# ssheybani/baby-vision-curriculum

Hardware: AMD Instinct MI355X
Metric: video clips/sec (node) VideoMAE-base 16x224^2 bf16 pretraining (higher is better)
Workload: dtype bf16; 1 GPU; VideoMAE-base (ViT-B/16 encoder, 4-layer decoder), 16x224x224 clips, tubelet 2, 90% tube mask, full training step (fwd + MSE + bwd + GradScaler + SGD-Nesterov); clips_per_gpu=256, global_batch=256, parallelism=dp1, weights=random init N(0,0.02), seed 0

## Files before the change

### baby-vision-curriculum_amd/_lib.py

```python
import ctypes
import os
import sys

_HERE = os.path.dirname(os.path.abspath(__file__))
LIB_PATH = os.environ.get("BVC_LIB_PATH") or os.path.join(_HERE, "libbvc_hip.so")

c_void_p, c_int, c_int64, c_float, c_char_p = ctypes.c_void_p, ctypes.c_int, ctypes.c_int64, ctypes.c_float, ctypes.c_char_p
c_double = ctypes.c_double


class BvcError(RuntimeError):
    pass


class VideoMAEConfigC(ctypes.Structure):
    _fields_ = [(n, c_int) for n in (
        "image_size", "patch_size", "num_channels", "num_frames", "tubelet_size",
        "hidden_size", "num_hidden_layers", "num_attention_heads", "intermediate_size",
        "decoder_hidden_size", "decoder_num_hidden_layers", "decoder_num_attention_heads",
        "decoder_intermediate_size")] + [("layer_norm_eps", c_float), ("decoder_norm_eps", c_float),
                                         ("norm_pix_loss", c_int)]


class VitConfigC(ctypes.Structure):
# ... 110 lines not shown
                                        c_void_p]),
    "bvc_videomae_forward_dual": (c_int, [c_void_p, c_void_p, ctypes.POINTER(PixelFormatC), c_void_p, c_void_p, c_int, c_void_p, c_void_p,
                                          c_void_p, c_void_p]),
    "bvc_videomae_backward": (c_int, [c_void_p, c_void_p, c_void_p, BUCKET_FN, c_void_p, c_void_p]),
    "bvc_videomae_tap": (c_int, [c_void_p, c_char_p, c_void_p, c_int64, ctypes.POINTER(c_int64), c_void_p]),
    "bvc_videomae_encoder_param_numel": (c_int64, [ctypes.POINTER(VideoMAEConfigC)]),
    "bvc_videomae_encoder_create": (c_int, [ctypes.POINTER(VideoMAEConfigC), c_int, ctypes.POINTER(c_void_p)]),
    "bvc_videomae_encoder_destroy": (None, [c_void_p]),
    "bvc_videomae_encode": (c_int, [c_void_p, c_void_p, c_int, c_void_p, c_void_p, c_void_p, c_float, c_void_p, c_void_p, c_void_p]),
    "bvc_videomae_encode_px": (c_int, [c_void_p, c_void_p, ctypes.POINTER(PixelFormatC), c_int, c_void_p, c_void_p, c_void_p, c_float,
                                       c_void_p, c_void_p, c_void_p]),
    "bvc_videomae_encode_ex": (c_int, [c_void_p, c_void_p, ctypes.POINTER(PixelFormatC), c_int, c_void_p, c_void_p, c_void_p, c_float,
                                       c_void_p, c_void_p, ctypes.POINTER(IntrospectC), c_void_p]),
    "bvc_videomae_cls_introspect": (c_int, [c_void_p, ctypes.POINTER(IntrospectC), c_void_p]),
    "bvc_videomae_encoder_fc_norm_backward": (c_int, [c_void_p, c_void_p, c_void_p, c_void_p, c_void_p, c_void_p]),
    "bvc_videomae_cls_create": (c_int, [ctypes.POINTER(VideoMAEConfigC), c_int, ctypes.POINTER(c_void_p)]),
    "bvc_videomae_cls_destroy": (None, [c_void_p]),
    "bvc_videomae_cls_forward_px": (c_int, [c_void_p, c_void_p, ctypes.POINTER(PixelFormatC), c_int, c_void_p, c_void_p, c_void_p,
                                            c_float, c_void_p, c_void_p, c_void_p]),
    "bvc_videomae_cls_backward": (c_int, [c_void_p, c_void_p, c_void_p, c_void_p, c_void_p, BUCKET_FN, c_void_p, c_void_p]),
    "bvc_videomae_cls_shadow": (c_int, [c_void_p, c_int, ctypes.POINTER(c_void_p), ctypes.POINTER(c_int64)]),
    "bvc_vit_param_count":(c_int, [ctypes.POINTER(VitConfigC)]),
    "bvc_vit_param_numel": (c_int64, [ctypes.POINTER(VitConfigC)]),
    "bvc_vit_param_info": (c_int, [ctypes.POINTER(VitConfigC), c_int, ctypes.c_char_p, c_int, ctypes.POINTER(c_int64),
                                   ctypes.POINTER(c_int64), ctypes.POINTER(c_int), ctypes.POINTER(c_int64)]),
    "bvc_vit_create": (c_int, [ctypes.POINTER(VitConfigC), c_int, ctypes.POINTER(c_void_p)]),
    "bvc_vit_destroy": (None, [c_void_p]),
    "bvc_vit_forward": (c_int, [c_void_p, c_void_p, c_void_p, c_int, c_int, c_void_p, c_void_p, c_void_p]),
    "bvc_vit_forward_px": (c_int, [c_void_p, c_void_p, ctypes.POINTER(PixelFormatC), c_void_p, c_int, c_int, c_void_p, c_void_p, c_void_p]),
    "bvc_vit_backward": (c_int, [c_void_p, c_void_p, c_void_p, BUCKET_FN, c_void_p, c_void_p]),
    "bvc_predictor_param_count": (c_int, [ctypes.POINTER(PredictorConfigC)]),
    "bvc_predictor_param_numel": (c_int64, [ctypes.POINTER(PredictorConfigC)]),
    "bvc_predictor_param_info": (c_int, [ctypes.POINTER(PredictorConfigC), c_int, ctypes.c_char_p, c_int, ctypes.POINTER(c_int64),
                                         ctypes.POINTER(c_int64), ctypes.POINTER(c_int), ctypes.POINTER(c_int64)]),
    "bvc_predictor_create": (c_int, [ctypes.POINTER(PredictorConfigC), c_int, c_int, c_int, ctypes.POINTER(c_void_p)]),
    "bvc_predictor_destroy": (None, [c_void_p]),
    "bvc_predictor_forward": (c_int, [c_void_p, c_void_p, c_void_p, c_void_p, c_int, c_int, c_int, c_int, c_void_p, c_void_p, c_void_p]),
    "bvc_predictor_backward": (c_int, [c_void_p, c_void_p, c_void_p, c_void_p, c_void_p]),
    "bvc_predictor_backward_cb": (c_int, [c_void_p, c_void_p, c_void_p, c_void_p, BUCKET_FN, c_void_p, c_void_p]),
    "bvc_op_target_select": (c_int, [c_void_p, c_void_p, c_void_p, c_int, c_int, c_int, c_int, c_int, c_float, c_void_p]),
    "bvc_op_smooth_l1_workspace": (c_int, [c_int64]),
    "bvc_op_smooth_l1_fwd": (c_int, [c_void_p, c_void_p, c_int64, c_void_p, c_void_p, c_void_p]),
    "bvc_op_smooth_l1_bwd": (c_int, [c_void_p, c_void_p, c_void_p, c_int64, c_void_p, c_void_p]),
    "bvc_op_ema": (c_int, [c_void_p, c_void_p, c_int64, c_float, c_void_p]),
    "bvc_op_token_mean": (c_int, [c_void_p, c_int, c_int, c_int, c_void_p, c_void_p]),
    "bvc_op_token_mean_bwd": (c_int, [c_void_p, c_int, c_int, c_int, c_void_p, c_void_p]),
    "bvc_op_gemm": (c_int, [ctypes.POINTER(GemmDesc), c_int, c_int, c_int, c_int, c_void_p]),
    "bvc_op_gemm_num_tiles": (c_int, [ctypes.POINTER(GemmDesc), c_int]),
    "bvc_op_gemm_kernel": (c_int, [ctypes.POINTER(GemmDesc), c_int, c_int, c_int, c_int, ctypes.c_char_p, c_int]),
    "bvc_op_gemm_plan_dw": (c_int, [ctypes.POINTER(GemmDesc), c_int]),
    "bvc_op_gemm_gate": (c_int, [ctypes.POINTER(GemmDesc), ctypes.POINTER(BranchDropC), c_int, c_int, c_int, c_void_p]),
    "bvc_op_gemm_gate_kernel": (c_int, [ctypes.POINTER(GemmDesc), c_int, ctypes.c_char_p, c_int]),
    "bvc_op_layernorm_bwd_gate": (c_int, [c_void_p, c_void_p, c_void_p, c_void_p, c_void_p, c_void_p, c_int, c_void_p, c_void_p, c_void_p,
                                          c_void_p, c_int, c_int, ctypes.POINTER(BranchDropC), c_int, c_int, c_void_p]),
    "bvc_op_dropout_mask": (c_int, [ctypes.c_uint64, ctypes.c_uint64, c_int, c_int, c_int, c_int, c_float, c_void_p, c_void_p]),
    "bvc_dropout_mask_host": (c_int, [ctypes.c_uint64, ctypes.c_uint64, c_int, c_int, c_int, c_int, c_float, c_void_p]),
    "bvc_op_clip_transform_workspace": (c_int64, [c_int, c_int, c_int]),
    "bvc_op_clip_transform": (c_int, [c_void_p, c_int, c_int, c_int, c_int, c_void_p, c_void_p, c_int, c_int, c_int, c_void_p, c_void_p, c_void_p]),
    "bvc_clip_transform_host": (c_int, [c_void_p, c_int, c_int, c_int, c_int, c_void_p, c_int, c_int, c_int, c_void_p]),
    "bvc_aug_blur_weights": (c_int, [c_float, ctypes.POINTER(ctypes.c_int32), ctypes.POINTER(ctypes.c_uint32), ctypes.POINTER(ctypes.c_uint32)]),
    "bvc_op_clip_post_workspace": (c_int64, [c_int, c_int, c_int]),
    "bvc_op_clip_post": (c_int, [c_void_p, c_void_p, c_void_p, c_int, c_int, c_int, c_void_p, c_void_p, c_void_p]),
    "bvc_clip_post_host": (c_int, [c_void_p, c_void_p, c_int, c_int, c_int, c_void_p]),
    "bvc_videomae_cls_set_drop": (c_int, [c_void_p, ctypes.POINTER(BranchDropC), c_int, c_void_p]),
    "bvc_videomae_encoder_set_drop": (c_int, [c_void_p, ctypes.POINTER(BranchDropC), c_int, c_void_p]),
    "bvc_videomae_cls_set_mix": (c_int, [c_void_p, c_void_p, c_int, c_void_p]),
    "bvc_videomae_encoder_set_mix": (c_int, [c_void_p, c_void_p, c_int, c_void_p]),
    "bvc_vit_set_drop": (c_int, [c_void_p, ctypes.POINTER(BranchDropC), c_int, c_void_p]),
    "bvc_predictor_set_drop": (c_int, [c_void_p, ctypes.POINTER(BranchDropC), c_int, c_void_p]),
    "bvc_op_attention_fwd": (c_int, [c_void_p, c_void_p, c_void_p, c_int, c_int, c_int, c_int, c_void_p]),
    "bvc_op_attention_bwd": (c_int, [c_void_p, c_void_p, c_void_p, c_void_p, c_void_p, c_void_p, c_int, c_int, c_int, c_int, c_void_p]),
    "bvc_op_attention_bwd_part": (c_int, [c_void_p, c_void_p, c_void_p, c_void_p, c_void_p, c_void_p, c_int, c_int, c_int, c_int, c_int, c_void_p]),
    "bvc_op_attention_width": (c_int, [c_int]),
    "bvc_op_attention_fwd_scaled": (c_int, [c_void_p, c_void_p, c_void_p, c_int, c_int, c_int, c_int, ctypes.c_float, c_void_p]),
    "bvc_op_attention_bwd_scaled": (c_int, [c_void_p, c_void_p, c_void_p, c_void_p, c_void_p, c_void_p, c_int, c_int, c_int, c_int,
                                            ctypes.c_float, c_void_p]),
    "bvc_op_attention_probs": (c_int, [c_void_p, c_void_p, c_void_p, c_int, c_int, c_int, c_int, ctypes.c_float, c_void_p]),
    "bvc_op_layernorm_fwd": (c_int, [c_void_p, c_int, c_int, c_int, c_void_p, c_void_p, c_void_p, c_void_p, c_void_p,
                                     c_int, c_int, c_float, c_void_p]),
    "bvc_op_layernorm_bwd": (c_int, [c_void_p, c_void_p, c_int, c_int, c_int, c_void_p, c_void_p, c_void_p, c_void_p,
                                     c_int, c_void_p, c_void_p, c_void_p, c_void_p, c_int, c_int, c_void_p]),
    "bvc_op_layernorm_bwd_workspace": (c_int64, [c_int, c_int]),
    "bvc_op_colsum_bf16": (c_int, [c_void_p, c_int, c_int, c_int, c_float, c_void_p, c_void_p, c_void_p]),
    "bvc_op_colsum_f32": (c_int, [c_void_p, c_int, c_int, c_int, c_int, c_int, c_void_p, c_void_p]),
    "bvc_op_cast_bf16": (c_int, [c_void_p, c_void_p, c_int64, c_void_p]),
    "bvc_op_row_normalize": (c_int, [c_void_p, c_void_p, c_void_p, c_int, c_int, c_float, c_void_p]),
    "bvc_op_row_normalize_bwd": (c_int, [c_void_p, c_void_p, c_void_p, c_void_p, c_int, c_int, c_void_p]),
    "bvc_op_nce_finalize": (c_int, [c_void_p, c_int, c_float, c_int64, c_void_p, c_void_p, c_void_p]),
    "bvc_op_sgd_step": (c_int, [c_void_p, c_void_p, c_void_p, c_int64, c_float, c_float, c_float, c_float, c_int, c_int, c_int,
                                c_void_p, c_void_p, c_int, c_void_p, c_void_p]),
    "bvc_videomae_shadow": (c_int, [c_void_p, c_int, ctypes.POINTER(c_void_p), ctypes.POINTER(c_int64)]),
    "bvc_vit_shadow": (c_int, [c_void_p, c_int, ctypes.POINTER(c_void_p), ctypes.POINTER(c_int64)]),
    "bvc_predictor_shadow": (c_int, [c_void_p, c_int, ctypes.POINTER(c_void_p), ctypes.POINTER(c_int64)]),
    "bvc_op_adam_prepare": (c_int, [c_void_p, c_double, c_double, c_double, c_void_p, c_void_p]),
    "bvc_op_adam_step": (c_int, [c_void_p, c_void_p, c_void_p, c_void_p, c_int64, c_double, c_double, c_double, c_double, c_double,
                                 c_int, c_int, c_void_p, c_void_p, c_void_p, c_int, c_void_p, c_void_p]),
    "bvc_op_row_ln_selected": (c_int, [c_int, c_int, c_int, c_int]),
    "bvc_op_sgd_step_segments": (c_int, [c_void_p, c_void_p, c_void_p, c_int64, c_void_p, c_void_p, c_void_p, c_int, c_void_p, c_void_p, c_void_p,
                                         c_int, c_void_p, c_void_p]),
    "bvc_op_adam_step_segments": (c_int, [c_void_p, c_void_p, c_void_p, c_void_p, c_int64, c_void_p, c_void_p, c_void_p, c_int, c_void_p, c_void_p,
                                          c_void_p, c_void_p, c_void_p, c_int, c_void_p, c_void_p]),
    "bvc_op_sgd_step_table": (c_int, [c_void_p, c_void_p, c_void_p, c_int64, c_void_p, c_void_p, c_void_p, c_int, c_int] + [c_void_p] * 7 +
                                      [c_void_p, c_void_p, c_void_p, c_int, c_void_p, c_void_p]),
    "bvc_op_adam_step_table": (c_int, [c_void_p, c_void_p, c_void_p, c_void_p, c_int64, c_void_p, c_void_p, c_void_p, c_int, c_int] + [c_void_p] * 7 +
                                       [c_void_p, c_void_p, c_void_p, c_void_p, c_int, c_void_p, c_void_p]),
    "bvc_op_lars_step_table": (c_int, [c_void_p, c_void_p, c_void_p, c_int64, c_void_p, c_void_p, c_void_p, c_int, c_void_p, c_int64, c_void_p,
                                       c_int] + [c_void_p] * 7 + [c_void_p, c_void_p, c_void_p, c_void_p, c_void_p, c_int, c_void_p, c_void_p]),
    "bvc_op_lamb_step_table": (c_int, [c_void_p, c_void_p, c_void_p, c_void_p, c_int64, c_void_p, c_void_p, c_void_p, c_int, c_void_p, c_int64,
                                       c_void_p, c_int] + [c_void_p] * 7 +
                                      [c_void_p, c_void_p, c_void_p, c_void_p, c_void_p, c_void_p, c_int, c_void_p, c_void_p]),
    "bvc_op_nonfinite_check": (c_int, [c_void_p, c_int64, c_void_p, c_void_p]),
    "bvc_op_grad_norm_item_cap": (c_int, []),
    "bvc_op_grad_norm_chain": (c_int, []),
    "bvc_grad_norm_items_host": (c_int, [c_void_p, c_void_p, c_int, c_void_p, c_int64, c_void_p, ctypes.POINTER(c_int64)]),
    "bvc_op_grad_sqnorm_items": (c_int, [c_void_p, c_void_p, c_int64, c_void_p, c_int, c_void_p, c_void_p, c_void_p, c_int, c_void_p, c_void_p]),
    "bvc_op_clip_finalize": (c_int, [c_void_p, c_int, c_float, c_void_p, c_void_p, c_void_p]),
    "bvc_op_scale_by_dev": (c_int, [c_void_p, c_int64, c_void_p, c_void_p]),
    "bvc_op_mask_index": (c_int, [c_void_p, c_int, c_int, c_int, c_int, c_void_p, c_void_p, c_void_p, c_void_p]),
    "bvc_op_dual_mask_index": (c_int, [c_void_p, c_void_p, c_int, c_int, c_int, c_int, c_void_p, c_void_p, c_void_p, c_void_p]),
    "bvc_op_gather_patches": (c_int, [c_void_p, c_void_p, c_void_p, c_int, c_int, c_int, c_int, c_int, c_int, c_int, c_int, c_void_p]),
    "bvc_op_gather_patches_mix": (c_int, [c_void_p, ctypes.POINTER(PixelFormatC), c_void_p, c_void_p, c_void_p, c_int, c_int, c_int, c_int,
                                          c_int, c_int, c_int, c_int, c_void_p]),
    "bvc_op_pixel_labels": (c_int, [c_void_p, c_void_p, c_void_p, c_int, c_int, c_int, c_int, c_int, c_int, c_int, c_int, c_int, c_void_p]),
    "bvc_comm_unique_id": (c_int, [c_void_p]),
    "bvc_comm_init": (c_int, [c_int, c_int, c_void_p, ctypes.POINTER(c_void_p)]),
    "bvc_comm_destroy": (c_int, [c_void_p]),
    "bvc_comm_stream": (c_void_p, [c_void_p]),
    "bvc_comm_rank": (c_int, [c_void_p]),
    "bvc_comm_world": (c_int, [c_void_p]),
    "bvc_comm_library": (c_char_p, []),
    "bvc_allreduce_bucket": (c_int, [c_void_p, c_void_p, c_int64, c_int, c_void_p]),
    "bvc_comm_wait": (c_int, [c_void_p, c_void_p]),
    "bvc_allgather": (c_int, [c_void_p, c_void_p, c_void_p, c_int64, c_void_p]),
    "bvc_allreduce": (c_int, [c_void_p, c_void_p, c_int64, c_int, c_void_p]),
    "bvc_broadcast": (c_int, [c_void_p, c_void_p, c_int64, c_int, c_void_p]),
}

_lib = None

_det_flag = False
_det_pushed = False


def use_deterministic_algorithms(mode):
    global _det_flag
    _det_flag = bool(mode)
    lib()


def are_deterministic_algorithms_enabled():
    return _det_flag


def _sync_deterministic(L):
    global _det_pushed
    torch = sys.modules.get("torch")
    want = _det_flag or (torch is not None and torch.are_deterministic_algorithms_enabled())
    if want != _det_pushed:
        rc = L.bvc_set_option(b"deterministic", 1 if want else 0)
        if rc != 0:
            raise BvcError(f"bvc_set_option(deterministic) failed with status {rc}")
        _det_pushed = want


def lib():
    global _lib
# ... 32 lines not shown
```

### baby-vision-curriculum_amd/csrc/context.h

```cpp
#pragma once
#include <functional>

#include "stack.h"

namespace bvc {

struct Shadow {
    bf16_t* wbf = nullptr;
    int64_t numel = 0;
    bool valid = false;
    int alloc(Arena& a, int64_t n) { numel = n; return a.alloc(&wbf, (size_t)n); }
    int refresh(const float* params, hipStream_t st);
    int query(int vouch, void** p, int64_t* n);
};

struct MixState {
    ClipMix* table = nullptr;
    int* status = nullptr;
    const bvc_clip_mix* armed = nullptr;
    int samples = 0;
};
int alloc_mix(Arena& a, MixState& m, int max_batch);
int set_mix(MixState& m, const bvc_clip_mix* mix, int samples, int max_batch, const char* who);

template <typename Config>
PatchGeom patch_geom(const Config& c) { return PatchGeom{c.num_frames, c.num_channels, c.image_size, c.image_size, c.tubelet_size, c.patch_size}; }
inline int seq_len(PatchGeom g) { return (g.T / g.ts) * (g.H / g.ps) * (g.W / g.ps); }
inline int patch_dim(PatchGeom g) { return g.C * g.ts * g.ps * g.ps; }
int pixel_src(const char* who, const void* pixels, const bvc_pixel_format* fmt, int channels, PixelSrc* out);

struct PatchFront {
    PatchGeom pg;
    int L = 0, Kp = 0;
    int* idx_all = nullptr;
    bf16_t* Ape = nullptr;
    int alloc(Arena& a, PatchGeom geom, size_t max_tokens, bool identity_list);
    int embed(PixelSrc px, const int* idx, int B, int N, const bf16_t* w, const float* bias, const float* pos, float* out, int D,
              hipStream_t st, const char* who, MixState* mix = nullptr, bool* mixed = nullptr);
    int embed_backward(Work& w, int M, int D, float* gw, float* gb, hipStream_t st);
};

int stack_forward(Work& w, Stack& s, const std::vector<LayerOff>& off, int B, int N, hipStream_t st, bool chain_ln, const LayerTail* last = nullptr);
int stack_backward(Work& w, Stack& s, const std::vector<LayerOff>& off, float* dres, float* G, int B, int N, hipStream_t st,
                   bvc_bucket_fn on_bucket, void* user, const LayerTail* last = nullptr);
int join_both(Work& w, hipStream_t st, bvc_bucket_fn on_bucket, void* user);

int param_info(const ParamTable& t, int index, char* name, int name_cap, int64_t* offset, int64_t* numel, int* ndim, int64_t shape[5]);

struct Making {
    std::function<void()> undo;
    bool done = false;
    ~Making() { if (!done) undo(); }
};
int refuse_operand_extent(const char* who, int max_batch, size_t tokens_per_clip, size_t bf16_columns, const char* side_name);

}
```

### baby-vision-curriculum_amd/csrc/context.hip

```cpp
#include "context.h"

#include <stdio.h>

namespace bvc {

int Shadow::refresh(const float* params, hipStream_t st) {
    const bool vouched = valid;
    valid = false;
    return vouched ? BVC_OK : launch_cast_bf16(params, wbf, (size_t)numel, st);
}

int Shadow::query(int vouch, void** p, int64_t* n) {
    if (p) *p = wbf;
    if (n) *n = numel;
    if (vouch >= 0) valid = vouch != 0;
    return BVC_OK;
}

int alloc_mix(Arena& a, MixState& m, int max_batch) {
    TRY(a.alloc(&m.table, (size_t)max_batch));
    return a.alloc(&m.status, 4);
}

int set_mix(MixState& m, const bvc_clip_mix* mix, int samples, int max_batch, const char* who) {
    m.armed = nullptr;
    if (!mix) return BVC_OK;
    BVC_REQUIRE(samples >= 1 && samples <= max_batch, "%s: %d samples outside [1, %d]", who, samples, max_batch);
    m.armed = mix;
    m.samples = samples;
    return BVC_OK;
}

static int gather_for_forward(MixState& m, bool* mixed, PixelSrc pixels, const int* idx, bf16_t* A, int B, int N, PatchGeom pg, const char* who,
                              hipStream_t st) {
    const bvc_clip_mix* src = m.armed;
    m.armed = nullptr;
    *mixed = src != nullptr;
    if (!src) return launch_gather_patches(pixels, idx, A, B, N, pg, st);
    BVC_REQUIRE(m.samples == B, "%s: the mix was set for %d samples, the call has %d", who, m.samples, B);
    BVC_CHECK_HIP(hipMemcpyAsync(m.table, src, (size_t)B * sizeof(ClipMix), hipMemcpyDeviceToDevice, st));
    BVC_CHECK_HIP(hipMemsetAsync(m.status, 0, 4, st));
    return launch_gather_patches_mix(pixels, idx, A, B, N, pg, m.table, st, m.status);
}

int pixel_src(const char* who, const void* pixels, const bvc_pixel_format* fmt, int channels, PixelSrc* out) {
    PixelSrc px = pixels_f32((const float*)pixels);
    if (fmt && fmt->dtype != BVC_PIXELS_F32) {
        BVC_REQUIRE(fmt->dtype == BVC_PIXELS_U8, "%s: pixel format: dtype %d unknown", who, fmt->dtype);
        BVC_REQUIRE(channels <= 4, "%s: pixel format: uint8 input supports at most 4 channels", who);
        px.is_u8 = 1;
        for (int c = 0; c < 4; ++c) {
            BVC_REQUIRE(fmt->std[c] != 0.f || c >= channels, "%s: pixel format: std[%d] is zero", who, c);
            px.mean[c] = fmt->mean[c];
            px.stdv[c] = c < channels ? fmt->std[c] : 1.f;
        }
    }
    *out = px;
    return BVC_OK;
}

int PatchFront::alloc(Arena& a, PatchGeom geom, size_t max_tokens, bool identity_list) {
    pg = geom;
    L = seq_len(geom);
    Kp = patch_dim(geom);
    TRY(a.alloc(&Ape, max_tokens * Kp));
    if (!identity_list) return BVC_OK;
    TRY(a.alloc(&idx_all, max_tokens));
    TRY(launch_iota_mod(idx_all, (int)max_tokens, L, nullptr));
    BVC_CHECK_HIP(hipStreamSynchronize(nullptr));
    return BVC_OK;
}

int PatchFront::embed(PixelSrc px, const int* idx, int B, int N, const bf16_t* w, const float* bias, const float* pos, float* out, int D,
                      hipStream_t st, const char* who, MixState* mix, bool* mixed) {
    if (mix) TRY(gather_for_forward(*mix, mixed, px, idx, Ape, B, N, pg, who, st));
    else TRY(launch_gather_patches(px, idx, Ape, B, N, pg, st));
    const int M = B * N;
    GemmProblem p = gemm(Ape, (size_t)M * Kp, Kp, w, (size_t)D * Kp, Kp, M, D, Kp, EPI_POS, out, D);
    p.bias = bias; p.rowtok = idx; p.pos = pos;
    return launch_gemm(&p, 1, GEMM_NT, -1, st);
}

int PatchFront::embed_backward(Work& w, int M, int D, float* gw, float* gb, hipStream_t st) {
    GemmProblem p = gemm(w.dyb[w.seq % 3], (size_t)M * D, D, Ape, (size_t)M * Kp, Kp, D, Kp, M, EPI_F32, gw, Kp);
    p.rowsum = gb;
    const int tile = plan_dw(&p, 1);
    return launch_gemm(&p, 1, GEMM_TN, tile, st);
}

int stack_forward(Work& w, Stack& s, const std::vector<LayerOff>& off, int B, int N, hipStream_t st, bool chain_ln, const LayerTail* last) {
    for (int i = 0; i < s.nlayers; ++i) {
        const bool end = i + 1 == s.nlayers;
        TRY(layer_forward(w, s, i, off[i], s.act[i].x_in, end ? s.x_out : s.act[i + 1].x_in, B, N, st, chain_ln && !end ? &off[i + 1] : nullptr,
                          end ? last : nullptr));
    }
    return BVC_OK;
}

int stack_backward(Work& w, Stack& s, const std::vector<LayerOff>& off, float* dres, float* G, int B, int N, hipStream_t st,
                   bvc_bucket_fn on_bucket, void* user, const LayerTail* last) {
    for (int i = s.nlayers - 1; i >= 0; --i)
        TRY(layer_backward(w, s, i, off[i], s.act[i].x_in, dres, G, B, N, st, on_bucket, user, i + 1 == s.nlayers ? last : nullptr));
    return BVC_OK;
}

int join_both(Work& w, hipStream_t st, bvc_bucket_fn on_bucket, void* user) {
    TRY(join_side(w, w.seq & 1, st, on_bucket, user));
    return join_side(w, (w.seq + 1) & 1, st, on_bucket, user);
}

int param_info(const ParamTable& t, int index, char* name, int name_cap, int64_t* offset, int64_t* numel, int* ndim, int64_t shape[5]) {
    BVC_REQUIRE(index >= 0 && index < (int)t.entries.size(), "param_info: index %d out of range", index);
    const ParamEntry& e = t.entries[index];
    snprintf(name, name_cap, "%s", e.name.c_str());
    *offset = e.offset; *numel = e.numel; *ndim = e.ndim;
    for (int i = 0; i < 5; ++i) shape[i] = e.shape[i];
    return BVC_OK;
}

int refuse_operand_extent(const char* who, int max_batch, size_t tokens_per_clip, size_t bf16_columns, const char* side_name) {
    const size_t per_clip = tokens_per_clip * bf16_columns * 2, bytes = (size_t)max_batch * per_clip;
    const size_t limit = 0x100000000ull - operand_tail_bytes(bf16_columns);
    if (bytes <= limit) return BVC_OK;
    char side[32] = "";
    if (side_name) snprintf(side, sizeof(side), "the %s's ", side_name);
    set_error("%s: max_batch %d exceeds the 4 GiB operand extent: %s%zu tokens x %zu bf16 columns are %.2f GiB; at most %zu clips", who, max_batch,
              side, (size_t)max_batch * tokens_per_clip, bf16_columns, bytes / 1073741824.0, limit / per_clip);
    return BVC_ERR_INVALID;
}

}
```

### baby-vision-curriculum_amd/csrc/gemm.h

```cpp
#pragma once
#include "common.h"
#include "dropgate.h"
#include "../../include/bvc.h"

namespace bvc {

enum GemmLayout { GEMM_NT = BVC_GEMM_NT, GEMM_NN = BVC_GEMM_NN, GEMM_TN = BVC_GEMM_TN };

enum GemmEpilogue {
    EPI_F32 = BVC_EPI_F32,
    EPI_BF16 = BVC_EPI_BF16,
    EPI_GELU = BVC_EPI_GELU,
    EPI_RESID = BVC_EPI_RESID,
    EPI_POS = BVC_EPI_POS,
    EPI_E2D = BVC_EPI_E2D,
    EPI_LOSS = BVC_EPI_LOSS,
    EPI_DGELU = BVC_EPI_DGELU,
    EPI_F32_BF16 = BVC_EPI_F32_BF16,
    EPI_RELU = BVC_EPI_RELU,
    EPI_DRELU = BVC_EPI_DRELU,
    EPI_NCE = BVC_EPI_NCE,
    EPI_NCE_BWD = BVC_EPI_NCE_BWD,
    EPI_RESID_LN = BVC_EPI_RESID_LN,
    EPI_DLN = BVC_EPI_DLN,
    EPI_RESID_GATE = BVC_EPI_RESID_GATE
};

using GemmProblem = bvc_gemm_desc;

constexpr int kMaxGroup = 4;

struct Options { int gemm8 = 0; int dw_overlap = 0; int row_ln = 0; int row_stagger = 1; int deterministic = 0; int head_pad = 0; int dec_tail = 1; };
Options& options();

float* det_scratch(size_t floats, hipStream_t stream);
size_t det_scratch_bytes();
int det_scratch_release();

struct DryRun { bool on = false; char name[160] = ""; };
DryRun& dry_run();

constexpr size_t operand_tail_bytes(size_t bf16_columns) { return 64 * bf16_columns * 2 + 1024; }
constexpr bool tn_tail_ok(int K, int ld) { return K % 64 == 0 || ((size_t)K + 63) / 64 * 64 * (size_t)ld * 2 + 1024 <= 0x100000000ull; }

int launch_gemm(const GemmProblem* probs, int nprob, GemmLayout layout, int tile_cfg, hipStream_t stream, int stages = -1);

int launch_gemm_gate(const GemmProblem& p, const Gate& gate, int tile_cfg, hipStream_t stream);

int gemm_num_tiles(const GemmProblem& p, int tile_cfg);
int gemm_pick_tile(const GemmProblem* probs, int nprob, int tile_cfg);
bool gemm_row_ln_ok(int M, int N, int K);
constexpr size_t kRowLnPartFloats = 512 * 2 * 384;

}
```

### baby-vision-curriculum_amd/csrc/ops.hip

```cpp
#include <stdarg.h>
#include <stdio.h>
#include <string.h>

#include "context.h"
#include "optim_layerwise.h"

namespace bvc {
static thread_local char g_err[1024] = "";
void set_error(const char* fmt, ...) {
    va_list ap;
    va_start(ap, fmt);
    vsnprintf(g_err, sizeof(g_err), fmt, ap);
    va_end(ap);
}
const char* last_error() { return g_err; }
}

using namespace bvc;

extern "C" {

const char* bvc_last_error(void) { return bvc::last_error(); }
const char* bvc_version(void) { return "gfx950;bvc-hip-r5"; }

int bvc_set_option(const char* name, int value) {
    BVC_REQUIRE(name != nullptr, "set_option: null name");
    if (!strcmp(name, "gemm8")) { BVC_REQUIRE(value >= -1 && value <= 1, "set_option: gemm8 takes -1 / 0 / 1"); options().gemm8 = value; }
    else if (!strcmp(name, "dw_overlap")) options().dw_overlap = value != 0;
    else if (!strcmp(name, "row_stagger")) options().row_stagger = value != 0;
    else if (!strcmp(name, "row_ln")) { BVC_REQUIRE(value >= -1 && value <= 1, "set_option: row_ln takes -1 / 0 / 1"); options().row_ln = value; }
    else if (!strcmp(name, "deterministic")) { BVC_REQUIRE(value == 0 || value == 1, "set_option: deterministic takes 0 / 1"); options().deterministic = value; }
    else if (!strcmp(name, "head_pad")) { BVC_REQUIRE(value == 0 || value == 1, "set_option: head_pad takes 0 / 1"); options().head_pad = value; }
    else if (!strcmp(name, "dec_tail")) { BVC_REQUIRE(value == 0 || value == 1, "set_option: dec_tail takes 0 / 1"); options().dec_tail = value; }
    else BVC_REQUIRE(false, "set_option: unknown option '%s'", name);
    return BVC_OK;
}
int bvc_get_option(const char* name) {
    if (name && !strcmp(name, "gemm8")) return options().gemm8;
    if (name && !strcmp(name, "dw_overlap")) return options().dw_overlap;
    if (name && !strcmp(name, "row_ln")) return options().row_ln;
    if (name && !strcmp(name, "row_stagger")) return options().row_stagger;
    if (name && !strcmp(name, "deterministic")) return options().deterministic;
    if (name && !strcmp(name, "head_pad")) return options().head_pad;
    if (name && !strcmp(name, "dec_tail")) return options().dec_tail;
    bvc::set_error("get_option: unknown option '%s'", name ? name : "(null)");
    return BVC_ERR_INVALID;
}

int bvc_op_gemm(const bvc_gemm_desc* problems, int count, int layout, int tile_cfg, int stages, void* stream) {
    BVC_REQUIRE(problems, "op_gemm: null problems");
    BVC_REQUIRE(layout >= 0 && layout <= 2, "op_gemm: bad layout %d", layout);
    return launch_gemm(problems, count, (GemmLayout)layout, tile_cfg, (hipStream_t)stream, stages);
}
static int op_gate(const bvc_branch_drop* drop, int layer, int branch, int M, Gate* g) {
    BVC_REQUIRE(drop && layer >= 0 && layer < (1 << 22) && (branch == 0 || branch == 1), "gate: null description, or layer / branch out of range");
    BVC_REQUIRE(drop->hidden_p >= 0.f && drop->hidden_p < 1.f && drop->rows_per_sample >= 1, "gate: hidden_p outside [0, 1) or rows_per_sample < 1");
    const int samples = (M + drop->rows_per_sample - 1) / drop->rows_per_sample;
    *g = make_gate(drop->hidden_p, drop->seed, drop->offset,
                   drop->path_scale ? drop->path_scale + ((size_t)layer * 2 + branch) * samples : nullptr, drop->rows_per_sample, layer, branch);
    return BVC_OK;
}
int bvc_op_gemm_gate(const bvc_gemm_desc* problem, const bvc_branch_drop* drop, int layer, int branch, int tile_cfg, void* stream) {
    BVC_REQUIRE(problem, "op_gemm_gate: null problem");
    Gate g;
    TRY(op_gate(drop, layer, branch, problem->M, &g));
    return launch_gemm_gate(*problem, g, tile_cfg, (hipStream_t)stream);
}
int bvc_op_gemm_gate_kernel(const bvc_gemm_desc* problem, int tile_cfg, char* name, int name_cap) {
    BVC_REQUIRE(problem && name && name_cap > 0, "op_gemm_gate_kernel: null argument");
    DryRun& d = dry_run();
    d.on = true;
    d.name[0] = 0;
    const int rc = launch_gemm_gate(*problem, make_gate(0.f, 0, 0, nullptr, 1, 0, 0), tile_cfg, nullptr);
    d.on = false;
    if (rc == BVC_OK) snprintf(name, name_cap, "%s", d.name);
    return rc;
}
int bvc_op_dropout_mask(uint64_t seed, uint64_t offset, int layer, int branch, int M, int N, float p, uint8_t* out_dev, void* stream) {
    BVC_REQUIRE(out_dev && M >= 1 && N >= 1 && layer >= 0 && layer < (1 << 22) && (branch == 0 || branch == 1) && p >= 0.f && p < 1.f,
                "op_dropout_mask: bad argument");
    return launch_dropout_mask(make_gate(p, seed, offset, nullptr, 1, layer, branch), (size_t)M * N, out_dev, (hipStream_t)stream);
}
int bvc_dropout_mask_host(uint64_t seed, uint64_t offset, int layer, int branch, int M, int N, float p, uint8_t* out_host) {
    BVC_REQUIRE(out_host && M >= 1 && N >= 1 && layer >= 0 && layer < (1 << 22) && (branch == 0 || branch == 1) && p >= 0.f && p < 1.f,
                "dropout_mask_host: bad argument");
    dropout_mask_host(make_gate(p, seed, offset, nullptr, 1, layer, branch), (size_t)M * N, out_host);
    return BVC_OK;
}
int bvc_op_layernorm_bwd_gate(const void* dy, const float* x, const float* mean, const float* rstd, const float* gamma, float* dres,
                              int accumulate, void* dres_bf16, float* dgamma, float* dbeta, float* workspace, int M, int D,
                              const bvc_branch_drop* drop, int layer, int branch, void* stream) {
    Gate g;
    TRY(op_gate(drop, layer, branch, M, &g));
    return launch_ln_bwd((const bf16_t*)dy, x, identity_rows(), mean, rstd, gamma, dres, accumulate, (bf16_t*)dres_bf16, dgamma, dbeta,
                         workspace, M, D, (hipStream_t)stream, &g);
}
int bvc_op_gemm_kernel(const bvc_gemm_desc* problems, int count, int layout, int tile_cfg, int stages, char* name, int name_cap) {
    BVC_REQUIRE(problems && name && name_cap > 0, "op_gemm_kernel: null argument");
    BVC_REQUIRE(layout >= 0 && layout <= 2, "op_gemm_kernel: bad layout %d", layout);
    DryRun& d = dry_run();
    d.on = true;
    d.name[0] = 0;
    const int rc = launch_gemm(problems, count, (GemmLayout)layout, tile_cfg, nullptr, stages);
    d.on = false;
    if (rc == BVC_OK) snprintf(name, name_cap, "%s", d.name);
    return rc;
}
int64_t bvc_deterministic_workspace_bytes(void) { return (int64_t)det_scratch_bytes(); }
int bvc_deterministic_workspace_release(void) { return det_scratch_release(); }
int bvc_op_gemm_plan_dw(bvc_gemm_desc* problems, int count) {
    BVC_REQUIRE(problems && count >= 1 && count <= 4, "op_gemm_plan_dw: bad argument");
    return plan_dw(problems, count);
}
int bvc_op_gemm_num_tiles(const bvc_gemm_desc* problem, int tile_cfg) {
    if (!problem) return BVC_ERR_INVALID;
    return gemm_num_tiles(*problem, tile_cfg);
}
int bvc_op_attention_fwd(const void* qkv, void* ctx_out, float* lse, int B, int N, int H, int head_dim, void* stream) {
    BVC_REQUIRE(qkv && ctx_out && lse, "op_attention_fwd: null argument");
    return launch_attn_fwd((const bf16_t*)qkv, (bf16_t*)ctx_out, lse, B, N, H, head_dim, (hipStream_t)stream);
}
int bvc_op_attention_bwd(const void* qkv, const void* ctx_in, const void* dctx, const float* lse, float* delta, void* dqkv,
                         int B, int N, int H, int head_dim, void* stream) {
    BVC_REQUIRE(qkv && ctx_in && dctx && lse && delta && dqkv, "op_attention_bwd: null argument");
    return launch_attn_bwd((const bf16_t*)qkv, (const bf16_t*)ctx_in, (const bf16_t*)dctx, lse, delta, (bf16_t*)dqkv, B, N, H, head_dim,
                           (hipStream_t)stream);
}
int bvc_op_attention_bwd_part(const void* qkv, const void* ctx_in, const void* dctx, const float* lse, float* delta, void* dqkv,
                              int B, int N, int H, int head_dim, int part, void* stream) {
    BVC_REQUIRE(qkv && ctx_in && dctx && lse && delta && dqkv, "op_attention_bwd_part: null argument");
    BVC_REQUIRE(part == 1 || part == 2, "op_attention_bwd_part: part is 1 (dQ + delta) or 2 (dK, dV)");
    return launch_attn_bwd((const bf16_t*)qkv, (const bf16_t*)ctx_in, (const bf16_t*)dctx, lse, delta, (bf16_t*)dqkv, B, N, H, head_dim,
                           (hipStream_t)stream, 0.f, part);
}
int bvc_op_attention_width(int head_dim) {
    BVC_REQUIRE(head_dim > 0 && head_dim <= 128 && head_dim % 8 == 0, "op_attention_width: head_dim %d unsupported", head_dim);
    return attn_width(head_dim);
}
int bvc_op_attention_fwd_scaled(const void* qkv, void* ctx_out, float* lse, int B, int N, int H, int head_dim, float softmax_scale,
                                void* stream) {
    BVC_REQUIRE(qkv && ctx_out && lse && softmax_scale >= 0.f, "op_attention_fwd_scaled: bad argument");
    return launch_attn_fwd((const bf16_t*)qkv, (bf16_t*)ctx_out, lse, B, N, H, head_dim, (hipStream_t)stream, softmax_scale);
}
int bvc_op_attention_bwd_scaled(const void* qkv, const void* ctx_in, const void* dctx, const float* lse, float* delta, void* dqkv,
                                int B, int N, int H, int head_dim, float softmax_scale, void* stream) {
    BVC_REQUIRE(qkv && ctx_in && dctx && lse && delta && dqkv && softmax_scale >= 0.f, "op_attention_bwd_scaled: bad argument");
    return launch_attn_bwd((const bf16_t*)qkv, (const bf16_t*)ctx_in, (const bf16_t*)dctx, lse, delta, (bf16_t*)dqkv, B, N, H, head_dim,
                           (hipStream_t)stream, softmax_scale);
}
int bvc_op_attention_probs(const void* qkv, const float* lse, float* probs, int B, int N, int H, int head_dim, float softmax_scale,
                           void* stream) {
    BVC_REQUIRE(qkv && lse && probs && softmax_scale >= 0.f, "op_attention_probs: bad argument");
    return launch_attn_probs((const bf16_t*)qkv, lse, probs, B, N, H, head_dim, (hipStream_t)stream, softmax_scale);
}
int bvc_op_layernorm_fwd(const float* x, int rin, int rout, int roff, const float* gamma, const float* beta, void* y,
                         float* mean, float* rstd, int M, int D, float eps, void* stream) {
    BVC_REQUIRE(x && gamma && beta && y && mean && rstd, "op_layernorm_fwd: null argument");
    return launch_ln_fwd(x, RowMap{rin, rout, roff}, gamma, beta, (bf16_t*)y, mean, rstd, M, D, eps, (hipStream_t)stream);
}
int bvc_op_layernorm_bwd(const void* dy, const float* x, int rin, int rout, int roff, const float* mean, const float* rstd,
                         const float* gamma, float* dres, int accumulate, void* dres_bf16, float* dgamma, float* dbeta,
                         float* workspace, int M, int D, void* stream) {
    BVC_REQUIRE(dy && x && mean && rstd && gamma && dres && dgamma && dbeta && workspace, "op_layernorm_bwd: null argument");
    return launch_ln_bwd((const bf16_t*)dy, x, RowMap{rin, rout, roff}, mean, rstd, gamma, dres, accumulate, (bf16_t*)dres_bf16,
                         dgamma, dbeta, workspace, M, D, (hipStream_t)stream);
}
int64_t bvc_op_layernorm_bwd_workspace(int M, int D) { return (int64_t)ln_bwd_workspace_floats(M, D); }
int bvc_op_colsum_f32(const float* X, int rin, int rout, int roff, int M, int D, float* out, void* stream) {
    BVC_REQUIRE(X && out && M > 0 && D > 0, "op_colsum_f32: bad argument");
    return launch_colsum_f32(X, RowMap{rin, rout, roff}, M, D, out, (hipStream_t)stream);
}
int bvc_op_colsum_bf16(const void* X, int M, int N, int ld, float alpha, const float* alpha_dev, float* out, void* stream) {
    BVC_REQUIRE(X && out, "op_colsum_bf16: null argument");
    return launch_colsum_bf16_scaled((const bf16_t*)X, M, N, ld, alpha, alpha_dev, out, (hipStream_t)stream);
}
int bvc_op_sgd_step(float* params, float* grads, float* momentum_buf, int64_t n, float lr, float momentum, float dampening,
                    float weight_decay, int nesterov, int first_step, int maximize, const float* grad_scale,
                    const float* found_inf, int write_unscaled_grads, void* bf16_shadow, void* stream) {
    BVC_REQUIRE(params && grads && n >= 0, "op_sgd_step: bad argument");
    return launch_sgd_step(params, grads, momentum_buf, (size_t)n, lr, momentum, dampening, weight_decay, nesterov, first_step,
                           maximize, grad_scale, found_inf, write_unscaled_grads, (bf16_t*)bf16_shadow, (hipStream_t)stream);
}
int bvc_op_adam_prepare(float* state3, double lr, double beta1, double beta2, const float* found_inf, void* stream) {
    BVC_REQUIRE(state3, "op_adam_prepare: null state");
    return launch_adam_prep(state3, lr, beta1, beta2, found_inf, (hipStream_t)stream);
}
int bvc_op_adam_step(float* params, float* grads, float* exp_avg, float* exp_avg_sq, int64_t n, double lr, double beta1, double beta2,
                     double eps, double weight_decay, int decoupled, int maximize, const float* state3, const float* grad_scale,
                     const float* found_inf, int write_unscaled_grads, void* bf16_shadow, void* stream) {
    BVC_REQUIRE(params && grads && exp_avg && exp_avg_sq && state3 && n >= 0, "op_adam_step: bad argument");
    return launch_adam_step(params, grads, exp_avg, exp_avg_sq, (size_t)n, lr, beta1, beta2, eps, weight_decay, decoupled, maximize,
                            state3, grad_scale, found_inf, write_unscaled_grads, (bf16_t*)bf16_shadow, (hipStream_t)stream);
}
int bvc_op_row_ln_selected(int tokens, int width, int mlp_width, int heads) {
    if (tokens <= 0 || width <= 0 || heads <= 0 || width % heads != 0) return 0;
    Stack s;
    s.D = width; s.I = mlp_width; s.H = heads; s.nlayers = 0; s.eps = 0.f; s.x_out = nullptr;
    s.hd = width / heads; s.hdp = attn_width(s.hd); s.Da = heads * s.hdp;
    return fuse_row_ln(s, tokens) ? 1 : 0;
}
int bvc_op_sgd_step_segments(float* params, float* grads, float* momentum_buf, int64_t n, const int64_t* seg_start, const int32_t* seg_group,
                             const int32_t* blk_seg, int nseg, const bvc_sgd_groups* groups, const float* grad_scale, const float* found_inf,
                             int write_unscaled_grads, void* bf16_shadow, void* stream) {
    BVC_REQUIRE(params && grads && n >= 0, "op_sgd_step_segments: bad argument");
    return launch_sgd_step_segments(params, grads, momentum_buf, n, seg_start, seg_group, blk_seg, nseg, groups, grad_scale, found_inf,
                                    write_unscaled_grads, (bf16_t*)bf16_shadow, (hipStream_t)stream);
}
int bvc_op_adam_step_segments(float* params, float* grads, float* exp_avg, float* exp_avg_sq, int64_t n, const int64_t* seg_start,
                              const int32_t* seg_group, const int32_t* blk_seg, int nseg, const bvc_adam_groups* groups, float* state,
                              double* hyper_scratch, const float* grad_scale, const float* found_inf, int write_unscaled_grads,
                              void* bf16_shadow, void* stream) {
    BVC_REQUIRE(params && grads && exp_avg && exp_avg_sq && n >= 0, "op_adam_step_segments: bad argument");
    return launch_adam_step_segments(params, grads, exp_avg, exp_avg_sq, n, seg_start, seg_group, blk_seg, nseg, groups, state, hyper_scratch,
                                     grad_scale, found_inf, write_unscaled_grads, (bf16_t*)bf16_shadow, (hipStream_t)stream);
}
int bvc_op_sgd_step_table(float* params, float* grads, float* momentum_buf, int64_t n, const int64_t* seg_start, const int32_t* seg_group,
                          const int32_t* blk_seg, int nseg, int ngroups, const float* lr, const float* momentum, const float* dampening,
                          const float* weight_decay, const int32_t* nesterov, const int32_t* first_step, const int32_t* maximize,
                          float* group_table, const float* grad_scale, const float* found_inf, int write_unscaled_grads,
                          void* bf16_shadow, void* stream) {
    BVC_REQUIRE(params && grads && n >= 0, "op_sgd_step_table: bad argument");
    return launch_sgd_step_table(params, grads, momentum_buf, n, seg_start, seg_group, blk_seg, nseg, ngroups, lr, momentum, dampening,
                                 weight_decay, nesterov, first_step, maximize, group_table, grad_scale, found_inf, write_unscaled_grads,
                                 (bf16_t*)bf16_shadow, (hipStream_t)stream);
}
int bvc_op_adam_step_table(float* params, float* grads, float* exp_avg, float* exp_avg_sq, int64_t n, const int64_t* seg_start,
                           const int32_t* seg_group, const int32_t* blk_seg, int nseg, int ngroups, const double* lr, const double* beta1,
                           const double* beta2, const double* eps, const double* weight_decay, const int32_t* decoupled,
                           const int32_t* maximize, float* state, float* group_table, const float* grad_scale, const float* found_inf,
                           int write_unscaled_grads, void* bf16_shadow, void* stream) {
    BVC_REQUIRE(params && grads && exp_avg && exp_avg_sq && n >= 0, "op_adam_step_table: bad argument");
    return launch_adam_step_table(params, grads, exp_avg, exp_avg_sq, n, seg_start, seg_group, blk_seg, nseg, ngroups, lr, beta1, beta2, eps,
                                  weight_decay, decoupled, maximize, state, group_table, grad_scale, found_inf, write_unscaled_grads,
                                  (bf16_t*)bf16_shadow, (hipStream_t)stream);
}
int bvc_op_nonfinite_check(const float* x, int64_t n, float* found_inf, void* stream) {
    BVC_REQUIRE(x && found_inf && n >= 0, "op_nonfinite_check: bad argument");
    return launch_nonfinite_check(x, (size_t)n, found_inf, (hipStream_t)stream);
}
int bvc_op_grad_norm_item_cap(void) { return BVC_GRAD_NORM_ITEM_CAP; }
int bvc_op_grad_norm_chain(void) { return grad_norm_chain(); }
int bvc_grad_norm_items_host(const int64_t* seg_start, const int32_t* seg_group, int nseg, bvc_norm_item* items, int64_t items_cap,
                             int64_t* seg_first_item, int64_t* nitems) {
    BVC_REQUIRE(nseg >= 0 && nitems && (nseg == 0 || (seg_start && seg_group)) && (items == nullptr || items_cap >= 0),
                "grad_norm_items_host: bad argument");
    return grad_norm_items_host(seg_start, seg_group, nseg, items, items_cap, seg_first_item, nitems);
}
int bvc_op_grad_sqnorm_items(const float* x, const bvc_norm_item* items, int64_t nitems, const int64_t* seg_first_item, int nseg,
                             double* item_partial, float* seg_sq, float* total_sq, int as_norm, float* found_inf, void* stream) {
    BVC_REQUIRE(x && total_sq && nitems >= 0, "op_grad_sqnorm_items: bad argument");
    return launch_grad_sqnorm_items(x, items, nitems, seg_first_item, nseg, item_partial, seg_sq, total_sq, as_norm, found_inf,
                                    (hipStream_t)stream);
}
int bvc_op_clip_finalize(const float* sq, int nranges, float max_norm, const float* grad_scale, float* out3, void* stream) {
    BVC_REQUIRE(out3 && nranges >= 0 && (nranges == 0 || sq) && !(max_norm < 0.f) && max_norm == max_norm, "op_clip_finalize: bad argument");
    return launch_clip_finalize(sq, nranges, max_norm, grad_scale, out3, (hipStream_t)stream);
}
int bvc_op_scale_by_dev(float* x, int64_t n, const float* coef, void* stream) {
    BVC_REQUIRE(x && coef && n >= 0 && ((uintptr_t)x % 4) == 0, "op_scale_by_dev: bad argument");
    return launch_scale_by_dev(x, (size_t)n, coef, (hipStream_t)stream);
}
int bvc_op_lars_step_table(float* params, float* grads, float* momentum_buf, int64_t n, const int64_t* seg_start, const int32_t* seg_group,
                           const int32_t* blk_seg, int nseg, const bvc_norm_item* items, int64_t nitems, const int64_t* seg_first_item,
                           int ngroups, const float* lr, const float* momentum, const float* weight_decay, const float* trust_coefficient,
                           const int32_t* nesterov, const int32_t* adapt, const int32_t* maximize, float* group_table, double* item_partial,
                           float* seg_stats, const float* grad_scale, float* found_inf, int write_unscaled_grads, void* bf16_shadow,
                           void* stream) {
    BVC_REQUIRE(params && grads && n >= 0, "op_lars_step_table: bad argument");
    return launch_lars_step_table(params, grads, momentum_buf, n, seg_start, seg_group, blk_seg, nseg, items, nitems, seg_first_item, ngroups,
                                  lr, momentum, weight_decay, trust_coefficient, nesterov, adapt, maximize, group_table, item_partial,
                                  seg_stats, grad_scale, found_inf, write_unscaled_grads, (bf16_t*)bf16_shadow, (hipStream_t)stream);
}
int bvc_op_lamb_step_table(float* params, float* grads, float* exp_avg, float* exp_avg_sq, int64_t n, const int64_t* seg_start,
                           const int32_t* seg_group, const int32_t* blk_seg, int nseg, const bvc_norm_item* items, int64_t nitems,
                           const int64_t* seg_first_item, int ngroups, const double* lr, const double* beta1, const double* beta2,
                           const double* eps, const double* weight_decay, const int32_t* adapt, const int32_t* maximize, float* state,
                           float* group_table, double* item_partial, float* seg_stats, const float* grad_scale, const float* found_inf,
                           int write_unscaled_grads, void* bf16_shadow, void* stream) {
    BVC_REQUIRE(params && grads && exp_avg && exp_avg_sq && n >= 0, "op_lamb_step_table: bad argument");
    return launch_lamb_step_table(params, grads, exp_avg, exp_avg_sq, n, seg_start, seg_group, blk_seg, nseg, items, nitems, seg_first_item,
                                  ngroups, lr, beta1, beta2, eps, weight_decay, adapt, maximize, state, group_table, item_partial, seg_stats,
                                  grad_scale, found_inf, write_unscaled_grads, (bf16_t*)bf16_shadow, (hipStream_t)stream);
}
int bvc_op_row_normalize(const float* f, void* fn_bf16, float* inv_norm, int n, int p, float eps, void* stream) {
    BVC_REQUIRE(f && fn_bf16 && inv_norm, "op_row_normalize: null argument");
    return launch_row_normalize(f, (bf16_t*)fn_bf16, inv_norm, n, p, eps, (hipStream_t)stream);
}
int bvc_op_row_normalize_bwd(const float* f, const float* inv_norm, const float* dfn, float* df, int n, int p, void* stream) {
    BVC_REQUIRE(f && inv_norm && dfn && df, "op_row_normalize_bwd: null argument");
    return launch_row_normalize_bwd(f, inv_norm, dfn, df, n, p, (hipStream_t)stream);
}
int bvc_op_nce_finalize(const float* partial, int ntiles, float inv_temperature, int64_t npos, float* loss, float* stats, void* stream) {
    BVC_REQUIRE(partial && loss && stats && ntiles > 0 && npos > 0, "op_nce_finalize: bad argument");
    return launch_nce_finalize(partial, ntiles, inv_temperature, (double)npos, loss, stats, (hipStream_t)stream);
}
int bvc_op_cast_bf16(const float* in, void* out, int64_t n, void* stream) {
    BVC_REQUIRE(in && out && n >= 0, "op_cast_bf16: bad argument");
    return launch_cast_bf16(in, (bf16_t*)out, (size_t)n, (hipStream_t)stream);
}
int bvc_op_mask_index(const uint8_t* mask, int B, int L, int nvis, int nmask, int* vis_idx, int* msk_idx, int* status, void* stream) {
    BVC_REQUIRE(mask && vis_idx && msk_idx && status, "op_mask_index: null argument");
    return launch_mask_index(mask, B, L, nvis, nmask, vis_idx, msk_idx, status, (hipStream_t)stream);
}
int bvc_op_dual_mask_index(const uint8_t* mask, const uint8_t* decode_mask, int B, int L, int nvis, int ndec, int* vis_idx, int* dec_idx,
                           int* status, void* stream) {
    BVC_REQUIRE(mask && decode_mask && vis_idx && dec_idx && status, "op_dual_mask_index: null argument");
    BVC_REQUIRE(B >= 1 && L >= 1 && nvis >= 1 && nvis < L && ndec >= 1 && ndec <= L - nvis, "op_dual_mask_index: bad counts (L %d, nvis %d, ndec %d)", L, nvis, ndec);
    return launch_dual_mask_index(mask, decode_mask, B, L, nvis, ndec, vis_idx, dec_idx, status, (hipStream_t)stream);
}
int bvc_op_gather_patches(const float* clip, const int* vis_idx, void* A, int B, int nvis, int T, int C, int H, int W, int ts,
                          int ps, void* stream) {
    BVC_REQUIRE(clip && vis_idx && A, "op_gather_patches: null argument");
    return launch_gather_patches(pixels_f32(clip), vis_idx, (bf16_t*)A, B, nvis, PatchGeom{T, C, H, W, ts, ps}, (hipStream_t)stream);
}
int bvc_op_gather_patches_mix(const void* clip, const bvc_pixel_format* fmt, const int* idx, void* A, const bvc_clip_mix* mix, int B, int n,
                              int T, int C, int H, int W, int ts, int ps, void* stream) {
    BVC_REQUIRE(clip && idx && A && mix, "op_gather_patches_mix: null argument");
    BVC_REQUIRE(T >= 1 && C >= 1 && H >= 1 && W >= 1 && ts >= 1 && ps >= 1 && T % ts == 0 && H % ps == 0 && W % ps == 0,
                "op_gather_patches_mix: bad geometry");
    PixelSrc px;
    TRY(pixel_src("op_gather_patches_mix", clip, fmt, C, &px));
    return launch_gather_patches_mix(px, idx, (bf16_t*)A, B, n, PatchGeom{T, C, H, W, ts, ps}, mix, (hipStream_t)stream);
}
int bvc_op_pixel_labels(const float* clip, const int* msk_idx, float* labels, int B, int nmask, int T, int C, int H, int W, int ts,
                        int ps, int norm_pix, void* stream) {
    BVC_REQUIRE(clip && msk_idx && labels, "op_pixel_labels: null argument");
    return launch_labels(pixels_f32(clip), msk_idx, labels, B, nmask, PatchGeom{T, C, H, W, ts, ps}, norm_pix, (hipStream_t)stream);
}

int bvc_op_target_select(const float* h, const int* idx_pred, float* out, int nsets, int B, int Np, int L, int D, float eps, void* stream) {
    BVC_REQUIRE(h && idx_pred && out, "op_target_select: null argument");
    return launch_target_select(h, idx_pred, out, nsets, B, Np, L, D, eps, (hipStream_t)stream);
}
int bvc_op_smooth_l1_workspace(int64_t n) { return smooth_l1_blocks((size_t)n); }
int bvc_op_smooth_l1_fwd(const float* z, const float* h, int64_t n, float* workspace, float* loss, void* stream) {
    BVC_REQUIRE(z && h && workspace && loss && n > 0, "op_smooth_l1_fwd: bad argument");
    return launch_smooth_l1_fwd(z, h, (size_t)n, workspace, loss, (hipStream_t)stream);
}
int bvc_op_smooth_l1_bwd(const float* z, const float* h, const float* grad_loss, int64_t n, float* dz, void* stream) {
    BVC_REQUIRE(z && h && grad_loss && dz && n > 0, "op_smooth_l1_bwd: bad argument");
    return launch_smooth_l1_bwd(z, h, grad_loss, (size_t)n, dz, (hipStream_t)stream);
}
int bvc_op_ema(float* target, const float* online, int64_t n, float momentum, void* stream) {
    BVC_REQUIRE(target && online && n >= 0, "op_ema: bad argument");
    return launch_ema(target, online, (size_t)n, momentum, (hipStream_t)stream);
}

int bvc_op_token_mean(const float* x, int batch, int ntok, int dim, float* out, void* stream) {
    BVC_REQUIRE(x && out && batch > 0 && ntok > 0 && dim > 0, "op_token_mean: bad argument");
    return launch_token_mean(x, batch, ntok, dim, out, (hipStream_t)stream);
}
int bvc_op_token_mean_bwd(const float* dmean, int batch, int ntok, int dim, float* dx, void* stream) {
    BVC_REQUIRE(dmean && dx && batch > 0 && ntok > 0 && dim > 0, "op_token_mean_bwd: bad argument");
    return launch_token_mean_bwd(dmean, batch, ntok, dim, dx, (hipStream_t)stream);
}

}
```

### baby-vision-curriculum_amd/csrc/rowops.h

```cpp
#pragma once
#include "common.h"
#include "dropgate.h"

namespace bvc {

struct RowMap { int rin, rout, roff; };
static inline RowMap identity_rows() { return RowMap{0, 0, 0}; }

struct PatchGeom { int T, C, H, W, ts, ps; };

struct PixelSrc {
    const void* ptr;
    int is_u8;
    float mean[4], stdv[4];
};
static inline PixelSrc pixels_f32(const float* p) { return PixelSrc{p, 0, {0, 0, 0, 0}, {1, 1, 1, 1}}; }

int launch_ln_fwd(const float* x, RowMap rm, const float* gamma, const float* beta, bf16_t* y, float* mean, float* rstd,
                  int M, int D, float eps, hipStream_t s, float* y32 = nullptr);
size_t ln_bwd_workspace_floats(int M, int D);
size_t ln_bwd_workspace_floats_upto(int Mmax, int D);
int launch_ln_bwd(const bf16_t* dy, const float* x, RowMap rm, const float* mean, const float* rstd, const float* gamma,
                  float* dres, int accumulate, bf16_t* dres_bf, float* dgamma, float* dbeta, float* part, int M, int D, hipStream_t s,
                  const Gate* gate = nullptr,
                  bool compact_x = false);
int launch_ln_param_reduce(const float* part, int nblk, int D, float* dgamma, float* dbeta, hipStream_t s);
int launch_colsum_bf16(const bf16_t* X, int M, int N, int ld, float alpha, float* out, hipStream_t s);
int launch_colsum_bf16_scaled(const bf16_t* X, int M, int N, int ld, float alpha, const float* alpha_dev, float* out, hipStream_t s);
int launch_colsum_f32(const float* X, RowMap rm, int M, int D, float* out, hipStream_t s);
int launch_token_mean(const float* x, int B, int N, int D, float* out, hipStream_t s);
int launch_token_mean_bwd(const float* dmean, int B, int N, int D, float* dx, hipStream_t s);
int launch_fcnorm_bwd_bcast(const float* dy, const float* p, const float* mean, const float* rstd, const float* gamma, float* dres,
                            bf16_t* dres_bf, float* dgamma, float* dbeta, int B, int N, int D, hipStream_t s, const Gate* gate = nullptr);
int launch_dropout_mask(const Gate& gate, size_t n, uint8_t* out, hipStream_t s);
void dropout_mask_host(const Gate& gate, size_t n, uint8_t* out);
int launch_cast_bf16(const float* in, bf16_t* out, size_t n, hipStream_t s);
int launch_gather_rows_bf16(const float* in, RowMap rm, bf16_t* out, int M, int D, hipStream_t s);
int launch_mask_index(const uint8_t* mask, int B, int L, int nvis, int nmask, int* vis_idx, int* msk_idx, int* status, hipStream_t s);
int launch_dual_mask_index(const uint8_t* mask, const uint8_t* decode, int B, int L, int nvis, int ndec, int* vis_idx, int* dec_idx,
                           int* status, hipStream_t s);
int launch_gather_patches(PixelSrc clip, const int* vis_idx, bf16_t* A, int B, int nvis, PatchGeom pg, hipStream_t s);
typedef bvc_clip_mix ClipMix;
int launch_gather_patches_mix(PixelSrc clip, const int* idx, bf16_t* A, int B, int n, PatchGeom pg, const ClipMix* mix, hipStream_t s,
                              int* status = nullptr);
int launch_poison_on_status(float* x, size_t count, const int* status, hipStream_t s);
int launch_labels(PixelSrc clip, const int* dec_idx, float* labels, int B, int ndec, PatchGeom pg, int norm_pix, hipStream_t s);
int launch_fill_masked(float* xfull, const float* mask_token, const float* pos, const int* dec_idx, int B, int Ld, int nvis,
                       int ndec, int D, hipStream_t s);
int launch_sgd_step(float* p, float* g, float* buf, size_t n, float lr, float momentum, float dampening, float wd, int nesterov,
                    int first, int maximize, const float* grad_scale, const float* found_inf, int write_grad, bf16_t* shadow,
                    hipStream_t s);
int launch_adam_prep(float* state, double lr, double beta1, double beta2, const float* found_inf, hipStream_t s);
int launch_adam_step(float* p, float* g, float* m, float* v, size_t n, double lr, double beta1, double beta2, double eps, double wd,
                     int decoupled, int maximize, const float* state, const float* grad_scale, const float* found_inf, int write_grad,
                     bf16_t* shadow, hipStream_t s);
int launch_sgd_step_segments(float* p, float* g, float* buf, int64_t n, const int64_t* seg_start, const int* seg_group, const int* blk_seg,
                             int nseg, const bvc_sgd_groups* groups, const float* grad_scale, const float* found_inf, int write_grad,
                             bf16_t* shadow, hipStream_t s);
int launch_adam_step_segments(float* p, float* g, float* m, float* v, int64_t n, const int64_t* seg_start, const int* seg_group,
                              const int* blk_seg, int nseg, const bvc_adam_groups* groups, float* state, double* hyper_dev,
                              const float* grad_scale, const float* found_inf, int write_grad, bf16_t* shadow, hipStream_t s);
int launch_sgd_step_table(float* p, float* g, float* buf, int64_t n, const int64_t* seg_start, const int* seg_group, const int* blk_seg,
                          int nseg, int ngroups, const float* lr, const float* momentum, const float* dampening, const float* wd,
                          const int* nesterov, const int* first_step, const int* maximize, float* table, const float* grad_scale,
                          const float* found_inf, int write_grad, bf16_t* shadow, hipStream_t s);
int launch_adam_step_table(float* p, float* g, float* m, float* v, int64_t n, const int64_t* seg_start, const int* seg_group,
                           const int* blk_seg, int nseg, int ngroups, const double* lr, const double* beta1, const double* beta2,
                           const double* eps, const double* wd, const int* decoupled, const int* maximize, float* state, float* table,
                           const float* grad_scale, const float* found_inf, int write_grad, bf16_t* shadow, hipStream_t s);
int launch_pad_heads(const bf16_t* wqkv, const float* bqkv, const bf16_t* wo, bf16_t* wqkv_p, float* bqkv_p, bf16_t* wo_p, int D, int H,
                     int hd, int hdp, hipStream_t s);
int launch_unpad_head_grads(const float* gwqkv_p, const float* gbqkv_p, const float* gwo_p, float* gwqkv, float* gbqkv, float* gwo, int D,
                            int H, int hd, int hdp, hipStream_t s);
int launch_nonfinite_check(const float* x, size_t n, float* found_inf, hipStream_t s);
int grad_norm_chain();
int grad_norm_items_host(const int64_t* seg_start, const int32_t* seg_group, int nseg, bvc_norm_item* items, int64_t items_cap,
                         int64_t* seg_first_item, int64_t* nitems);
int launch_grad_sqnorm_items(const float* x, const bvc_norm_item* items, int64_t nitems, const int64_t* seg_first_item, int nseg,
                             double* item_partial, float* seg_sq, float* total_sq, int as_norm, float* found_inf, hipStream_t s);
int launch_clip_finalize(const float* sq, int nranges, float max_norm, const float* grad_scale, float* out3, hipStream_t s);
int launch_scale_by_dev(float* x, size_t n, const float* coef, hipStream_t s);
int launch_row_normalize(const float* f, bf16_t* fn, float* inv, int n, int p, float eps, hipStream_t s);
int launch_row_normalize_bwd(const float* f, const float* inv, const float* dfn, float* df, int n, int p, hipStream_t s);
int launch_nce_finalize(const float* partial, int ntiles, float inv_t, double npos, float* loss, float* stats, hipStream_t s);
int launch_target_select(const float* h, const int* idx, float* out, int nsets, int B, int Np, int L, int D, float eps, hipStream_t s);
int launch_pred_assemble(const float* xe, const float* mask_token, const float* pos, const int* idx_pred, float* X, int nsets, int B,
                         int Nc, int Np, int D, hipStream_t s);
int launch_pred_ctx_grad(const float* dX, bf16_t* dxe, int nsets, int B, int Nc, int Np, int D, hipStream_t s);
int smooth_l1_blocks(size_t n);
int launch_smooth_l1_fwd(const float* z, const float* h, size_t n, float* partial, float* loss, hipStream_t s);
int launch_smooth_l1_bwd(const float* z, const float* h, const float* gout, size_t n, float* dz, hipStream_t s);
int launch_ema(float* k, const float* q, size_t n, float m, hipStream_t s);
int launch_iota_mod(int* idx, int n, int L, hipStream_t s);
int launch_loss_finalize(const float* partial, int n, double count, const int* status, float* loss, hipStream_t s);

}
```

### baby-vision-curriculum_amd/csrc/rowops.hip

```cpp
#include "rowops.h"
#include "gemm.h"

#include <algorithm>

namespace bvc {

constexpr int kMaxChunks = 4;
constexpr int kWideChunks = 6;

__device__ __forceinline__ int map_row(int m, RowMap rm) {
    return rm.rin > 0 ? (m / rm.rin) * rm.rout + rm.roff + (m % rm.rin) : m;
}

template <int LPR>
__device__ __forceinline__ float row_sum(float v) {
#pragma unroll
    for (int o = LPR / 2; o > 0; o >>= 1) v += __shfl_xor(v, o, 64);
    return v;
}

template <int LPR, int NC>
__global__ __launch_bounds__(256) void ln_fwd_kernel(const float* __restrict__ x, RowMap rm, const float* __restrict__ gamma,
                                                     const float* __restrict__ beta, bf16_t* __restrict__ y, float* __restrict__ y32,
                                                     float* __restrict__ mean, float* __restrict__ rstd, int M, int D, float eps) {
// ... 676 lines not shown

template <int NE>
__global__ __launch_bounds__(256, 6) void labels_wave3_kernel(const PixelSrc clip, const int* __restrict__ dec_idx, float* __restrict__ labels,
                                                              int ntok, int ndec, PatchGeom pg, int norm_pix) {
    extern __shared__ __attribute__((aligned(16))) char smem[];
    constexpr int C = 3, E = 256 * NE, CE = C * E, NCH = C * NE;
    const int lane = threadIdx.x & 63, wave = threadIdx.x >> 6;
    float* buf = reinterpret_cast<float*>(smem) + wave * CE;
    const int nb = gridDim.x, xq = nb >> 3, xr = nb & 7, xcd = blockIdx.x & 7;
    const int blk = (xcd < xr ? xcd * (xq + 1) : xr * (xq + 1) + (xcd - xr) * xq) + (blockIdx.x >> 3);
    const int m = blk * 4 + wave;
    if (m >= ntok) return;
    const int b = m / ndec, tok = dec_idx[m];
    const int wp = pg.W / pg.ps, hp = pg.H / pg.ps;
    const int tp = tok / (hp * wp), yp = (tok / wp) % hp, xp = tok % wp;
    const float mean3[3] = {0.485f, 0.456f, 0.406f}, std3[3] = {0.229f, 0.224f, 0.225f};
    f32x4 v[NCH];
#pragma unroll
    for (int k = 0; k < NCH; ++k) {
        constexpr int e4n = E / 4;
        const int i = lane + 64 * k;
        const int c = k / NE, e = (i - c * e4n) * 4;
        const int dx = e % pg.ps, dy = (e / pg.ps) % pg.ps, dt = e / (pg.ps * pg.ps);
        const size_t src = ((((size_t)b * pg.T + tp * pg.ts + dt) * C + c) * pg.H + yp * pg.ps + dy) * pg.W + xp * pg.ps + dx;
        v[k] = load_pixels4(clip, src, c);
    }
    float mu[3], rinv[3];
#pragma unroll
    for (int c = 0; c < C; ++c) {
        float sm = 0.f;
#pragma unroll
        for (int k = c * NE; k < (c + 1) * NE; ++k) {
            v[k] = v[k] * std3[c] + mean3[c];
            *reinterpret_cast<f32x4*>(buf + c * E + (lane + 64 * (k - c * NE)) * 4) = v[k];
            sm += (v[k][0] + v[k][1]) + (v[k][2] + v[k][3]);
        }
        const float mean = wave_sum(sm) * (1.0f / E);
        float q = 0.f;
#pragma unroll
        for (int k = c * NE; k < (c + 1) * NE; ++k)
#pragma unroll
            for (int j = 0; j < 4; ++j) { const float d = v[k][j] - mean; q += d * d; }
        const float var = wave_sum(q) / (float)(E - 1);
        mu[c] = norm_pix ? mean : 0.f;
        rinv[c] = norm_pix ? 1.0f / (sqrtf(var) + 1e-6f) : 1.f;
    }
    const int l3 = lane % 3;
    float mr[3], rr[3];
#pragma unroll
    for (int i = 0; i < 3; ++i) {
        const int c = l3 + i;
        mr[i] = (c == 0 || c == 3) ? mu[0] : (c == 1 || c == 4) ? mu[1] : mu[2];
        rr[i] = (c == 0 || c == 3) ? rinv[0] : (c == 1 || c == 4) ? rinv[1] : rinv[2];
    }
    __builtin_amdgcn_fence(__ATOMIC_RELEASE, "wavefront");
    __builtin_amdgcn_wave_barrier();
    __builtin_amdgcn_fence(__ATOMIC_ACQUIRE, "wavefront");
    float* out = labels + (size_t)m * CE;
#pragma unroll
    for (int k = 0; k < CE / 256; ++k) {
        const int o = lane * 4 + 256 * k;
        f32x4 r;
#pragma unroll
        for (int j = 0; j < 4; ++j) {
            const int t = o + j, e = t / 3, c = t - 3 * e;
            r[j] = (buf[c * E + e] - mr[(k + j) % 3]) * rr[(k + j) % 3];
        }
        *reinterpret_cast<f32x4*>(out + o) = r;
    }
}

__global__ void fill_masked_kernel(float* __restrict__ xfull, const float* __restrict__ mask_token, const float* __restrict__ pos,
                                   const int* __restrict__ dec_idx, int B, int Ld, int nvis, int ndec, int D) {
    const size_t i = (size_t)blockIdx.x * blockDim.x + threadIdx.x;
    const int nch = D >> 2;
    if (i >= (size_t)B * ndec * nch) return;
    const int m = (int)(i / nch), c = (int)(i % nch);
    const int b = m / ndec, j = m % ndec;
    const f32x4 mt = reinterpret_cast<const f32x4*>(mask_token)[c];
    const f32x4 pe = reinterpret_cast<const f32x4*>(pos + (size_t)dec_idx[m] * D)[c];
    reinterpret_cast<f32x4*>(xfull + ((size_t)b * Ld + nvis + j) * D)[c] = mt + pe;
}

__global__ __launch_bounds__(256) void loss_finalize_kernel(const float* __restrict__ partial, int n, double count,
                                                            const int* __restrict__ status, float* __restrict__ loss) {
    __shared__ double red[256];
    double s = 0.0;
    for (int i = threadIdx.x; i < n; i += 256) s += (double)partial[i];
    red[threadIdx.x] = s;
    __syncthreads();
    for (int o = 128; o > 0; o >>= 1) {
        if (threadIdx.x < o) red[threadIdx.x] += red[threadIdx.x + o];
        __syncthreads();
    }
    if (threadIdx.x == 0) *loss = (status && *status) ? __int_as_float(0x7fc00000) : (float)(red[0] / count);
}

template <int NC>
__global__ __launch_bounds__(256) void target_select_kernel(const float* __restrict__ h, const int* __restrict__ idx,
                                                            float* __restrict__ out, int rows, int B, int Np, int L, int D, float eps) {
    const int lane = threadIdx.x & 63, m = blockIdx.x * 4 + (threadIdx.x >> 6);
    if (m >= rows) return;
    const int b = (m / Np) % B;
    const f32x4* xr = reinterpret_cast<const f32x4*>(h + ((size_t)b * L + idx[m]) * D);
    const int nch = D >> 2;
    f32x4 v[NC];
    float s = 0.f;
#pragma unroll
    for (int i = 0; i < NC; ++i) {
        const int c = lane + 64 * i;
        if (c < nch) { v[i] = xr[c]; s += (v[i][0] + v[i][1]) + (v[i][2] + v[i][3]); }
    }
    const float mu = wave_sum(s) / D;
    float q = 0.f;
#pragma unroll
    for (int i = 0; i < NC; ++i) {
        const int c = lane + 64 * i;
        if (c < nch) {
#pragma unroll
            for (int e = 0; e < 4; ++e) { const float d = v[i][e] - mu; q += d * d; }
        }
    }
    const float rs = rsqrtf(wave_sum(q) / D + eps);
    f32x4* o = reinterpret_cast<f32x4*>(out + (size_t)m * D);
#pragma unroll
    for (int i = 0; i < NC; ++i) {
        const int c = lane + 64 * i;
        if (c < nch) o[c] = (v[i] - mu) * rs;
    }
}

__global__ void pred_assemble_kernel(const float* __restrict__ xe, const float* __restrict__ mask_token, const float* __restrict__ pos,
                                     const int* __restrict__ idx_pred, float* __restrict__ X, int nseq, int B, int Nc, int Np, int D) {
    const size_t i = (size_t)blockIdx.x * blockDim.x + threadIdx.x;
    const int nch = D >> 2, T = Nc + Np;
    if (i >= (size_t)nseq * T * nch) return;
    const int c = (int)(i % nch);
    const int t = (int)((i / nch) % T), sq = (int)(i / ((size_t)nch * T));
    f32x4 v;
    if (t < Nc) {
        v = reinterpret_cast<const f32x4*>(xe + ((size_t)(sq % B) * Nc + t) * D)[c];
    } else {
        v = reinterpret_cast<const f32x4*>(mask_token)[c] + reinterpret_cast<const f32x4*>(pos + (size_t)idx_pred[(size_t)sq * Np + (t - Nc)] * D)[c];
    }
    reinterpret_cast<f32x4*>(X + ((size_t)sq * T + t) * D)[c] = v;
}

__global__ void pred_ctx_grad_kernel(const float* __restrict__ dX, bf16_t* __restrict__ dxe, int nsets, int B, int Nc, int Np, int D) {
    const size_t i = (size_t)blockIdx.x * blockDim.x + threadIdx.x;
    const int nch = D >> 2, T = Nc + Np;
    if (i >= (size_t)B * Nc * nch) return;
    const int c = (int)(i % nch);
    const int t = (int)((i / nch) % Nc), b = (int)(i / ((size_t)nch * Nc));
    f32x4 a = {0, 0, 0, 0};
    for (int k = 0; k < nsets; ++k) a += reinterpret_cast<const f32x4*>(dX + (((size_t)k * B + b) * T + t) * D)[c];
    reinterpret_cast<uint2*>(dxe + ((size_t)b * Nc + t) * D)[c] = uint2{pack2bf(a[0], a[1]), pack2bf(a[2], a[3])};
}

__global__ __launch_bounds__(256) void smooth_l1_fwd_kernel(const float* __restrict__ z, const float* __restrict__ h, size_t n,
                                                            float* __restrict__ partial) {
    __shared__ float red[4];
    float s = 0.f;
    for (size_t i = ((size_t)blockIdx.x * 256 + threadIdx.x) * 4; i < n; i += (size_t)gridDim.x * 1024) {
        if (i + 4 <= n) {
            const f32x4 d = *reinterpret_cast<const f32x4*>(z + i) - *reinterpret_cast<const f32x4*>(h + i);
#pragma unroll
// ... 859 lines not shown
}

int launch_gather_rows_bf16(const float* in, RowMap rm, bf16_t* out, int M, int D, hipStream_t s) {
    hipLaunchKernelGGL(gather_rows_bf16_kernel, dim3(blocks_for((size_t)M * (D / 4))), dim3(256), 0, s, in, rm, out, M, D);
    BVC_CHECK_HIP(hipGetLastError());
    return BVC_OK;
}

int launch_mask_index(const uint8_t* mask, int B, int L, int nvis, int nmask, int* vis_idx, int* msk_idx, int* status, hipStream_t s) {
    hipLaunchKernelGGL(mask_index_kernel, dim3(B), dim3(64), 0, s, mask, L, nvis, nmask, vis_idx, msk_idx, status);
    BVC_CHECK_HIP(hipGetLastError());
    return BVC_OK;
}

int launch_dual_mask_index(const uint8_t* mask, const uint8_t* decode, int B, int L, int nvis, int ndec, int* vis_idx, int* dec_idx,
                           int* status, hipStream_t s) {
    hipLaunchKernelGGL(dual_mask_index_kernel, dim3(B), dim3(64), 0, s, mask, decode, L, nvis, ndec, vis_idx, dec_idx, status);
    BVC_CHECK_HIP(hipGetLastError());
    return BVC_OK;
}

int launch_gather_patches(PixelSrc clip, const int* vis_idx, bf16_t* A, int B, int nvis, PatchGeom pg, hipStream_t s) {
    BVC_REQUIRE(pg.ps % 8 == 0 && pg.W % 4 == 0, "gather_patches: patch size must be a multiple of 8");
    const size_t items = (size_t)B * nvis * (pg.C * pg.ts * pg.ps * pg.ps / 8);
    hipLaunchKernelGGL(gather_patches_kernel, dim3(blocks_for(items)), dim3(256), 0, s, clip, vis_idx, A, B, nvis, pg);
    BVC_CHECK_HIP(hipGetLastError());
    return BVC_OK;
}

int launch_gather_patches_mix(PixelSrc clip, const int* idx, bf16_t* A, int B, int n, PatchGeom pg, const ClipMix* mix, hipStream_t s,
                              int* status) {
    BVC_REQUIRE(clip.ptr && idx && A && mix, "gather_patches_mix: null argument");
    BVC_REQUIRE(B >= 1 && n >= 1, "gather_patches_mix: B=%d clips of n=%d tokens", B, n);
    BVC_REQUIRE(pg.ps % 8 == 0 && pg.W % 4 == 0, "gather_patches_mix: patch size must be a multiple of 8");
    const size_t items = (size_t)B * n * (pg.C * pg.ts * pg.ps * pg.ps / 8);
    if ((pg.C * pg.ts * pg.ps * pg.ps / 8) % 64 == 0)
        hipLaunchKernelGGL(gather_patches_mix_kernel<true>, dim3(blocks_for(items)), dim3(256), 0, s, clip, idx, A, B, n, pg, mix, status);
    else
        hipLaunchKernelGGL(gather_patches_mix_kernel<false>, dim3(blocks_for(items)), dim3(256), 0, s, clip, idx, A, B, n, pg, mix, status);
    BVC_CHECK_HIP(hipGetLastError());
    return BVC_OK;
}

int launch_poison_on_status(float* x, size_t count, const int* status, hipStream_t s) {
    hipLaunchKernelGGL(poison_on_status_kernel, dim3(blocks_for(count)), dim3(256), 0, s, x, count, status);
    BVC_CHECK_HIP(hipGetLastError());
    return BVC_OK;
}

int launch_labels(PixelSrc clip, const int* dec_idx, float* labels, int B, int ndec, PatchGeom pg, int norm_pix, hipStream_t s) {
    BVC_REQUIRE(pg.ps % 4 == 0, "labels: patch size must be a multiple of 4");
    const int E = pg.ts * pg.ps * pg.ps;
    const size_t lds = (size_t)(pg.C * E + 2 * pg.C) * 4;
    const int nchunk = pg.C * (E >> 2), ntok = B * ndec;
    if (pg.C == 3 && (E == 512 || E == 256)) {
        const int nblk = (ntok + 3) / 4;
        if (E == 512) hipLaunchKernelGGL(labels_wave3_kernel<2>, dim3(nblk), dim3(256), (size_t)4 * 3 * E * 4, s, clip, dec_idx, labels, ntok, ndec, pg, norm_pix);
        else hipLaunchKernelGGL(labels_wave3_kernel<1>, dim3(nblk), dim3(256), (size_t)4 * 3 * E * 4, s, clip, dec_idx, labels, ntok, ndec, pg, norm_pix);
        BVC_CHECK_HIP(hipGetLastError());
        return BVC_OK;
    }
    if (nchunk <= 512 && lds <= 16384) {
        const int per_wave = (pg.C * E + 2 * pg.C + 3) & ~3;
        const int nblk = (ntok + 3) / 4;
        if (nchunk <= 384)
            hipLaunchKernelGGL(labels_wave_kernel<6>, dim3(nblk), dim3(256), (size_t)per_wave * 16, s, clip, dec_idx, labels, ntok, ndec, pg, norm_pix);
        else
            hipLaunchKernelGGL(labels_wave_kernel<8>, dim3(nblk), dim3(256), (size_t)per_wave * 16, s, clip, dec_idx, labels, ntok, ndec, pg, norm_pix);
        BVC_CHECK_HIP(hipGetLastError());
        return BVC_OK;
    }
    hipLaunchKernelGGL(labels_kernel, dim3(B * ndec), dim3(256), lds, s, clip, dec_idx, labels, ndec, pg, norm_pix);
    BVC_CHECK_HIP(hipGetLastError());
    return BVC_OK;
}

int launch_fill_masked(float* xfull, const float* mask_token, const float* pos, const int* dec_idx, int B, int Ld, int nvis,
                       int ndec, int D, hipStream_t s) {
    hipLaunchKernelGGL(fill_masked_kernel, dim3(blocks_for((size_t)B * ndec * (D / 4))), dim3(256), 0, s, xfull, mask_token, pos, dec_idx, B, Ld, nvis, ndec, D);
    BVC_CHECK_HIP(hipGetLastError());
    return BVC_OK;
}

int launch_target_select(const float* h, const int* idx, float* out, int nsets, int B, int Np, int L, int D, float eps, hipStream_t s) {
    BVC_REQUIRE(D % 4 == 0 && D <= kWideChunks * 256, "target_select: D=%d unsupported", D);
    const int rows = nsets * B * Np;
    if (D > kMaxChunks * 256)
        hipLaunchKernelGGL(target_select_kernel<kWideChunks>, dim3((rows + 3) / 4), dim3(256), 0, s, h, idx, out, rows, B, Np, L, D, eps);
    else
        hipLaunchKernelGGL(target_select_kernel<kMaxChunks>, dim3((rows + 3) / 4), dim3(256), 0, s, h, idx, out, rows, B, Np, L, D, eps);
    BVC_CHECK_HIP(hipGetLastError());
    return BVC_OK;
}

int launch_pred_assemble(const float* xe, const float* mask_token, const float* pos, const int* idx_pred, float* X, int nsets, int B,
                         int Nc, int Np, int D, hipStream_t s) {
    const size_t items = (size_t)nsets * B * (Nc + Np) * (D / 4);
    hipLaunchKernelGGL(pred_assemble_kernel, dim3(blocks_for(items)), dim3(256), 0, s, xe, mask_token, pos, idx_pred, X, nsets * B, B, Nc, Np, D);
    BVC_CHECK_HIP(hipGetLastError());
    return BVC_OK;
}

int launch_pred_ctx_grad(const float* dX, bf16_t* dxe, int nsets, int B, int Nc, int Np, int D, hipStream_t s) {
    hipLaunchKernelGGL(pred_ctx_grad_kernel, dim3(blocks_for((size_t)B * Nc * (D / 4))), dim3(256), 0, s, dX, dxe, nsets, B, Nc, Np, D);
    BVC_CHECK_HIP(hipGetLastError());
    return BVC_OK;
}

int smooth_l1_blocks(size_t n) { return (int)std::min<size_t>(1024, (n + 1023) / 1024); }

int launch_smooth_l1_fwd(const float* z, const float* h, size_t n, float* partial, float* loss, hipStream_t s) {
    BVC_REQUIRE(n > 0, "smooth_l1: empty input");
    const int nb = smooth_l1_blocks(n);
    hipLaunchKernelGGL(smooth_l1_fwd_kernel, dim3(nb), dim3(256), 0, s, z, h, n, partial);
    BVC_CHECK_HIP(hipGetLastError());
    return launch_loss_finalize(partial, nb, (double)n, nullptr, loss, s);
}

int launch_smooth_l1_bwd(const float* z, const float* h, const float* gout, size_t n, float* dz, hipStream_t s) {
    hipLaunchKernelGGL(smooth_l1_bwd_kernel, dim3(blocks_for((n + 3) / 4)), dim3(256), 0, s, z, h, gout, n, dz);
    BVC_CHECK_HIP(hipGetLastError());
    return BVC_OK;
}

int launch_ema(float* k, const float* q, size_t n, float m, hipStream_t s) {
    if (n == 0) return BVC_OK;
    hipLaunchKernelGGL(ema_kernel, dim3(blocks_for((n + 3) / 4)), dim3(256), 0, s, k, q, n, m);
    BVC_CHECK_HIP(hipGetLastError());
    return BVC_OK;
}

int launch_iota_mod(int* idx, int n, int L, hipStream_t s) {
    hipLaunchKernelGGL(iota_mod_kernel, dim3(blocks_for((size_t)n)), dim3(256), 0, s, idx, n, L);
    BVC_CHECK_HIP(hipGetLastError());
    return BVC_OK;
}

int launch_row_normalize(const float* f, bf16_t* fn, float* inv, int n, int p, float eps, hipStream_t s) {
    BVC_REQUIRE(p % 4 == 0, "row_normalize: width must be a multiple of 4");
    hipLaunchKernelGGL(row_normalize_kernel, dim3((n + 3) / 4), dim3(256), 0, s, f, fn, inv, n, p, eps);
    BVC_CHECK_HIP(hipGetLastError());
    return BVC_OK;
}

int launch_row_normalize_bwd(const float* f, const float* inv, const float* dfn, float* df, int n, int p, hipStream_t s) {
    BVC_REQUIRE(p % 4 == 0, "row_normalize_bwd: width must be a multiple of 4");
    hipLaunchKernelGGL(row_normalize_bwd_kernel, dim3((n + 3) / 4), dim3(256), 0, s, f, inv, dfn, df, n, p);
    BVC_CHECK_HIP(hipGetLastError());
    return BVC_OK;
}

int launch_nce_finalize(const float* partial, int ntiles, float inv_t, double npos, float* loss, float* stats, hipStream_t s) {
    hipLaunchKernelGGL(nce_finalize_kernel, dim3(1), dim3(256), 0, s, partial, ntiles, inv_t, npos, loss, stats);
    BVC_CHECK_HIP(hipGetLastError());
    return BVC_OK;
}

int launch_sgd_step(float* p, float* g, float* buf, size_t n, float lr, float momentum, float dampening, float wd, int nesterov,
                    int first, int maximize, const float* grad_scale, const float* found_inf, int write_grad, bf16_t* shadow,
                    hipStream_t s) {
    BVC_REQUIRE(momentum == 0.f || buf != nullptr, "sgd_step: momentum needs a buffer");
    BVC_REQUIRE(shadow == nullptr || (uintptr_t)shadow % 8 == 0, "sgd_step: the bf16 shadow must be 8-byte aligned");
    BVC_REQUIRE(((uintptr_t)p % 16 == 0) && ((uintptr_t)g % 16 == 0) && (buf == nullptr || (uintptr_t)buf % 16 == 0),
                "sgd_step: buffers must be 16-byte aligned");
    if (n == 0) return BVC_OK;
    hipLaunchKernelGGL(sgd_step_kernel, dim3(blocks_for((n + 3) / 4)), dim3(256), 0, s, p, g, buf, n, lr, momentum, dampening, wd,
// ... 225 lines not shown
```

### baby-vision-curriculum_amd/csrc/stack.h

```cpp
#pragma once
#include <string>
#include <vector>

#include "attention.h"
#include "gemm.h"
#include "rowops.h"

namespace bvc {

#define TRY(expr)                      \
    do {                               \
        int _rc = (expr);              \
        if (_rc != BVC_OK) return _rc; \
    } while (0)

struct LayerOff {
    int64_t ln1w, ln1b, wqkv, bqkv, wo, bo, ln2w, ln2b, w1, b1, w2, b2, end;
};

struct ParamEntry {
    std::string name;
    int64_t offset, numel;
    int ndim;
    int64_t shape[5];
};

struct ParamTable {
    std::vector<ParamEntry> entries;
    int64_t total = 0;
    int64_t add(const std::string& name, std::initializer_list<int64_t> shp);
};

struct LayerAct {
    float* x_in;
    float* h;
    bf16_t* ln1o;
    bf16_t* qkv;
    bf16_t* ctx;
    float* lse;
    bf16_t* ln2o;
    bf16_t* pre;
    bf16_t* act;
    float *mean1, *rstd1, *mean2, *rstd2;
};

struct Stack {
    int D, I, H, nlayers;
    float eps;
    std::vector<LayerAct> act;
    float* x_out;
    int hd, hdp, Da;
    bool ln1_ready = false;
    bf16_t *wqkv_pad = nullptr, *wo_pad = nullptr;
    float *bqkv_pad = nullptr;
    float *gwqkv_pad = nullptr, *gbqkv_pad = nullptr, *gwo_pad = nullptr;
};

struct Arena {
    std::vector<void*> ptrs;
    template <typename T>
    int alloc(T** p, size_t count) {
        void* q = nullptr;
        BVC_CHECK_HIP(hipMalloc(&q, count * sizeof(T) + 256));
        ptrs.push_back(q);
        *p = reinterpret_cast<T*>(q);
        return BVC_OK;
    }
    void release() {
        for (void* p : ptrs) (void)hipFree(p);
        ptrs.clear();
    }
};

struct Work {
    const float* params = nullptr;
    const bf16_t* wbf = nullptr;
    bf16_t *dyb[3] = {}, *dhb[2] = {}, *dqkv[2] = {}, *dh[2] = {};
    bf16_t *dln = nullptr, *dctx = nullptr;
    float *delta = nullptr, *ln_part = nullptr;
    hipStream_t side = nullptr;
    hipEvent_t ev_fork = nullptr, ev_join[2] = {nullptr, nullptr};
    bool overlap = false;
    int seq = 0;
    bool join_pending[2] = {false, false};
    int64_t pend_lo[2], pend_hi[2];
    const DropState* drop = nullptr;
    int drop_layer = -1;
};

inline int attn_width(int hd) {
    if ((hd == 80 || hd == 88) && !options().head_pad) return hd;
    return hd <= 32 ? 32 : hd <= 64 ? 64 : hd <= 96 ? 96 : 128;
}

struct LayerTail { int nvis, ndec; };
bool layer_tail_ok(const Work& w, const Stack& s, int B, int nvis, int ndec);

LayerOff add_layer_params(ParamTable& t, const std::string& prefix, int64_t d, int64_t inter, bool hf_names);
int alloc_stack(Arena& a, Stack& s, int D, int I, int H, int nlayers, float eps, size_t M, size_t BHN);
int alloc_work(Arena& a, Work& w, size_t MD, size_t MI, size_t delta_elems, size_t lnpart_elems);
void free_work(Work& w);

GemmProblem gemm(const bf16_t* A, size_t a_elems, int lda, const bf16_t* B, size_t b_elems, int ldb, int M, int N, int K,
                 int epi, void* C, int ldc);
int plan_dw(GemmProblem* g, int n);
int join_side(Work& w, int parity, hipStream_t st, bvc_bucket_fn on_bucket, void* user);
void begin_backward(Work& w);
int layer_forward(Work& w, Stack& s, int li, const LayerOff& o, const float* x_in, float* x_out, int B, int N, hipStream_t st,
                  const LayerOff* next = nullptr, const LayerTail* tail = nullptr);
bool fuse_row_ln(const Stack& s, int M);
int set_drop(DropState& d, const bvc_branch_drop* drop, int samples, const char* who, hipStream_t st);
int alloc_drop(Arena& a, DropState& d, int nlayers, int max_samples);
int take_drop(DropState& d, int samples, int rows, const char* who);
inline const Gate* top_gate(const DropState& d, Gate& store) {
    if (!d.active) return nullptr;
    store = d.gate(d.nlayers - 1, 1);
    return &store;
}
int layer_backward(Work& w, Stack& s, int li, const LayerOff& o, const float* x_in, float* dres, float* G, int B, int N,
                   hipStream_t st, bvc_bucket_fn on_bucket, void* user, const LayerTail* tail = nullptr);

}
```

### baby-vision-curriculum_amd/csrc/stack.hip

```cpp
#include <math.h>
#include <stdlib.h>
#include <string.h>

#include <algorithm>

#include "stack.h"

namespace bvc {

int64_t ParamTable::add(const std::string& name, std::initializer_list<int64_t> shp) {
    ParamEntry e;
    e.name = name;
    e.offset = total;
    e.numel = 1;
    e.ndim = (int)shp.size();
    int i = 0;
    for (auto s : shp) { e.shape[i++] = s; e.numel *= s; }
    for (; i < 5; ++i) e.shape[i] = 1;
    entries.push_back(e);
    total += e.numel;
    return e.offset;
}

LayerOff add_layer_params(ParamTable& t, const std::string& p, int64_t d, int64_t inter, bool hf_names) {
// ... 51 lines not shown
        TRY(a.alloc(&s.gwo_pad, (size_t)D * Da));
    }
    s.act.resize(nlayers);
    for (auto& l : s.act) {
        TRY(a.alloc(&l.x_in, M * D));
        TRY(a.alloc(&l.h, M * D));
        TRY(a.alloc(&l.ln1o, M * D));
        TRY(a.alloc(&l.qkv, M * 3 * Da));
        TRY(a.alloc(&l.ctx, M * Da));
        TRY(a.alloc(&l.lse, BHN));
        TRY(a.alloc(&l.ln2o, M * D));
        TRY(a.alloc(&l.pre, M * I));
        TRY(a.alloc(&l.act, M * I));
        TRY(a.alloc(&l.mean1, M));
        TRY(a.alloc(&l.rstd1, M));
        TRY(a.alloc(&l.mean2, M));
        TRY(a.alloc(&l.rstd2, M));
    }
    TRY(a.alloc(&s.x_out, M * D));
    return BVC_OK;
}

int alloc_work(Arena& a, Work& w, size_t MD, size_t MI, size_t delta_elems, size_t lnpart_elems) {
    for (int i = 0; i < 3; ++i) TRY(a.alloc(&w.dyb[i], MD));
    for (int i = 0; i < 2; ++i) {
        TRY(a.alloc(&w.dhb[i], MD));
        TRY(a.alloc(&w.dqkv[i], 3 * MD));
        TRY(a.alloc(&w.dh[i], MI));
    }
    TRY(a.alloc(&w.dln, MD));
    TRY(a.alloc(&w.dctx, MD));
    TRY(a.alloc(&w.delta, delta_elems));
    TRY(a.alloc(&w.ln_part, std::max(lnpart_elems, kRowLnPartFloats)));
    w.overlap = false;
    BVC_CHECK_HIP(hipStreamCreateWithFlags(&w.side, hipStreamNonBlocking));
    BVC_CHECK_HIP(hipEventCreateWithFlags(&w.ev_fork, hipEventDisableTiming));
    BVC_CHECK_HIP(hipEventCreateWithFlags(&w.ev_join[0], hipEventDisableTiming));
    BVC_CHECK_HIP(hipEventCreateWithFlags(&w.ev_join[1], hipEventDisableTiming));
    return BVC_OK;
}

void free_work(Work& w) {
    if (w.side) { (void)hipStreamSynchronize(w.side); (void)hipStreamDestroy(w.side); w.side = nullptr; }
    if (w.ev_fork) { (void)hipEventDestroy(w.ev_fork); w.ev_fork = nullptr; }
    for (int i = 0; i < 2; ++i) if (w.ev_join[i]) { (void)hipEventDestroy(w.ev_join[i]); w.ev_join[i] = nullptr; }
}

void begin_backward(Work& w) {
    w.overlap = options().dw_overlap != 0;
    w.seq = 0;
    w.join_pending[0] = w.join_pending[1] = false;
}

GemmProblem gemm(const bf16_t* A, size_t a_elems, int lda, const bf16_t* B, size_t b_elems, int ldb, int M, int N, int K,
                 int epi, void* C, int ldc) {
    GemmProblem p;
    memset(&p, 0, sizeof(p));
    p.A = A; p.B = B; p.M = M; p.N = N; p.K = K; p.lda = lda; p.ldb = ldb;
    p.a_bytes = (uint32_t)(a_elems * 2); p.b_bytes = (uint32_t)(b_elems * 2);
    p.alpha = 1.f; p.epi = epi; p.split_k = 1; p.C = C; p.ldc = ldc;
    return p;
}

int plan_dw(GemmProblem* g, int n) {
    static const int bm[3] = {128, 128, 64}, bn[3] = {128, 64, 64};
    int ksteps = 1 << 30;
    for (int i = 0; i < n; ++i) ksteps = std::min(ksteps, (g[i].K + 63) / 64);
    const int g8 = options().gemm8;
    if (g8 >= 0) {
        bool ok = true, by384 = true;
        double flops = 0.0, outs = 0.0;
        int units256 = 0, units384 = 0;
        for (int i = 0; i < n; ++i) {
            ok = ok && g[i].epi == EPI_F32 && g[i].a_bytes < 0x80000000u && g[i].b_bytes < 0x80000000u;
            by384 = by384 && g[i].N % 384 == 0 && g[i].M % 128 == 0;
            flops += 2.0 * g[i].M * g[i].N * g[i].K;
            outs += (double)g[i].M * g[i].N;
            units256 += ((g[i].M + 255) / 256) * ((g[i].N + 255) / 256);
            units384 += ((g[i].M + 127) / 128) * ((g[i].N + 383) / 384);
        }
        const bool long_enough = g8 > 0 ? ksteps >= 2 : (ksteps >= 16 && flops >= 80e9);
        if (ok && by384 && long_enough && units256 * 65536.0 >= 1.2 * outs) {
            const int smax = std::max(1, std::min(24, ksteps / (g8 > 0 ? 2 : 16)));
            int best = 1;
            double best_cost = 1e300;
            for (int sp = 1; sp <= smax; ++sp) {
                const int rounds = (units384 * sp + 255) / 256;
                const double cost = (double)rounds * ((ksteps + sp - 1) / sp) + 4.0 * rounds;
                if (cost < best_cost * 0.999) { best_cost = cost; best = sp; }
            }
            if (units384 * best >= (g8 > 0 ? 1 : 160)) {
                for (int i = 0; i < n; ++i) g[i].split_k = best;
                return 12;
            }
        }
        if (ok && g8 > 0 && ksteps >= 2) {
            const int split = std::max(1, std::min((232 + units256 / 2) / units256, ksteps / 2));
            for (int i = 0; i < n; ++i) g[i].split_k = split;
            return 10;
        }
        if (ok && ksteps >= 16 && flops >= 140e9) {
            for (int t = 0; t < 2; ++t) {
                const int bnw = t == 0 ? 256 : 128;
                int units = 0;
                for (int i = 0; i < n; ++i) units += ((g[i].M + 255) / 256) * ((g[i].N + bnw - 1) / bnw);
                int split = std::max(1, (232 + units / 2) / units);
                split = std::min(split, std::max(1, ksteps / 16));
                if (units >= 16 && units * split >= (t == 0 ? 200 : 160) && units * split <= 272) {
                    for (int i = 0; i < n; ++i) g[i].split_k = split;
                    return t == 0 ? 10 : 11;
                }
            }
            if (units256 >= 128 && units256 <= 240 && ksteps >= 64) {
                for (int i = 0; i < n; ++i) g[i].split_k = 1;
                return 13;
            }
        }
    }
    const int cap = std::max(1, std::min(12, ksteps / 8));
    int tile = 2, split = 1;
    for (int t = 0; t < 3; ++t) {
        int tiles = 0;
        for (int i = 0; i < n; ++i) tiles += ((g[i].M + bm[t] - 1) / bm[t]) * ((g[i].N + bn[t] - 1) / bn[t]);
        const int s = std::max(1, std::min(cap, (480 + tiles / 2) / tiles));
        tile = t; split = s;
        if (tiles * s >= 400) break;
    }
    for (int i = 0; i < n; ++i) g[i].split_k = split;
    return tile;
}

bool fuse_row_ln(const Stack& s, int M) {
    const int mode = options().row_ln;
    if (mode < 0 || options().gemm8 < 0) return false;
    if (!gemm_row_ln_ok(M, s.D, s.D) || s.I % 64 != 0 || (3 * s.Da) % 64 != 0) return false;
    if ((size_t)M * std::max<size_t>(3 * (size_t)s.Da, (size_t)s.I) * 2 >= 0x80000000ull) return false;
    if (mode > 0 || options().gemm8 > 0) return true;
    return M >= 128 * 128;
}

bool layer_tail_ok(const Work& w, const Stack& s, int B, int nvis, int ndec) {
    if (!options().dec_tail || nvis < 1 || ndec < 128 || ndec % 128 != 0) return false;
    if (w.drop != nullptr && w.drop->active) return false;
    if (s.hdp != s.hd || !attn_window_ok(s.hd)) return false;
    if (nvis + ndec <= 160) return false;
    return fuse_row_ln(s, B * (nvis + ndec)) && gemm_row_ln_ok(B * ndec, s.D, s.D);
}

int alloc_drop(Arena& a, DropState& d, int nlayers, int max_samples) {
    d.nlayers = nlayers;
    d.max_samples = max_samples;
    return a.alloc(&d.path_scale, (size_t)nlayers * 2 * max_samples);
}

int set_drop(DropState& d, const bvc_branch_drop* drop, int samples, const char* who, hipStream_t st) {
    d.armed = false;
    if (!drop || (drop->hidden_p == 0.f && drop->path_scale == nullptr)) return BVC_OK;
    BVC_REQUIRE(drop->hidden_p >= 0.f && drop->hidden_p < 1.f, "%s: hidden_p %g outside [0, 1)", who, (double)drop->hidden_p);
    BVC_REQUIRE(samples >= 1 && samples <= d.max_samples, "%s: %d samples outside [1, %d]", who, samples, d.max_samples);
    BVC_REQUIRE(drop->rows_per_sample >= 1, "%s: rows_per_sample must be >= 1", who);
    d.hidden_p = drop->hidden_p;
    d.seed = drop->seed;
    d.offset = drop->offset;
    d.samples = samples;
    d.rows = drop->rows_per_sample;
    d.has_path = drop->path_scale != nullptr;
    if (d.has_path)
        BVC_CHECK_HIP(hipMemcpyAsync(d.path_scale, drop->path_scale, (size_t)d.nlayers * 2 * samples * sizeof(float), hipMemcpyDeviceToDevice, st));
    d.armed = true;
    return BVC_OK;
}

int take_drop(DropState& d, int samples, int rows, const char* who) {
    d.active = d.armed;
    d.armed = false;
    if (!d.active) return BVC_OK;
    if (d.samples != samples || d.rows != rows) {
        d.active = false;
        set_error("%s: the gate was set for %d samples of %d rows, the call has %d of %d", who, d.samples, d.rows, samples, rows);
        return BVC_ERR_INVALID;
    }
    return BVC_OK;
}

int layer_forward(Work& w, Stack& s, int li, const LayerOff& o, const float* x_in, float* x_out, int B, int N, hipStream_t st,
                  const LayerOff* next, const LayerTail* tail) {
    LayerAct& a = s.act[li];
    const int D = s.D, I = s.I, M = B * N;
    const int Mq = tail ? B * tail->ndec : M;
    if (tail) BVC_REQUIRE(next == nullptr && tail->nvis + tail->ndec == N && layer_tail_ok(w, s, B, tail->nvis, tail->ndec), "layer_forward: tail mode is not available for this layer");
    const float* P = w.params;
    const bf16_t* W = w.wbf;
    const float eps = s.eps;
    const bool gated = w.drop != nullptr && w.drop->active;
    const int gl = w.drop_layer >= 0 ? w.drop_layer : li;
    const bool fuse = !gated && fuse_row_ln(s, M);
    if (li == 0) s.ln1_ready = false;
    if (!(fuse && s.ln1_ready)) TRY(launch_ln_fwd(x_in, identity_rows(), P + o.ln1w, P + o.ln1b, a.ln1o, a.mean1, a.rstd1, M, D, eps, st));
    s.ln1_ready = false;
    const int Da = s.Da;
    const bool pad = s.hdp != s.hd;
    const bf16_t *Wqkv = W + o.wqkv, *Wo = W + o.wo;
    const float* bqkv = P + o.bqkv;
    const float sm_scale = pad ? 1.0f / sqrtf((float)s.hd) : 0.f;
    if (pad) {
        TRY(launch_pad_heads(W + o.wqkv, P + o.bqkv, W + o.wo, s.wqkv_pad, s.bqkv_pad, s.wo_pad, D, s.H, s.hd, s.hdp, st));
        Wqkv = s.wqkv_pad; Wo = s.wo_pad; bqkv = s.bqkv_pad;
    }
    {
        GemmProblem p = gemm(a.ln1o, (size_t)M * D, D, Wqkv, (size_t)3 * Da * D, D, M, 3 * Da, D, EPI_BF16, a.qkv, 3 * Da);
        p.bias = bqkv;
        TRY(launch_gemm(&p, 1, GEMM_NT, -1, st));
    }
    if (tail) TRY(launch_attn_fwd_win(a.qkv, a.ctx, a.lse, B, N, s.H, s.hdp, tail->nvis, tail->ndec, st, sm_scale));
    else TRY(launch_attn_fwd(a.qkv, a.ctx, a.lse, B, N, s.H, s.hdp, st, sm_scale));
    {
        GemmProblem p = gemm(a.ctx, (size_t)Mq * Da, Da, Wo, (size_t)D * Da, Da, Mq, D, Da, fuse ? EPI_RESID_LN : EPI_RESID, a.h, D);
        p.bias = P + o.bo; p.resid = x_in;
        if (fuse) { p.C2 = a.ln2o; p.ln_gamma = P + o.ln2w; p.ln_beta = P + o.ln2b; p.ln_mean = a.mean2; p.ln_rstd = a.rstd2; p.ln_eps = eps; }
        if (tail) { p.seg_rows = tail->ndec; p.seg_stride = N; p.seg_off = tail->nvis; }
        if (gated) TRY(launch_gemm_gate(p, w.drop->gate(gl, 0), -1, st));
        else TRY(launch_gemm(&p, 1, GEMM_NT, -1, st));
    }
    if (!fuse) TRY(launch_ln_fwd(a.h, identity_rows(), P + o.ln2w, P + o.ln2b, a.ln2o, a.mean2, a.rstd2, M, D, eps, st));
    {
        GemmProblem p = gemm(a.ln2o, (size_t)Mq * D, D, W + o.w1, (size_t)I * D, D, Mq, I, D, EPI_GELU, a.pre, I);
        p.bias = P + o.b1; p.C2 = a.act;
        TRY(launch_gemm(&p, 1, GEMM_NT, -1, st));
    }
    {
        const bool fuse_next = fuse && next != nullptr && li + 1 < (int)s.act.size();
        GemmProblem p = gemm(a.act, (size_t)Mq * I, I, W + o.w2, (size_t)D * I, I, Mq, D, I, fuse_next ? EPI_RESID_LN : EPI_RESID, x_out, D);
        p.bias = P + o.b2; p.resid = a.h;
        if (fuse_next) {
            LayerAct& an = s.act[li + 1];
            p.C2 = an.ln1o; p.ln_gamma = P + next->ln1w; p.ln_beta = P + next->ln1b; p.ln_mean = an.mean1; p.ln_rstd = an.rstd1; p.ln_eps = eps;
        }
        if (gated) TRY(launch_gemm_gate(p, w.drop->gate(gl, 1), -1, st));
        else TRY(launch_gemm(&p, 1, GEMM_NT, -1, st));
        s.ln1_ready = fuse_next;
    }
    return BVC_OK;
}

int join_side(Work& c_, int parity, hipStream_t st, bvc_bucket_fn on_bucket, void* user) {
    if (!c_.join_pending[parity]) return BVC_OK;
    BVC_CHECK_HIP(hipStreamWaitEvent(st, c_.ev_join[parity], 0));
    c_.join_pending[parity] = false;
    if (on_bucket) on_bucket(c_.pend_lo[parity], c_.pend_hi[parity] - c_.pend_lo[parity], user);
    return BVC_OK;
}

int layer_backward(Work& c_, Stack& s, int li, const LayerOff& o, const float* x_in, float* dres, float* G, int B, int N,
                   hipStream_t st, bvc_bucket_fn on_bucket, void* user, const LayerTail* tail) {
    LayerAct& a = s.act[li];
    const int D = s.D, I = s.I, M = B * N;
    const int Mq = tail ? B * tail->ndec : M;
    const float* P = c_.params;
    const bf16_t* W = c_.wbf;
    const int q = c_.seq, par = q & 1;
    bf16_t* dyb = c_.dyb[q % 3];
    bf16_t* dyb_next = c_.dyb[(q + 1) % 3];
    bf16_t *dh = c_.dh[par], *dhb = c_.dhb[par], *dqkv = c_.dqkv[par];
    TRY(join_side(c_, par, st, on_bucket, user));
    {
        GemmProblem p = gemm(dyb, (size_t)Mq * D, D, W + o.w2, (size_t)D * I, I, Mq, I, D, EPI_DGELU, dh, I);
        p.aux = a.pre; p.ldaux = I;
        TRY(launch_gemm(&p, 1, GEMM_NN, -1, st));
    }
    const bool gated = c_.drop != nullptr && c_.drop->active;
    Gate g_attn, g_below;
    if (gated) { g_attn = c_.drop->gate(li, 0); if (li > 0) g_below = c_.drop->gate(li - 1, 1); }
    const bool fuse = !gated && fuse_row_ln(s, M);
    if (tail) BVC_REQUIRE(fuse && tail->nvis + tail->ndec == N, "layer_backward: tail mode needs the row-LayerNorm epilogues");
    if (fuse) {
        GemmProblem p = gemm(dh, (size_t)Mq * I, I, W + o.w1, (size_t)I * D, D, Mq, D, I, EPI_DLN, dres, D);
        p.C2 = dhb; p.ln_x = a.h; p.ln_mean = a.mean2; p.ln_rstd = a.rstd2; p.ln_gamma = P + o.ln2w;
        p.ln_part = c_.ln_part; p.ln_dgamma = G + o.ln2w; p.ln_dbeta = G + o.ln2b;
        if (tail) { p.seg_rows = tail->ndec; p.seg_stride = N; p.seg_off = tail->nvis; }
        TRY(launch_gemm(&p, 1, GEMM_NN, -1, st));
    } else {
        GemmProblem p = gemm(dh, (size_t)M * I, I, W + o.w1, (size_t)I * D, D, M, D, I, EPI_BF16, c_.dln, D);
        TRY(launch_gemm(&p, 1, GEMM_NN, -1, st));
        TRY(launch_ln_bwd(c_.dln, a.h, identity_rows(), a.mean2, a.rstd2, P + o.ln2w, dres, 1, dhb, G + o.ln2w, G + o.ln2b, c_.ln_part, M, D, st,
                          gated ? &g_attn : nullptr));
    }
    const int Da = s.Da;
    const bool pad = s.hdp != s.hd;
    const bf16_t *Wqkv = W + o.wqkv, *Wo = W + o.wo;
    const float sm_scale = pad ? 1.0f / sqrtf((float)s.hd) : 0.f;
    if (pad) {
        TRY(launch_pad_heads(W + o.wqkv, P + o.bqkv, W + o.wo, s.wqkv_pad, s.bqkv_pad, s.wo_pad, D, s.H, s.hd, s.hdp, st));
        Wqkv = s.wqkv_pad; Wo = s.wo_pad;
    }
    {
        GemmProblem p = gemm(dhb, (size_t)Mq * D, D, Wo, (size_t)D * Da, Da, Mq, Da, D, EPI_BF16, c_.dctx, Da);
        TRY(launch_gemm(&p, 1, GEMM_NN, -1, st));
    }
    if (tail) TRY(launch_attn_bwd_win(a.qkv, a.ctx, c_.dctx, a.lse, c_.delta, dqkv, B, N, s.H, s.hdp, tail->nvis, tail->ndec, st, sm_scale));
    else TRY(launch_attn_bwd(a.qkv, a.ctx, c_.dctx, a.lse, c_.delta, dqkv, B, N, s.H, s.hdp, st, sm_scale));
    if (fuse) {
        GemmProblem p = gemm(dqkv, (size_t)M * 3 * Da, 3 * Da, Wqkv, (size_t)3 * Da * D, D, M, D, 3 * Da, EPI_DLN, dres, D);
        p.C2 = dyb_next; p.ln_x = x_in; p.ln_mean = a.mean1; p.ln_rstd = a.rstd1; p.ln_gamma = P + o.ln1w;
        p.ln_part = c_.ln_part; p.ln_dgamma = G + o.ln1w; p.ln_dbeta = G + o.ln1b;
        TRY(launch_gemm(&p, 1, GEMM_NN, -1, st));
    } else {
        GemmProblem p = gemm(dqkv, (size_t)M * 3 * Da, 3 * Da, Wqkv, (size_t)3 * Da * D, D, M, D, 3 * Da, EPI_BF16, c_.dln, D);
        TRY(launch_gemm(&p, 1, GEMM_NN, -1, st));
    }
    hipStream_t ws = st;
    if (c_.overlap) {
        BVC_CHECK_HIP(hipEventRecord(c_.ev_fork, st));
        BVC_CHECK_HIP(hipStreamWaitEvent(c_.side, c_.ev_fork, 0));
        ws = c_.side;
    }
    {
        GemmProblem g[4];
        g[0] = gemm(dyb, (size_t)Mq * D, D, a.act, (size_t)Mq * I, I, D, I, Mq, EPI_F32, G + o.w2, I);
        g[1] = gemm(dh, (size_t)Mq * I, I, a.ln2o, (size_t)Mq * D, D, I, D, Mq, EPI_F32, G + o.w1, D);
        g[2] = gemm(dhb, (size_t)Mq * D, D, a.ctx, (size_t)Mq * Da, Da, D, Da, Mq, EPI_F32, pad ? s.gwo_pad : G + o.wo, Da);
        g[3] = gemm(dqkv, (size_t)M * 3 * Da, 3 * Da, a.ln1o, (size_t)M * D, D, 3 * Da, D, M, EPI_F32, pad ? s.gwqkv_pad : G + o.wqkv, D);
        g[0].rowsum = G + o.b2;
        g[1].rowsum = G + o.b1;
        g[2].rowsum = G + o.bo;
        g[3].rowsum = pad ? s.gbqkv_pad : G + o.bqkv;
        const int tile = plan_dw(g, 4);
        if (pad) {
            BVC_CHECK_HIP(hipMemsetAsync(s.gwo_pad, 0, (size_t)D * Da * 4, ws));
            BVC_CHECK_HIP(hipMemsetAsync(s.gwqkv_pad, 0, (size_t)3 * Da * D * 4, ws));
            BVC_CHECK_HIP(hipMemsetAsync(s.gbqkv_pad, 0, (size_t)3 * Da * 4, ws));
        }
        TRY(launch_gemm(g, 4, GEMM_TN, tile, ws));
        if (pad)
            TRY(launch_unpad_head_grads(s.gwqkv_pad, s.gbqkv_pad, s.gwo_pad, G + o.wqkv, G + o.bqkv, G + o.wo, D, s.H, s.hd, s.hdp, ws));
    }
    if (!fuse) TRY(launch_ln_bwd(c_.dln, x_in, identity_rows(), a.mean1, a.rstd1, P + o.ln1w, dres, 1, dyb_next, G + o.ln1w, G + o.ln1b, c_.ln_part, M, D, st,
                                 gated && li > 0 ? &g_below : nullptr));
    if (c_.overlap) {
        BVC_CHECK_HIP(hipEventRecord(c_.ev_join[par], c_.side));
        c_.join_pending[par] = true;
        c_.pend_lo[par] = o.ln1w;
        c_.pend_hi[par] = o.end;
    } else if (on_bucket) {
        on_bucket(o.ln1w, o.end - o.ln1w, user);
    }
    c_.seq = q + 1;
    return BVC_OK;
}

}
```

### baby-vision-curriculum_amd/csrc/videomae.hip

```cpp
#include <math.h>
#include <stdio.h>
#include <string.h>

#include <algorithm>
#include <string>
#include <vector>

#include "context.h"

using namespace bvc;

namespace {

struct Layout : ParamTable {
    int64_t pe_w = 0, pe_b = 0, e2d_w = 0, mask_token = 0, norm_w = 0, norm_b = 0, head_w = 0, head_b = 0;
    std::vector<LayerOff> enc, dec;
};

int check_config(const bvc_videomae_config& c) {
    BVC_REQUIRE(c.image_size > 0 && c.patch_size > 0 && c.image_size % c.patch_size == 0, "config: image_size %% patch_size != 0");
    BVC_REQUIRE(c.num_frames > 0 && c.tubelet_size > 0 && c.num_frames % c.tubelet_size == 0, "config: num_frames %% tubelet_size != 0");
    BVC_REQUIRE(c.patch_size % 8 == 0, "config: patch_size must be a multiple of 8");
    BVC_REQUIRE(c.num_attention_heads > 0 && c.hidden_size % c.num_attention_heads == 0, "config: encoder head_dim undefined (hidden_size %d %% num_attention_heads %d != 0)",
                c.hidden_size, c.num_attention_heads);
    BVC_REQUIRE(c.decoder_num_attention_heads > 0 && c.decoder_hidden_size % c.decoder_num_attention_heads == 0,
                "config: decoder head_dim undefined (decoder_hidden_size %d %% decoder_num_attention_heads %d != 0)", c.decoder_hidden_size, c.decoder_num_attention_heads);
    const int hd = c.hidden_size / c.num_attention_heads, hdd = c.decoder_hidden_size / c.decoder_num_attention_heads;
    BVC_REQUIRE(hd % 8 == 0 && hd <= 128, "config: encoder head_dim %d unsupported (multiples of 8 up to 128)", hd);
    BVC_REQUIRE(hdd % 8 == 0 && hdd <= 128, "config: decoder head_dim %d unsupported (multiples of 8 up to 128)", hdd);
    BVC_REQUIRE(c.hidden_size % 64 == 0 && c.decoder_hidden_size % 64 == 0, "config: hidden sizes must be multiples of 64");
    BVC_REQUIRE(c.hidden_size <= 1536 && c.decoder_hidden_size <= 1536, "config: hidden sizes above 1536 unsupported (hidden %d, decoder %d)",
                c.hidden_size, c.decoder_hidden_size);
    BVC_REQUIRE(c.intermediate_size % 64 == 0 && c.decoder_intermediate_size % 64 == 0, "config: intermediate sizes must be multiples of 64");
    BVC_REQUIRE((c.num_channels * c.tubelet_size * c.patch_size * c.patch_size) % 64 == 0, "config: patch dim must be a multiple of 64");
    BVC_REQUIRE(c.num_hidden_layers >= 1 && c.decoder_num_hidden_layers >= 1, "config: need at least one layer each");
    return BVC_OK;
}

Layout make_layout(const bvc_videomae_config& c) {
    Layout L;
    const int64_t D = c.hidden_size, Dd = c.decoder_hidden_size;
    const int64_t P = (int64_t)c.num_channels * c.tubelet_size * c.patch_size * c.patch_size;
    const std::string pe = "videomae.embeddings.patch_embeddings.projection.";
    L.pe_w = L.add(pe + "weight", {D, c.num_channels, c.tubelet_size, c.patch_size, c.patch_size});
    L.pe_b = L.add(pe + "bias", {D});
    for (int i = 0; i < c.num_hidden_layers; ++i)
        L.enc.push_back(add_layer_params(L, "videomae.encoder.layer." + std::to_string(i) + ".", D, c.intermediate_size, true));
    L.e2d_w = L.add("encoder_to_decoder.weight", {Dd, D});
    L.mask_token = L.add("mask_token", {1, 1, Dd});
    for (int i = 0; i < c.decoder_num_hidden_layers; ++i)
        L.dec.push_back(add_layer_params(L, "decoder.decoder_layers." + std::to_string(i) + ".", Dd, c.decoder_intermediate_size, true));
    L.norm_w = L.add("decoder.norm.weight", {Dd});
    L.norm_b = L.add("decoder.norm.bias", {Dd});
    L.head_w = L.add("decoder.head.weight", {P, Dd});
    L.head_b = L.add("decoder.head.bias", {P});
    return L;
}

}

struct bvc_ctx {
    bvc_videomae_config cfg;
    Layout lay;
    int max_batch, nmask, nvis, L, P;
    int ndec, Ld;
    Arena arena;
    Work w;
    float *pos_enc, *pos_dec;
    int batch = 0;
    bool have_forward = false;
    Shadow shadow;
    const float* params = nullptr;
    int *vis_idx, *dec_idx, *status;
    PatchFront front;
    Stack enc, dec;
    bf16_t* xe_bf;
    float *meanf, *rstdf;
    bf16_t* lnf;
    float* labels;
    bf16_t* diff;
    float* partial;
    int npartial = 0;
    float *dres_enc, *dres_dec;
    bf16_t* de2d;
    bool tail_on = false;
};

namespace {

int upload_sinusoid(float* dst, int n, int d) {
    std::vector<float> out((size_t)n * d);
    for (int p = 0; p < n; ++p)
        for (int j = 0; j < d; ++j) {
            const double ang = (double)p / pow(10000.0, 2.0 * (j / 2) / (double)d);
            out[(size_t)p * d + j] = (float)((j & 1) ? cos(ang) : sin(ang));
        }
    if (hipMemcpy(dst, out.data(), out.size() * 4, hipMemcpyHostToDevice) != hipSuccess) { set_error("create: pos upload failed"); return BVC_ERR_HIP; }
    return BVC_OK;
}

float stack_sm_scale(const Stack& s) { return s.hdp != s.hd ? 1.0f / sqrtf((float)s.hd) : 0.f; }

}

extern "C" {

int bvc_videomae_param_count(const bvc_videomae_config* cfg) {
    if (!cfg || check_config(*cfg) != BVC_OK) return BVC_ERR_INVALID;
    return (int)make_layout(*cfg).entries.size();
}

int64_t bvc_videomae_param_numel(const bvc_videomae_config* cfg) {
    if (!cfg || check_config(*cfg) != BVC_OK) return BVC_ERR_INVALID;
    return make_layout(*cfg).total;
}

int bvc_videomae_param_info(const bvc_videomae_config* cfg, int index, char* name, int name_cap, int64_t* offset,
                            int64_t* numel, int* ndim, int64_t shape[5]) {
    BVC_REQUIRE(cfg && name && offset && numel && ndim && shape, "param_info: null argument");
    TRY(check_config(*cfg));
    return param_info(make_layout(*cfg), index, name, name_cap, offset, numel, ndim, shape);
}

void bvc_videomae_destroy(bvc_ctx* c) {
    if (!c) return;
    free_work(c->w);
    c->arena.release();
    delete c;
}

int bvc_videomae_create(const bvc_videomae_config* cfg, int max_batch, int num_masked, bvc_ctx** out) {
    return bvc_videomae_create_dual(cfg, max_batch, num_masked, num_masked, out);
}

int bvc_videomae_create_dual(const bvc_videomae_config* cfg, int max_batch, int num_masked, int num_decoded, bvc_ctx** out) {
    BVC_REQUIRE(cfg && out, "create: null argument");
    TRY(check_config(*cfg));
    BVC_REQUIRE(max_batch >= 1, "create: max_batch must be >= 1");
    const PatchGeom pg = patch_geom(*cfg);
    const int L = seq_len(pg), nvis = L - num_masked, Ld = nvis + num_decoded;
    BVC_REQUIRE(num_masked >= 1 && nvis >= 1, "create: num_masked=%d must leave at least one visible and one masked token of %d", num_masked, L);
    BVC_REQUIRE(num_decoded >= 1 && num_decoded <= num_masked, "create: num_decoded=%d must lie in [1, num_masked=%d]", num_decoded, num_masked);
    const size_t B = max_batch, Mv = B * nvis, Md = B * Ld, Mm = B * num_decoded;
    const int D = cfg->hidden_size, Dd = cfg->decoder_hidden_size, I = cfg->intermediate_size, Id = cfg->decoder_intermediate_size;
    const int H = cfg->num_attention_heads, Hd = cfg->decoder_num_attention_heads;
    {
        const size_t we = std::max<size_t>(3 * (size_t)H * attn_width(D / H), (size_t)I), wd = std::max<size_t>(3 * (size_t)Hd * attn_width(Dd / Hd), (size_t)Id);
        const bool dec = Ld * wd >= nvis * we;
        TRY(refuse_operand_extent("create", max_batch, dec ? Ld : nvis, dec ? wd : we, dec ? "decoder" : "encoder"));
    }
    bvc_ctx* c = new bvc_ctx();
    Making guard{[&] { bvc_videomae_destroy(c); }};
    c->cfg = *cfg;
    c->lay = make_layout(*cfg);
    c->max_batch = max_batch;
    c->L = L; c->P = patch_dim(pg);
    c->nmask = num_masked; c->nvis = nvis; c->ndec = num_decoded; c->Ld = Ld;
    TRY(c->arena.alloc(&c->pos_enc, (size_t)L * D));
    TRY(c->arena.alloc(&c->pos_dec, (size_t)L * Dd));
    TRY(c->shadow.alloc(c->arena, c->lay.total));
    TRY(c->arena.alloc(&c->vis_idx, Mv));
    TRY(c->arena.alloc(&c->dec_idx, Mm));
    BVC_CHECK_HIP(hipMemset(c->vis_idx, 0, (size_t)Mv * sizeof(int)));
    BVC_CHECK_HIP(hipMemset(c->dec_idx, 0, (size_t)Mm * sizeof(int)));
    TRY(c->arena.alloc(&c->status, 4));
    TRY(c->front.alloc(c->arena, pg, Mv, false));
    TRY(alloc_stack(c->arena, c->enc, D, I, H, cfg->num_hidden_layers, cfg->layer_norm_eps, Mv, B * H * nvis));
    TRY(alloc_stack(c->arena, c->dec, Dd, Id, Hd, cfg->decoder_num_hidden_layers, cfg->layer_norm_eps, Md, B * Hd * Ld));
    TRY(c->arena.alloc(&c->xe_bf, Mv * D));
    TRY(c->arena.alloc(&c->meanf, Mm));
    TRY(c->arena.alloc(&c->rstdf, Mm));
    TRY(c->arena.alloc(&c->lnf, Mm * Dd));
    TRY(c->arena.alloc(&c->labels, Mm * c->P));
    TRY(c->arena.alloc(&c->diff, Mm * c->P));
    TRY(c->arena.alloc(&c->partial, (Mm / 64 + 2) * (c->P / 64 + 2)));
    TRY(c->arena.alloc(&c->dres_enc, Mv * D));
    TRY(c->arena.alloc(&c->dres_dec, Md * Dd));
    TRY(c->arena.alloc(&c->de2d, Mv * Dd));
    TRY(alloc_work(c->arena, c->w, std::max(Mv * D, Md * Dd), std::max(Mv * I, Md * Id), std::max(B * H * nvis, B * Hd * Ld),
                   std::max(ln_bwd_workspace_floats_upto((int)Mv, D), ln_bwd_workspace_floats_upto((int)Md, Dd))));
    TRY(upload_sinusoid(c->pos_enc, L, D));
    TRY(upload_sinusoid(c->pos_dec, L, Dd));
    guard.done = true;
    *out = c;
    return BVC_OK;
}

int bvc_videomae_forward(bvc_ctx* c, const float* pixels, const uint8_t* mask, int batch, const float* params,
                         float* loss, float* logits, void* stream) {
    return bvc_videomae_forward_px(c, pixels, nullptr, mask, batch, params, loss, logits, stream);
}

int bvc_videomae_forward_px(bvc_ctx* c, const void* pixels_any, const bvc_pixel_format* fmt, const uint8_t* mask, int batch,
                            const float* params, float* loss, float* logits, void* stream) {
    return bvc_videomae_forward_dual(c, pixels_any, fmt, mask, nullptr, batch, params, loss, logits, stream);
}

int bvc_videomae_forward_dual(bvc_ctx* c, const void* pixels_any, const bvc_pixel_format* fmt, const uint8_t* mask, const uint8_t* decode_mask,
                              int batch, const float* params, float* loss, float* logits, void* stream) {
    BVC_REQUIRE(c && pixels_any && mask && params && loss, "forward: null argument");
    BVC_REQUIRE(decode_mask || c->ndec == c->nmask, "forward: the context decodes %d of %d masked tokens and needs a decode mask", c->ndec, c->nmask);
    PixelSrc pixels;
    TRY(pixel_src("forward", pixels_any, fmt, c->cfg.num_channels, &pixels));
    BVC_REQUIRE(batch >= 1 && batch <= c->max_batch, "forward: batch %d outside [1, %d]", batch, c->max_batch);
    hipStream_t st = (hipStream_t)stream;
    const bvc_videomae_config& cf = c->cfg;
    const Layout& L = c->lay;
    const int B = batch, nvis = c->nvis, ndec = c->ndec, Lq = c->L, Ld = c->Ld;
    const int Mv = B * nvis, Mm = B * ndec;
    const int D = cf.hidden_size, Dd = cf.decoder_hidden_size, P = c->P;
    c->have_forward = false;
    c->batch = B;
    c->params = params;
    c->w.params = params;
    c->w.wbf = c->shadow.wbf;
    const bf16_t* W = c->shadow.wbf;

    TRY(c->shadow.refresh(params, st));
    BVC_CHECK_HIP(hipMemsetAsync(c->status, 0, 16, st));
    if (decode_mask) TRY(launch_dual_mask_index(mask, decode_mask, B, Lq, nvis, ndec, c->vis_idx, c->dec_idx, c->status, st));
    else TRY(launch_mask_index(mask, B, Lq, nvis, ndec, c->vis_idx, c->dec_idx, c->status, st));
    TRY(c->front.embed(pixels, c->vis_idx, B, nvis, W + L.pe_w, params + L.pe_b, c->pos_enc, c->enc.act[0].x_in, D, st, "forward"));
    TRY(stack_forward(c->w, c->enc, L.enc, B, nvis, st, true));
    TRY(launch_gather_rows_bf16(c->enc.x_out, identity_rows(), c->xe_bf, Mv, D, st));
    {
        GemmProblem p = gemm(c->xe_bf, (size_t)Mv * D, D, W + L.e2d_w, (size_t)Dd * D, D, Mv, Dd, D, EPI_E2D, c->dec.act[0].x_in, Dd);
        p.rowtok = c->vis_idx; p.pos = c->pos_dec; p.rin = nvis; p.rout = Ld;
        TRY(launch_gemm(&p, 1, GEMM_NT, -1, st));
    }
    TRY(launch_fill_masked(c->dec.act[0].x_in, params + L.mask_token, c->pos_dec, c->dec_idx, B, Ld, nvis, ndec, Dd, st));
    const LayerTail lt{nvis, ndec};
    c->tail_on = layer_tail_ok(c->w, c->dec, B, nvis, ndec);
    TRY(stack_forward(c->w, c->dec, L.dec, B, Ld, st, true, c->tail_on ? &lt : nullptr));
    const RowMap tail = c->tail_on ? identity_rows() : RowMap{ndec, Ld, nvis};
    TRY(launch_ln_fwd(c->dec.x_out, tail, params + L.norm_w, params + L.norm_b, c->lnf, c->meanf, c->rstdf, Mm, Dd, cf.decoder_norm_eps, st));
    TRY(launch_labels(pixels, c->dec_idx, c->labels, B, ndec, c->front.pg, cf.norm_pix_loss, st));
    {
        GemmProblem p = gemm(c->lnf, (size_t)Mm * Dd, Dd, W + L.head_w, (size_t)P * Dd, Dd, Mm, P, Dd, EPI_LOSS, c->diff, P);
        p.bias = params + L.head_b; p.labels = c->labels; p.partial = c->partial; p.C2 = logits;
        c->npartial = gemm_num_tiles(p, -1);
        TRY(launch_gemm(&p, 1, GEMM_NT, -1, st));
    }
    TRY(launch_loss_finalize(c->partial, c->npartial, (double)Mm * (double)P, c->status, loss, st));
    c->have_forward = true;
    return BVC_OK;
}

int bvc_videomae_backward(bvc_ctx* c, const float* grad_loss, float* G, bvc_bucket_fn on_bucket, void* user, void* stream) {
    BVC_REQUIRE(c && grad_loss && G, "backward: null argument");
    if (!c->have_forward) { set_error("backward: no forward state (call bvc_videomae_forward first; one backward per forward)"); return BVC_ERR_STATE; }
    c->have_forward = false;
    hipStream_t st = (hipStream_t)stream;
    const bvc_videomae_config& cf = c->cfg;
    const Layout& L = c->lay;
    const int B = c->batch, nvis = c->nvis, ndec = c->ndec, Ld = c->Ld;
    const int Mv = B * nvis, Md = B * Ld, Mm = B * ndec;
    const int D = cf.hidden_size, Dd = cf.decoder_hidden_size, P = c->P;
    const bf16_t* W = c->shadow.wbf;
    const float* params = c->params;
    begin_backward(c->w);

    BVC_CHECK_HIP(hipMemsetAsync(G, 0, (size_t)L.total * 4, st));
    const float cmse = (float)(2.0 / ((double)Mm * (double)P));
    {
        GemmProblem p = gemm(c->diff, (size_t)Mm * P, P, c->lnf, (size_t)Mm * Dd, Dd, P, Dd, Mm, EPI_F32, G + L.head_w, Dd);
        p.alpha = cmse; p.alpha_dev = grad_loss;
        p.rowsum = G + L.head_b;
        const int tile = plan_dw(&p, 1);
        TRY(launch_gemm(&p, 1, GEMM_TN, tile, st));
    }
    {
        GemmProblem p = gemm(c->diff, (size_t)Mm * P, P, W + L.head_w, (size_t)P * Dd, Dd, Mm, Dd, P, EPI_BF16, c->w.dln, Dd);
        p.alpha = cmse; p.alpha_dev = grad_loss;
        TRY(launch_gemm(&p, 1, GEMM_NN, -1, st));
    }
    const RowMap tail{ndec, Ld, nvis};
    const LayerTail lt{nvis, ndec};
    if (c->tail_on) {
        BVC_CHECK_HIP(hipMemset2DAsync(c->dres_dec, (size_t)Ld * Dd * 4, 0, (size_t)nvis * Dd * 4, (size_t)B, st));
        TRY(launch_ln_bwd(c->w.dln, c->dec.x_out, tail, c->meanf, c->rstdf, params + L.norm_w, c->dres_dec, 0, c->w.dyb[0],
                          G + L.norm_w, G + L.norm_b, c->w.ln_part, Mm, Dd, st, nullptr, true));
    } else {
        BVC_CHECK_HIP(hipMemsetAsync(c->dres_dec, 0, (size_t)Md * Dd * 4, st));
        BVC_CHECK_HIP(hipMemsetAsync(c->w.dyb[0], 0, (size_t)Md * Dd * 2, st));
        TRY(launch_ln_bwd(c->w.dln, c->dec.x_out, tail, c->meanf, c->rstdf, params + L.norm_w, c->dres_dec, 0, c->w.dyb[0],
                          G + L.norm_w, G + L.norm_b, c->w.ln_part, Mm, Dd, st));
    }
    if (on_bucket) on_bucket(L.norm_w, L.total - L.norm_w, user);
    TRY(stack_backward(c->w, c->dec, L.dec, c->dres_dec, G, B, Ld, st, on_bucket, user, c->tail_on ? &lt : nullptr));
    TRY(launch_colsum_f32(c->dres_dec, tail, Mm, Dd, G + L.mask_token, st));
    const RowMap headrows{nvis, Ld, 0};
    TRY(launch_gather_rows_bf16(c->dres_dec, headrows, c->de2d, Mv, Dd, st));
    {
        GemmProblem p = gemm(c->de2d, (size_t)Mv * Dd, Dd, c->xe_bf, (size_t)Mv * D, D, Dd, D, Mv, EPI_F32, G + L.e2d_w, D);
        const int tile = plan_dw(&p, 1);
        TRY(launch_gemm(&p, 1, GEMM_TN, tile, st));
    }
    {
        GemmProblem p = gemm(c->de2d, (size_t)Mv * Dd, Dd, W + L.e2d_w, (size_t)Dd * D, D, Mv, D, Dd, EPI_F32_BF16, c->dres_enc, D);
        p.C2 = c->w.dyb[c->w.seq % 3];
        TRY(launch_gemm(&p, 1, GEMM_NN, -1, st));
    }
    if (on_bucket) on_bucket(L.e2d_w, L.dec.front().ln1w - L.e2d_w, user);
    TRY(stack_backward(c->w, c->enc, L.enc, c->dres_enc, G, B, nvis, st, on_bucket, user));
    TRY(c->front.embed_backward(c->w, Mv, D, G + L.pe_w, G + L.pe_b, st));
    TRY(join_both(c->w, st, on_bucket, user));
    if (on_bucket) on_bucket(0, L.enc.front().ln1w, user);
    return BVC_OK;
}

static int tail_tap(bvc_ctx* c, float* dst, hipStream_t st) {
    const Layout& L = c->lay;
    Stack& s = c->dec;
    LayerAct& a = s.act.back();
    const LayerOff& o = L.dec.back();
    const int B = c->batch, nvis = c->nvis, ndec = c->ndec, Ld = c->Ld, D = s.D, I = s.I, Da = s.Da;
    const size_t Mq = (size_t)B * ndec, Mv = (size_t)B * nvis;
    const float* P = c->params;
    const bf16_t* W = c->shadow.wbf;
    bf16_t *ctx_v = a.ctx + Mq * Da, *ln2o_v = a.ln2o + Mq * D, *pre_v = a.pre + Mq * I, *act_v = a.act + Mq * I;
    float *lse_v = a.lse + (size_t)B * s.H * ndec, *h_v = a.h + Mq * D, *mean_v = a.mean2 + Mq, *rstd_v = a.rstd2 + Mq, *out_v = s.x_out + Mq * D;
    const size_t full = (size_t)Ld * D * 4, vis = (size_t)nvis * D * 4, dec = (size_t)ndec * D * 4;
    TRY(launch_attn_fwd_win(a.qkv, ctx_v, lse_v, B, Ld, s.H, s.hdp, 0, nvis, st));
    BVC_CHECK_HIP(hipMemcpy2DAsync(h_v, vis, a.x_in, full, vis, (size_t)B, hipMemcpyDeviceToDevice, st));
    {
        GemmProblem p = gemm(ctx_v, Mv * Da, Da, W + o.wo, (size_t)D * Da, Da, (int)Mv, D, Da, EPI_RESID, h_v, D);
        p.bias = P + o.bo; p.resid = h_v;
        TRY(launch_gemm(&p, 1, GEMM_NT, -1, st));
    }
    TRY(launch_ln_fwd(h_v, identity_rows(), P + o.ln2w, P + o.ln2b, ln2o_v, mean_v, rstd_v, (int)Mv, D, s.eps, st));
    {
        GemmProblem p = gemm(ln2o_v, Mv * D, D, W + o.w1, (size_t)I * D, D, (int)Mv, I, D, EPI_GELU, pre_v, I);
        p.bias = P + o.b1; p.C2 = act_v;
        TRY(launch_gemm(&p, 1, GEMM_NT, -1, st));
    }
    {
        GemmProblem p = gemm(act_v, Mv * I, I, W + o.w2, (size_t)D * I, I, (int)Mv, D, I, EPI_RESID, out_v, D);
        p.bias = P + o.b2; p.resid = h_v;
        TRY(launch_gemm(&p, 1, GEMM_NT, -1, st));
    }
    BVC_CHECK_HIP(hipMemcpy2DAsync(dst, full, out_v, vis, vis, (size_t)B, hipMemcpyDeviceToDevice, st));
    BVC_CHECK_HIP(hipMemcpy2DAsync(dst + (size_t)nvis * D, full, s.x_out, dec, dec, (size_t)B, hipMemcpyDeviceToDevice, st));
    return BVC_OK;
}

int bvc_videomae_tap(bvc_ctx* c, const char* name, float* dst, int64_t capacity, int64_t* numel, void* stream) {
    BVC_REQUIRE(c && name && dst && numel, "tap: null argument");
    BVC_REQUIRE(c->batch > 0, "tap: no forward has run");
    const int B = c->batch;
    const size_t Mv = (size_t)B * c->nvis, Md = (size_t)B * c->Ld, Mm = (size_t)B * c->ndec;
    const int D = c->cfg.hidden_size, Dd = c->cfg.decoder_hidden_size;
    const float* src = nullptr;
    size_t n = 0;
    int idx = -1;
    if (!strcmp(name, "embed")) { src = c->enc.act[0].x_in; n = Mv * D; }
    else if (!strcmp(name, "x_full")) { src = c->dec.act[0].x_in; n = Md * Dd; }
    else if (!strcmp(name, "labels")) { src = c->labels; n = Mm * c->P; }
    else if (sscanf(name, "enc%d", &idx) == 1 && idx >= 0 && idx < c->enc.nlayers) {
        src = idx + 1 < c->enc.nlayers ? c->enc.act[idx + 1].x_in : c->enc.x_out; n = Mv * D;
    } else if (sscanf(name, "dec%d", &idx) == 1 && idx >= 0 && idx < c->dec.nlayers) {
        src = idx + 1 < c->dec.nlayers ? c->dec.act[idx + 1].x_in : c->dec.x_out; n = Md * Dd;
    }
    BVC_REQUIRE(src, "tap: unknown activation '%s'", name);
    *numel = (int64_t)n;
    BVC_REQUIRE((int64_t)n <= capacity, "tap: destination holds %lld elements, '%s' has %lld", (long long)capacity, name, (long long)n);
    if (src == c->dec.x_out && c->tail_on) return tail_tap(c, dst, (hipStream_t)stream);
    BVC_CHECK_HIP(hipMemcpyAsync(dst, src, n * 4, hipMemcpyDeviceToDevice, (hipStream_t)stream));
    return BVC_OK;
}

struct bvc_encoder_ctx {
    bvc_videomae_config cfg;
// ... 287 lines not shown
```

### baby-vision-curriculum_amd/probe.py

```python
import ctypes

import torch

from . import _lib, _ops

PEAK_BF16_TFLOPS = 2500.0
PEAK_HBM_GBS = 8000.0


def _time(fn, iters=5, warm=2):
    for _ in range(warm):
        fn()
    e0, e1 = torch.cuda.Event(enable_timing=True), torch.cuda.Event(enable_timing=True)
    e0.record()
    for _ in range(iters):
        fn()
    e1.record()
    torch.cuda.synchronize()
    return e0.elapsed_time(e1) * 1e3 / iters


def _rb(dev, *shape):
    return torch.randn(*shape, device=dev, dtype=torch.bfloat16)


def _gemm_rows(dev, B, add):
    E = _ops.EPI
    Mv, Md, Mm = B * 160, B * 1568, B * 1408
    D, I, Dd, Id, P = 768, 3072, 384, 1536, 1536

    def one(label, layout, M, N, K, epi, count, tile=-1):
        A = _rb(dev, M, K)
        Bm = _rb(dev, N, K) if layout == _ops.NT else _rb(dev, K, N)
        Bm.mul_(0.02)
        kw = {}
        out_f32 = epi in ("F32", "RESID", "POS", "E2D", "F32_BF16", "RESID_LN", "DLN")
        nbytes = 2.0 * (M * K + N * K)
        Mo = M
        if epi == "E2D":
            Mo = (M // 160) * 1568
        C = torch.empty(Mo, N, device=dev, dtype=torch.float32 if out_f32 else torch.bfloat16)
        nbytes += (4.0 if out_f32 else 2.0) * M * N
        if epi not in ("DGELU", "E2D", "DLN"):
            kw["bias"] = torch.zeros(N, device=dev)
        if epi == "GELU":
            kw["C2"] = torch.empty_like(C)
            nbytes += 2.0 * M * N
        if epi == "F32_BF16":
            kw["C2"] = torch.empty(M, N, device=dev, dtype=torch.bfloat16)
            nbytes += 2.0 * M * N
        if epi in ("RESID", "RESID_LN"):
            kw["resid"] = torch.randn(M, N, device=dev)
            nbytes += 4.0 * M * N
        if epi == "RESID_LN":
            kw.update(C2=torch.empty(M, N, device=dev, dtype=torch.bfloat16), ln_gamma=torch.ones(N, device=dev), ln_beta=torch.zeros(N, device=dev),
                      ln_mean=torch.empty(M, device=dev), ln_rstd=torch.empty(M, device=dev), ln_eps=1e-12)
            nbytes += 2.0 * M * N
        if epi == "DLN":
            kw.update(C2=torch.empty(M, N, device=dev, dtype=torch.bfloat16), ln_gamma=torch.ones(N, device=dev), ln_x=torch.randn(M, N, device=dev),
                      ln_mean=torch.zeros(M, device=dev), ln_rstd=torch.ones(M, device=dev), ln_part=torch.empty(512 * 2 * N, device=dev),
                      ln_dgamma=torch.zeros(N, device=dev), ln_dbeta=torch.zeros(N, device=dev))
            nbytes += (4.0 + 4.0 + 2.0) * M * N
        if epi == "DGELU":
            kw["aux"] = _rb(dev, M, N)
            nbytes += 2.0 * M * N
        if epi in ("POS", "E2D"):
            kw["rowtok"] = (torch.arange(M, device=dev, dtype=torch.int32) % 160) * 9
            kw["pos"] = torch.randn(1568, N, device=dev)
            nbytes += 4.0 * M * N
            if epi == "E2D":
                kw["rin"], kw["rout"] = 160, 1568
        if epi == "LOSS":
            kw["labels"] = torch.randn(M, N, device=dev)
            kw["partial"] = torch.empty(1 << 16, device=dev)
            nbytes += 4.0 * M * N
        d = _ops.gemm_desc(A, Bm, M, N, K, E[epi], C, **kw)
        name = _ops.gemm_kernel_name(d, layout, tile)
        us = _time(lambda: _ops.gemm(d, layout, tile))
        add(name, label, count, us, 2.0 * M * N * K, nbytes)

    def dw_single(label, Mo, No, K, count):
        A, Bm = _rb(dev, K, Mo), _rb(dev, K, No)
        C = torch.zeros(Mo, No, device=dev)
        rs = torch.zeros(Mo, device=dev)
        d = _ops.gemm_desc(A, Bm, Mo, No, K, E["F32"], C, rowsum=rs)
        tile, _ = _ops.plan_dw([d])
        name = _ops.gemm_kernel_name(d, _ops.TN, tile)
        us = _time(lambda: _ops.gemm(d, _ops.TN, tile))
        add(name, label, count, us, 2.0 * Mo * No * K, 2.0 * K * (Mo + No) + 4.0 * Mo * No)

    def dw_group(label, M, Dm, Im, count):
        dy, act, dh, ln2, dqkv = _rb(dev, M, Dm), _rb(dev, M, Im), _rb(dev, M, Im), _rb(dev, M, Dm), _rb(dev, M, 3 * Dm)
        shapes = [(Dm, Im), (Im, Dm), (Dm, Dm), (3 * Dm, Dm)]
        outs = [torch.zeros(s, device=dev) for s in shapes]
        bs = [torch.zeros(s[0], device=dev) for s in shapes]
        ds = [_ops.gemm_desc(dy, act, Dm, Im, M, E["F32"], outs[0], rowsum=bs[0]),
              _ops.gemm_desc(dh, ln2, Im, Dm, M, E["F32"], outs[1], rowsum=bs[1]),
              _ops.gemm_desc(dy, ln2, Dm, Dm, M, E["F32"], outs[2], rowsum=bs[2]),
              _ops.gemm_desc(dqkv, ln2, 3 * Dm, Dm, M, E["F32"], outs[3], rowsum=bs[3])]
        tile, split = _ops.plan_dw(ds)
        name = _ops.gemm_kernel_name(ds, _ops.TN, tile)
        us = _time(lambda: _ops.gemm(ds, _ops.TN, tile), iters=3)
        fl = 2.0 * M * (2 * Dm * Im + 4 * Dm * Dm)
        nb = 2.0 * M * (2 * Dm + 2 * Im + 2 * Dm + Dm + 3 * Dm) + 4.0 * (2 * Dm * Im + 4 * Dm * Dm)
        add(name, f"{label} (tile {tile}, split {split})", count, us, fl, nb)

    NT, NN = _ops.NT, _ops.NN
    fused = bool(_lib.lib().bvc_op_row_ln_selected(Md, Dd, Id, 6))
    one("patch embed", NT, Mv, D, 1536, "POS", 1)
    one("enc qkv", NT, Mv, 3 * D, D, "BF16", 12)
    one("enc proj", NT, Mv, D, D, "RESID", 12)
    one("enc fc1+GELU", NT, Mv, I, D, "GELU", 12)
    one("enc fc2", NT, Mv, D, I, "RESID", 12)
    one("enc->dec", NT, Mv, Dd, D, "E2D", 1)
    one("dec qkv", NT, Md, 3 * Dd, Dd, "BF16", 4)
    if fused:
        one("dec proj + LayerNorm", NT, Md, Dd, Dd, "RESID_LN", 4)
    else:
        one("dec proj", NT, Md, Dd, Dd, "RESID", 4)
    one("dec fc1+GELU", NT, Md, Id, Dd, "GELU", 4)
    if fused:
        one("dec fc2 + next LayerNorm", NT, Md, Dd, Id, "RESID_LN", 3)
        one("dec fc2", NT, Md, Dd, Id, "RESID", 1)
    else:
        one("dec fc2", NT, Md, Dd, Id, "RESID", 4)
    one("head+MSE", NT, Mm, P, Dd, "LOSS", 1)
    one("head dX", NN, Mm, Dd, P, "BF16", 1)
    one("dec dX fc2", NN, Md, Id, Dd, "DGELU", 4)
    one("dec dX fc1 + LayerNorm bwd" if fused else "dec dX fc1", NN, Md, Dd, Id, "DLN" if fused else "BF16", 4)
    one("dec dX proj", NN, Md, Dd, Dd, "BF16", 4)
    one("dec dX qkv + LayerNorm bwd" if fused else "dec dX qkv", NN, Md, Dd, 3 * Dd, "DLN" if fused else "BF16", 4)
    one("enc->dec dX", NN, Mv, D, Dd, "F32_BF16", 1)
    one("enc dX fc2", NN, Mv, I, D, "DGELU", 12)
    one("enc dX fc1", NN, Mv, D, I, "BF16", 12)
    one("enc dX proj", NN, Mv, D, D, "BF16", 12)
    one("enc dX qkv", NN, Mv, D, 3 * D, "BF16", 12)
    dw_single("head dW", P, Dd, Mm, 1)
    dw_single("enc->dec dW", Dd, D, Mv, 1)
    dw_single("patch dW", D, 1536, Mv, 1)
    dw_group("dec layer dW group", Md, Dd, Id, 4)
    dw_group("enc layer dW group", Mv, D, I, 12)


def _attention_rows(dev, B, add):
    lib = _lib.lib()
    st = _lib.current_stream_ptr
    for label, N, H, count in (("enc", 160, 12, 12), ("dec", 1568, 6, 4)):
        Dm = 64 * H
        qkv, ctx, dctx, dqkv = _rb(dev, B * N, 3 * Dm), _rb(dev, B * N, Dm), _rb(dev, B * N, Dm), _rb(dev, B * N, 3 * Dm)
        lse = torch.empty(B * H * N, device=dev)
        delta = torch.empty(B * H * N, device=dev)
        p = lambda t: ctypes.c_void_p(t.data_ptr())
        fwd = lambda: _lib.check(lib.bvc_op_attention_fwd(p(qkv), p(ctx), p(lse), B, N, H, 64, st()), "attention_fwd")
        dq = lambda: _lib.check(lib.bvc_op_attention_bwd_part(p(qkv), p(ctx), p(dctx), p(lse), p(delta), p(dqkv), B, N, H, 64, 1, st()), "attention_bwd dq")
        dkv = lambda: _lib.check(lib.bvc_op_attention_bwd_part(p(qkv), p(ctx), p(dctx), p(lse), p(delta), p(dqkv), B, N, H, 64, 2, st()), "attention_bwd dkdv")
        unit = 2.0 * N * N * 64 * H * B
        tok = 2.0 * B * N * Dm
        add("bvc::attn_fwd_kernel<64>", f"{label} attention fwd", count, _time(fwd), 2 * unit, 4 * tok)
        if N <= 160:
            bwd = lambda: _lib.check(lib.bvc_op_attention_bwd(p(qkv), p(ctx), p(dctx), p(lse), p(delta), p(dqkv), B, N, H, 64, st()), "attention_bwd")
            add(f"bvc::attn_bwd_head_kernel<64, {5 if N > 128 else 0}>", f"{label} attention bwd (whole head: S, dP, dV, dK, dQ)", count, _time(bwd),
                5 * unit, 8 * tok)
            continue
        add("bvc::attn_bwd_dq_kernel<64>", f"{label} attention bwd dQ (S, dP, dQ)", count, _time(dq), 3 * unit, 6 * tok)
        add("bvc::attn_bwd_dkdv_kernel<64>", f"{label} attention bwd dK dV (recomputes S, dP)", count, _time(dkv), 2 * unit, 6 * tok)


def _layernorm_rows(dev, B, add):
    lib = _lib.lib()
    st = _lib.current_stream_ptr
    p = lambda t: ctypes.c_void_p(t.data_ptr())
    fused = bool(lib.bvc_op_row_ln_selected(B * 1568, 384, 1536, 6))
    for label, M, Dm, count, count_bwd in (("enc", B * 160, 768, 24, 24), ("dec", B * 1568, 384, 1 if fused else 8, 0 if fused else 8),
                                           ("final", B * 1408, 384, 1, 1)):
        x, dres = torch.randn(M, Dm, device=dev), torch.randn(M, Dm, device=dev)
        gmm, bta = torch.ones(Dm, device=dev), torch.zeros(Dm, device=dev)
        y, dy, dresb = _rb(dev, M, Dm), _rb(dev, M, Dm), _rb(dev, M, Dm)
        mean, rstd = torch.empty(M, device=dev), torch.empty(M, device=dev)
        dg, db = torch.zeros(Dm, device=dev), torch.zeros(Dm, device=dev)
        ws = torch.empty(int(lib.bvc_op_layernorm_bwd_workspace(M, Dm)), device=dev)
        fwd = lambda: _lib.check(lib.bvc_op_layernorm_fwd(p(x), 0, 0, 0, p(gmm), p(bta), p(y), p(mean), p(rstd), M, Dm, 1e-12, st()), "layernorm_fwd")
        bwd = lambda: _lib.check(lib.bvc_op_layernorm_bwd(p(dy), p(x), 0, 0, 0, p(mean), p(rstd), p(gmm), p(dres), 1, p(dresb), p(dg), p(db),
                                                          p(ws), M, Dm, st()), "layernorm_bwd")
        e = float(M) * Dm
        add("bvc::ln_fwd_kernel", f"{label} LayerNorm fwd", count, _time(fwd), 0.0, 6 * e)
        if count_bwd:
            add("bvc::ln_bwd_kernel (+ ln_param_reduce)", f"{label} LayerNorm bwd", count_bwd, _time(bwd), 0.0, 16 * e)


def step_kernels(batch, device):
    rows = {}

    def add(kernel, label, count, us, flops, nbytes):
        r = rows.setdefault(kernel, {"kernel": kernel, "launches_per_step": 0, "us_per_step": 0.0, "flops": 0.0, "bytes": 0.0, "products": []})
        r["launches_per_step"] += count
        r["us_per_step"] += count * us
        r["flops"] += count * flops
        r["bytes"] += count * nbytes
        r["products"].append({"name": label, "launches": count, "launch_us": round(us, 1),
                              "tflops": round(flops / us / 1e6, 1), "gb_per_s": round(nbytes / us / 1e3, 1)})

    with torch.no_grad():
        _gemm_rows(device, batch, add)
        _attention_rows(device, batch, add)
        _layernorm_rows(device, batch, add)
    torch.cuda.empty_cache()
    out = sorted(rows.values(), key=lambda r: -r["us_per_step"])
    total = sum(r["us_per_step"] for r in out)
    for r in out:
        us = r["us_per_step"]
        t_mfma, t_hbm = r["flops"] / (PEAK_BF16_TFLOPS * 1e6), r["bytes"] / (PEAK_HBM_GBS * 1e3)
        r["share_of_probed"] = round(us / total, 4)
        r["tflops"] = round(r["flops"] / us / 1e6, 1)
        r["gb_per_s"] = round(r["bytes"] / us / 1e3, 1)
        r["bound"] = "hbm" if t_hbm > t_mfma else "mfma"
        r["frac"] = round(max(t_mfma, t_hbm) / us, 4)
        r["us_per_step"] = round(us, 1)
        r["algorithmic_flops"] = r.pop("flops")
        r["algorithmic_bytes"] = r.pop("bytes")
    return out, total
```

### include/bvc.h

```cpp
#ifndef BVC_H
#define BVC_H

#include <stddef.h>
#include <stdint.h>

#ifdef __cplusplus
extern "C" {
#endif

#define BVC_OK 0
#define BVC_ERR_INVALID (-1)
#define BVC_ERR_HIP (-2)
#define BVC_ERR_STATE (-3)

const char* bvc_last_error(void);
const char* bvc_version(void);
int bvc_set_option(const char* name, int value);
int bvc_get_option(const char* name);
int64_t bvc_deterministic_workspace_bytes(void);
int bvc_deterministic_workspace_release(void);

typedef struct bvc_videomae_config {
    int image_size, patch_size, num_channels, num_frames, tubelet_size;
    int hidden_size, num_hidden_layers, num_attention_heads, intermediate_size;
// ... 212 lines not shown
                           void* stream);
int bvc_op_layernorm_fwd(const float* x, int rin, int rout, int roff, const float* gamma, const float* beta, void* y_bf16,
                         float* mean, float* rstd, int M, int D, float eps, void* stream);
int bvc_op_layernorm_bwd(const void* dy_bf16, const float* x, int rin, int rout, int roff, const float* mean,
                         const float* rstd, const float* gamma, float* dres, int accumulate, void* dres_bf16,
                         float* dgamma, float* dbeta, float* workspace, int M, int D, void* stream);
int64_t bvc_op_layernorm_bwd_workspace(int M, int D);
int bvc_op_layernorm_bwd_gate(const void* dy_bf16, const float* x, const float* mean, const float* rstd, const float* gamma, float* dres,
                              int accumulate, void* dres_bf16, float* dgamma, float* dbeta, float* workspace, int M, int D,
                              const bvc_branch_drop* drop, int layer, int branch, void* stream);
int bvc_op_colsum_bf16(const void* X, int M, int N, int ld, float alpha, const float* alpha_dev, float* out, void* stream);
int bvc_op_colsum_f32(const float* X, int rin, int rout, int roff, int M, int D, float* out, void* stream);
int bvc_op_cast_bf16(const float* in, void* out, int64_t n, void* stream);
int bvc_op_row_normalize(const float* f, void* fn_bf16, float* inv_norm, int n, int p, float eps, void* stream);
int bvc_op_row_normalize_bwd(const float* f, const float* inv_norm, const float* dfn, float* df, int n, int p, void* stream);
int bvc_op_nce_finalize(const float* partial, int ntiles, float inv_temperature, int64_t npos, float* loss, float* stats, void* stream);
int bvc_op_sgd_step(float* params, float* grads, float* momentum_buf, int64_t n, float lr, float momentum, float dampening,
                    float weight_decay, int nesterov, int first_step, int maximize, const float* grad_scale,
                    const float* found_inf, int write_unscaled_grads, void* bf16_shadow, void* stream);
int bvc_op_adam_prepare(float* state3, double lr, double beta1, double beta2, const float* found_inf, void* stream);
int bvc_op_adam_step(float* params, float* grads, float* exp_avg, float* exp_avg_sq, int64_t n, double lr, double beta1, double beta2,
                     double eps, double weight_decay, int decoupled, int maximize, const float* state3, const float* grad_scale,
                     const float* found_inf, int write_unscaled_grads, void* bf16_shadow, void* stream);
#define BVC_OPT_MAX_GROUPS 8
typedef struct bvc_sgd_groups {
    int ngroups;
    float lr[BVC_OPT_MAX_GROUPS], momentum[BVC_OPT_MAX_GROUPS], dampening[BVC_OPT_MAX_GROUPS], weight_decay[BVC_OPT_MAX_GROUPS];
    int nesterov[BVC_OPT_MAX_GROUPS], first_step[BVC_OPT_MAX_GROUPS], maximize[BVC_OPT_MAX_GROUPS];
} bvc_sgd_groups;
typedef struct bvc_adam_groups {
    int ngroups;
    double lr[BVC_OPT_MAX_GROUPS], beta1[BVC_OPT_MAX_GROUPS], beta2[BVC_OPT_MAX_GROUPS], eps[BVC_OPT_MAX_GROUPS], weight_decay[BVC_OPT_MAX_GROUPS];
    int decoupled[BVC_OPT_MAX_GROUPS], maximize[BVC_OPT_MAX_GROUPS];
} bvc_adam_groups;
int bvc_op_sgd_step_segments(float* params, float* grads, float* momentum_buf, int64_t n, const int64_t* seg_start, const int32_t* seg_group,
                             const int32_t* blk_seg, int nseg, const bvc_sgd_groups* groups, const float* grad_scale, const float* found_inf,
                             int write_unscaled_grads, void* bf16_shadow, void* stream);
int bvc_op_adam_step_segments(float* params, float* grads, float* exp_avg, float* exp_avg_sq, int64_t n, const int64_t* seg_start,
                              const int32_t* seg_group, const int32_t* blk_seg, int nseg, const bvc_adam_groups* groups, float* state,
                              double* hyper_scratch, const float* grad_scale, const float* found_inf, int write_unscaled_grads,
                              void* bf16_shadow, void* stream);
#define BVC_OPT_TABLE_MAX_GROUPS 1024
#define BVC_OPT_TABLE_CHUNK 64
int bvc_op_sgd_step_table(float* params, float* grads, float* momentum_buf, int64_t n, const int64_t* seg_start, const int32_t* seg_group,
                          const int32_t* blk_seg, int nseg, int ngroups, const float* lr, const float* momentum, const float* dampening,
                          const float* weight_decay, const int32_t* nesterov, const int32_t* first_step, const int32_t* maximize,
                          float* group_table, const float* grad_scale, const float* found_inf, int write_unscaled_grads,
                          void* bf16_shadow, void* stream);
int bvc_op_adam_step_table(float* params, float* grads, float* exp_avg, float* exp_avg_sq, int64_t n, const int64_t* seg_start,
                           const int32_t* seg_group, const int32_t* blk_seg, int nseg, int ngroups, const double* lr, const double* beta1,
                           const double* beta2, const double* eps, const double* weight_decay, const int32_t* decoupled,
                           const int32_t* maximize, float* state, float* group_table, const float* grad_scale, const float* found_inf,
                           int write_unscaled_grads, void* bf16_shadow, void* stream);
int bvc_op_nonfinite_check(const float* x, int64_t n, float* found_inf, void* stream);
#define BVC_GRAD_NORM_ITEM_CAP 16384
typedef struct bvc_norm_item {
    int64_t start;
    int32_t length;
    int32_t segment;
} bvc_norm_item;
int bvc_op_grad_norm_item_cap(void);
int bvc_op_grad_norm_chain(void);
int bvc_grad_norm_items_host(const int64_t* seg_start, const int32_t* seg_group, int nseg, bvc_norm_item* items, int64_t items_cap,
                             int64_t* seg_first_item, int64_t* nitems);
int bvc_op_grad_sqnorm_items(const float* x, const bvc_norm_item* items, int64_t nitems, const int64_t* seg_first_item, int nseg,
                             double* item_partial, float* seg_sq, float* total_sq, int as_norm, float* found_inf, void* stream);
int bvc_op_clip_finalize(const float* sq, int nranges, float max_norm, const float* grad_scale, float* out3, void* stream);
int bvc_op_scale_by_dev(float* x, int64_t n, const float* coef, void* stream);
int bvc_op_lars_step_table(float* params, float* grads, float* momentum_buf, int64_t n, const int64_t* seg_start, const int32_t* seg_group,
                           const int32_t* blk_seg, int nseg, const bvc_norm_item* items, int64_t nitems, const int64_t* seg_first_item,
                           int ngroups, const float* lr, const float* momentum, const float* weight_decay, const float* trust_coefficient,
                           const int32_t* nesterov, const int32_t* adapt, const int32_t* maximize, float* group_table, double* item_partial,
                           float* seg_stats, const float* grad_scale, float* found_inf, int write_unscaled_grads, void* bf16_shadow,
                           void* stream);
int bvc_op_lamb_step_table(float* params, float* grads, float* exp_avg, float* exp_avg_sq, int64_t n, const int64_t* seg_start,
                           const int32_t* seg_group, const int32_t* blk_seg, int nseg, const bvc_norm_item* items, int64_t nitems,
                           const int64_t* seg_first_item, int ngroups, const double* lr, const double* beta1, const double* beta2,
                           const double* eps, const double* weight_decay, const int32_t* adapt, const int32_t* maximize, float* state,
                           float* group_table, double* item_partial, float* seg_stats, const float* grad_scale, const float* found_inf,
                           int write_unscaled_grads, void* bf16_shadow, void* stream);
int bvc_op_mask_index(const uint8_t* mask, int B, int L, int nvis, int nmask, int* vis_idx, int* msk_idx, int* status, void* stream);
int bvc_op_dual_mask_index(const uint8_t* mask, const uint8_t* decode_mask, int B, int L, int nvis, int ndec, int* vis_idx, int* dec_idx,
                           int* status, void* stream);
int bvc_op_gather_patches(const float* clip, const int* vis_idx, void* A_bf16, int B, int nvis, int T, int C, int H, int W,
                          int ts, int ps, void* stream);
int bvc_op_gather_patches_mix(const void* clip, const bvc_pixel_format* fmt, const int* idx, void* A_bf16, const bvc_clip_mix* mix,
                              int B, int n, int T, int C, int H, int W, int ts, int ps, void* stream);
int bvc_op_pixel_labels(const float* clip, const int* msk_idx, float* labels, int B, int nmask, int T, int C, int H, int W,
                        int ts, int ps, int norm_pix, void* stream);

#define BVC_COMM_ID_BYTES 128
typedef struct bvc_comm bvc_comm;
int bvc_comm_unique_id(void* id_out_host );
int bvc_comm_init(int rank, int world, const void* id_host, bvc_comm** out);
int bvc_comm_destroy(bvc_comm* comm);
void* bvc_comm_stream(const bvc_comm* comm);
int bvc_comm_rank(const bvc_comm* comm);
int bvc_comm_world(const bvc_comm* comm);
const char* bvc_comm_library(void);
int bvc_allreduce_bucket(bvc_comm* comm, float* buf_dev, int64_t count, int average, void* producer_stream);
int bvc_comm_wait(bvc_comm* comm, void* stream);
int bvc_allgather(bvc_comm* comm, const void* send_dev, void* recv_dev, int64_t bytes_per_rank, void* stream);
int bvc_allreduce(bvc_comm* comm, float* buf_dev, int64_t count, int average, void* stream);
int bvc_broadcast(bvc_comm* comm, void* buf_dev, int64_t bytes, int root, void* stream);

#ifdef __cplusplus
}
#endif
#endif
```

Measured before the change: 3355 clips/s.

## Compute first decoder layer's masked-token rows once per position table

In the first decoder layer, every masked-token row is just mask_token plus a positional embedding, so its LayerNorm and QKV projection depend only on the patch position. The change computes these for a table of positions (2*L rows) once and assembles per-clip QKV by gathering, instead of running the GEMM over all B*ndec masked rows. In backward, gradients for masked rows are summed per position (first_reduce with a bf16 hi/lo pair) before the dX/dW GEMMs, which shrinks the K dimension. The cost is extra gather, scatter and reduce kernels, more arena memory, and hi/lo bf16 splitting to keep accuracy. The path is gated by a heuristic option (dec_first=-1, auto).

```diff
diff --git a/baby-vision-curriculum_amd/_lib.py b/baby-vision-curriculum_amd/_lib.py
--- a/baby-vision-curriculum_amd/_lib.py
+++ b/baby-vision-curriculum_amd/_lib.py
@@ -216,6 +216,9 @@
                                      c_int, c_void_p, c_void_p, c_void_p, c_void_p, c_int, c_int, c_void_p]),
     "bvc_op_layernorm_bwd_workspace": (c_int64, [c_int, c_int]),
     "bvc_op_colsum_bf16": (c_int, [c_void_p, c_int, c_int, c_int, c_float, c_void_p, c_void_p, c_void_p]),
+    "bvc_op_dec_first_selected": (c_int, [c_int, c_int]),
+    "bvc_op_dec_slot": (c_int, [c_void_p, c_void_p, c_int, c_int, c_int, c_void_p]),
+    "bvc_op_first_reduce": (c_int, [c_void_p, c_void_p, c_int, c_int, c_int, c_int, c_int, c_void_p, c_void_p, c_void_p, c_void_p]),
     "bvc_op_colsum_f32": (c_int, [c_void_p, c_int, c_int, c_int, c_int, c_int, c_void_p, c_void_p]),
     "bvc_op_cast_bf16": (c_int, [c_void_p, c_void_p, c_int64, c_void_p]),
     "bvc_op_row_normalize": (c_int, [c_void_p, c_void_p, c_void_p, c_int, c_int, c_float, c_void_p]),
diff --git a/baby-vision-curriculum_amd/csrc/context.h b/baby-vision-curriculum_amd/csrc/context.h
--- a/baby-vision-curriculum_amd/csrc/context.h
+++ b/baby-vision-curriculum_amd/csrc/context.h
@@ -40,9 +40,10 @@
     int embed_backward(Work& w, int M, int D, float* gw, float* gb, hipStream_t st);
 };
 
-int stack_forward(Work& w, Stack& s, const std::vector<LayerOff>& off, int B, int N, hipStream_t st, bool chain_ln, const LayerTail* last = nullptr);
+int stack_forward(Work& w, Stack& s, const std::vector<LayerOff>& off, int B, int N, hipStream_t st, bool chain_ln, const LayerTail* last = nullptr,
+                  const LayerFirst* first = nullptr);
 int stack_backward(Work& w, Stack& s, const std::vector<LayerOff>& off, float* dres, float* G, int B, int N, hipStream_t st,
-                   bvc_bucket_fn on_bucket, void* user, const LayerTail* last = nullptr);
+                   bvc_bucket_fn on_bucket, void* user, const LayerTail* last = nullptr, const LayerFirst* first = nullptr);
 int join_both(Work& w, hipStream_t st, bvc_bucket_fn on_bucket, void* user);
 
 int param_info(const ParamTable& t, int index, char* name, int name_cap, int64_t* offset, int64_t* numel, int* ndim, int64_t shape[5]);
diff --git a/baby-vision-curriculum_amd/csrc/context.hip b/baby-vision-curriculum_amd/csrc/context.hip
--- a/baby-vision-curriculum_amd/csrc/context.hip
+++ b/baby-vision-curriculum_amd/csrc/context.hip
@@ -88,19 +88,20 @@
     return launch_gemm(&p, 1, GEMM_TN, tile, st);
 }
 
-int stack_forward(Work& w, Stack& s, const std::vector<LayerOff>& off, int B, int N, hipStream_t st, bool chain_ln, const LayerTail* last) {
+int stack_forward(Work& w, Stack& s, const std::vector<LayerOff>& off, int B, int N, hipStream_t st, bool chain_ln, const LayerTail* last,
+                  const LayerFirst* first) {
     for (int i = 0; i < s.nlayers; ++i) {
         const bool end = i + 1 == s.nlayers;
         TRY(layer_forward(w, s, i, off[i], s.act[i].x_in, end ? s.x_out : s.act[i + 1].x_in, B, N, st, chain_ln && !end ? &off[i + 1] : nullptr,
-                          end ? last : nullptr));
+                          end ? last : nullptr, i == 0 ? first : nullptr));
     }
     return BVC_OK;
 }
 
 int stack_backward(Work& w, Stack& s, const std::vector<LayerOff>& off, float* dres, float* G, int B, int N, hipStream_t st,
-                   bvc_bucket_fn on_bucket, void* user, const LayerTail* last) {
+                   bvc_bucket_fn on_bucket, void* user, const LayerTail* last, const LayerFirst* first) {
     for (int i = s.nlayers - 1; i >= 0; --i)
-        TRY(layer_backward(w, s, i, off[i], s.act[i].x_in, dres, G, B, N, st, on_bucket, user, i + 1 == s.nlayers ? last : nullptr));
+        TRY(layer_backward(w, s, i, off[i], s.act[i].x_in, dres, G, B, N, st, on_bucket, user, i + 1 == s.nlayers ? last : nullptr, i == 0 ? first : nullptr));
     return BVC_OK;
 }
 
diff --git a/baby-vision-curriculum_amd/csrc/gemm.h b/baby-vision-curriculum_amd/csrc/gemm.h
--- a/baby-vision-curriculum_amd/csrc/gemm.h
+++ b/baby-vision-curriculum_amd/csrc/gemm.h
@@ -30,7 +30,7 @@
 
 constexpr int kMaxGroup = 4;
 
-struct Options { int gemm8 = 0; int dw_overlap = 0; int row_ln = 0; int row_stagger = 1; int deterministic = 0; int head_pad = 0; int dec_tail = 1; };
+struct Options { int gemm8 = 0; int dw_overlap = 0; int row_ln = 0; int row_stagger = 1; int deterministic = 0; int head_pad = 0; int dec_tail = 1; int dec_first = -1; };
 Options& options();
 
 float* det_scratch(size_t floats, hipStream_t stream);
diff --git a/baby-vision-curriculum_amd/csrc/ops.hip b/baby-vision-curriculum_amd/csrc/ops.hip
--- a/baby-vision-curriculum_amd/csrc/ops.hip
+++ b/baby-vision-curriculum_amd/csrc/ops.hip
@@ -32,6 +32,7 @@
     else if (!strcmp(name, "deterministic")) { BVC_REQUIRE(value == 0 || value == 1, "set_option: deterministic takes 0 / 1"); options().deterministic = value; }
     else if (!strcmp(name, "head_pad")) { BVC_REQUIRE(value == 0 || value == 1, "set_option: head_pad takes 0 / 1"); options().head_pad = value; }
     else if (!strcmp(name, "dec_tail")) { BVC_REQUIRE(value == 0 || value == 1, "set_option: dec_tail takes 0 / 1"); options().dec_tail = value; }
+    else if (!strcmp(name, "dec_first")) { BVC_REQUIRE(value >= -1 && value <= 1, "set_option: dec_first takes -1 / 0 / 1"); options().dec_first = value; }
     else BVC_REQUIRE(false, "set_option: unknown option '%s'", name);
     return BVC_OK;
 }
@@ -43,6 +44,7 @@
     if (name && !strcmp(name, "deterministic")) return options().deterministic;
     if (name && !strcmp(name, "head_pad")) return options().head_pad;
     if (name && !strcmp(name, "dec_tail")) return options().dec_tail;
+    if (name && !strcmp(name, "dec_first")) return options().dec_first;
     bvc::set_error("get_option: unknown option '%s'", name ? name : "(null)");
     return BVC_ERR_INVALID;
 }
@@ -199,6 +201,14 @@
     s.hd = width / heads; s.hdp = attn_width(s.hd); s.Da = heads * s.hdp;
     return fuse_row_ln(s, tokens) ? 1 : 0;
 }
+int bvc_op_dec_first_selected(int clips, int decoder_layers) {
+    if (clips <= 0 || decoder_layers <= 0) return 0;
+    Work w;
+    Stack s;
+    s.D = 384; s.I = 1536; s.H = 6; s.nlayers = decoder_layers; s.eps = 0.f; s.x_out = nullptr;
+    s.hd = 64; s.hdp = attn_width(s.hd); s.Da = s.H * s.hdp;
+    return layer_first_ok(w, s, clips, 1, 1) ? 1 : 0;
+}
 int bvc_op_sgd_step_segments(float* params, float* grads, float* momentum_buf, int64_t n, const int64_t* seg_start, const int32_t* seg_group,
                              const int32_t* blk_seg, int nseg, const bvc_sgd_groups* groups, const float* grad_scale, const float* found_inf,
                              int write_unscaled_grads, void* bf16_shadow, void* stream) {
@@ -308,6 +318,15 @@
     BVC_REQUIRE(B >= 1 && L >= 1 && nvis >= 1 && nvis < L && ndec >= 1 && ndec <= L - nvis, "op_dual_mask_index: bad counts (L %d, nvis %d, ndec %d)", L, nvis, ndec);
     return launch_dual_mask_index(mask, decode_mask, B, L, nvis, ndec, vis_idx, dec_idx, status, (hipStream_t)stream);
 }
+int bvc_op_dec_slot(const int* dec_idx, int* dec_slot, int B, int L, int ndec, void* stream) {
+    BVC_REQUIRE(dec_idx && dec_slot && B >= 1 && L >= 1 && ndec >= 1 && ndec <= L, "op_dec_slot: bad argument");
+    return launch_dec_slot(dec_idx, dec_slot, B, L, ndec, (hipStream_t)stream);
+}
+int bvc_op_first_reduce(const void* dqkv, const int* dec_slot, int B, int L, int Ld, int nvis, int W, float* S, void* hi_bf16, void* lo_bf16,
+                        void* stream) {
+    BVC_REQUIRE(dqkv && dec_slot, "op_first_reduce: null argument");
+    return launch_first_reduce((const bf16_t*)dqkv, dec_slot, B, L, Ld, nvis, W, S, (bf16_t*)hi_bf16, (bf16_t*)lo_bf16, (hipStream_t)stream);
+}
 int bvc_op_gather_patches(const float* clip, const int* vis_idx, void* A, int B, int nvis, int T, int C, int H, int W, int ts,
                           int ps, void* stream) {
     BVC_REQUIRE(clip && vis_idx && A, "op_gather_patches: null argument");
diff --git a/baby-vision-curriculum_amd/csrc/rowops.h b/baby-vision-curriculum_amd/csrc/rowops.h
--- a/baby-vision-curriculum_amd/csrc/rowops.h
+++ b/baby-vision-curriculum_amd/csrc/rowops.h
@@ -47,6 +47,13 @@
 int launch_labels(PixelSrc clip, const int* dec_idx, float* labels, int B, int ndec, PatchGeom pg, int norm_pix, hipStream_t s);
 int launch_fill_masked(float* xfull, const float* mask_token, const float* pos, const int* dec_idx, int B, int Ld, int nvis,
                        int ndec, int D, hipStream_t s);
+int launch_dec_slot(const int* dec_idx, int* dec_slot, int B, int L, int ndec, hipStream_t s);
+int launch_first_assemble(const bf16_t* qkv_vis, const bf16_t* t2, const float* t0, const int* dec_idx, bf16_t* qkv, float* xfull, int B,
+                          int nvis, int ndec, int W, int D, hipStream_t s);
+int launch_first_reduce(const bf16_t* dqkv, const int* dec_slot, int B, int L, int Ld, int nvis, int W, float* S, bf16_t* hi, bf16_t* lo,
+                        hipStream_t s);
+int launch_gather_rows_copy_bf16(const bf16_t* in, RowMap rm, bf16_t* out, int M, int W, hipStream_t s);
+int launch_pair_split(const float* a, const float* b, bf16_t* hi, bf16_t* lo, size_t n, hipStream_t s);
 int launch_sgd_step(float* p, float* g, float* buf, size_t n, float lr, float momentum, float dampening, float wd, int nesterov,
                     int first, int maximize, const float* grad_scale, const float* found_inf, int write_grad, bf16_t* shadow,
                     hipStream_t s);
diff --git a/baby-vision-curriculum_amd/csrc/rowops.hip b/baby-vision-curriculum_amd/csrc/rowops.hip
--- a/baby-vision-curriculum_amd/csrc/rowops.hip
+++ b/baby-vision-curriculum_amd/csrc/rowops.hip
@@ -782,6 +782,96 @@
     reinterpret_cast<f32x4*>(xfull + ((size_t)b * Ld + nvis + j) * D)[c] = mt + pe;
 }
 
+__global__ void dec_slot_kernel(const int* __restrict__ dec_idx, int* __restrict__ dec_slot, int B, int L, int ndec) {
+    const size_t i = (size_t)blockIdx.x * blockDim.x + threadIdx.x;
+    if (i >= (size_t)B * ndec) return;
+    const int b = (int)(i / ndec), p = dec_idx[i];
+    if ((unsigned)p < (unsigned)L) dec_slot[(size_t)b * L + p] = (int)(i % ndec);
+}
+
+__global__ void first_assemble_kernel(const bf16_t* __restrict__ qkv_vis, const bf16_t* __restrict__ t2, const float* __restrict__ t0,
+                                      const int* __restrict__ dec_idx, bf16_t* __restrict__ qkv, float* __restrict__ xfull, int B,
+                                      int nvis, int ndec, int W, int D) {
+    const size_t i = (size_t)blockIdx.x * blockDim.x + threadIdx.x;
+    const int wch = W >> 3, dch = D >> 2, Ld = nvis + ndec;
+    const size_t n1 = (size_t)B * Ld * wch;
+    if (i < n1) {
+        const size_t row = i / wch;
+        const int c = (int)(i % wch), b = (int)(row / Ld), r = (int)(row % Ld);
+        const bf16_t* src = r < nvis ? qkv_vis + ((size_t)b * nvis + r) * W : t2 + (size_t)dec_idx[(size_t)b * ndec + (r - nvis)] * W;
+        reinterpret_cast<uint4*>(qkv + row * W)[c] = reinterpret_cast<const uint4*>(src)[c];
+        return;
+    }
+    const size_t j = i - n1;
+    if (j >= (size_t)B * ndec * dch) return;
+    const size_t m = j / dch;
+    const int c = (int)(j % dch), b = (int)(m / ndec), jj = (int)(m % ndec);
+    reinterpret_cast<f32x4*>(xfull + ((size_t)b * Ld + nvis + jj) * D)[c] = reinterpret_cast<const f32x4*>(t0 + (size_t)dec_idx[m] * D)[c];
+}
+
+constexpr int kFirstReduceClips = 8;
+__global__ __launch_bounds__(64) void first_reduce_kernel(const bf16_t* __restrict__ dqkv, const int* __restrict__ dec_slot, int B, int L,
+                                                          int Ld, int nvis, int W, float* __restrict__ S, bf16_t* __restrict__ hi,
+                                                          bf16_t* __restrict__ lo) {
+    const int p = blockIdx.x, col = (blockIdx.y * 64 + threadIdx.x) * 8;
+    if (col >= W) return;
+    float acc[8] = {0.f, 0.f, 0.f, 0.f, 0.f, 0.f, 0.f, 0.f};
+    for (int b0 = 0; b0 < B; b0 += kFirstReduceClips) {
+        uint4 v[kFirstReduceClips];
+#pragma unroll
+        for (int u = 0; u < kFirstReduceClips; ++u) {
+            const int b = b0 + u;
+            const int slot = b < B ? dec_slot[(size_t)b * L + p] : -1;
+            v[u] = slot >= 0 ? *reinterpret_cast<const uint4*>(dqkv + ((size_t)b * Ld + nvis + slot) * W + col) : uint4{0u, 0u, 0u, 0u};
+        }
+#pragma unroll
+        for (int u = 0; u < kFirstReduceClips; ++u) {
+            const uint32_t w[4] = {v[u].x, v[u].y, v[u].z, v[u].w};
+#pragma unroll
+            for (int e = 0; e < 4; ++e) {
+                acc[2 * e] += __uint_as_float(w[e] << 16);
+                acc[2 * e + 1] += __uint_as_float(w[e] & 0xffff0000u);
+            }
+        }
+    }
+    const size_t o = (size_t)p * W + col;
+    if (S) {
+        *reinterpret_cast<f32x4*>(S + o) = f32x4{acc[0], acc[1], acc[2], acc[3]};
+        *reinterpret_cast<f32x4*>(S + o + 4) = f32x4{acc[4], acc[5], acc[6], acc[7]};
+    }
+    if (hi) {
+        uint32_t h[4], l[4];
+#pragma unroll
+        for (int e = 0; e < 4; ++e) {
+            h[e] = pack2bf(acc[2 * e], acc[2 * e + 1]);
+            l[e] = pack2bf(acc[2 * e] - __uint_as_float(h[e] << 16), acc[2 * e + 1] - __uint_as_float(h[e] & 0xffff0000u));
+        }
+        *reinterpret_cast<uint4*>(hi + o) = uint4{h[0], h[1], h[2], h[3]};
+        *reinterpret_cast<uint4*>(lo + o) = uint4{l[0], l[1], l[2], l[3]};
+    }
+}
+
+__global__ void gather_rows_copy_bf16_kernel(const bf16_t* __restrict__ in, RowMap rm, bf16_t* __restrict__ out, int M, int W) {
+    const size_t i = (size_t)blockIdx.x * blockDim.x + threadIdx.x;
+    const int nch = W >> 3;
+    if (i >= (size_t)M * nch) return;
+    const int m = (int)(i / nch), c = (int)(i % nch);
+    reinterpret_cast<uint4*>(out + (size_t)m * W)[c] = reinterpret_cast<const uint4*>(in + (size_t)map_row(m, rm) * W)[c];
+}
+
+__global__ void pair_split_kernel(const float* __restrict__ a, const float* __restrict__ b, bf16_t* __restrict__ hi, bf16_t* __restrict__ lo,
+                                  size_t n) {
+    const size_t i = (size_t)blockIdx.x * blockDim.x + threadIdx.x;
+    if (i >= n) return;
+    f32x4 v = reinterpret_cast<const f32x4*>(a)[i];
+    if (b) v += reinterpret_cast<const f32x4*>(b)[i];
+    const uint32_t h0 = pack2bf(v[0], v[1]), h1 = pack2bf(v[2], v[3]);
+    const uint32_t l0 = pack2bf(v[0] - __uint_as_float(h0 << 16), v[1] - __uint_as_float(h0 & 0xffff0000u));
+    const uint32_t l1 = pack2bf(v[2] - __uint_as_float(h1 << 16), v[3] - __uint_as_float(h1 & 0xffff0000u));
+    reinterpret_cast<uint2*>(hi)[i] = uint2{h0, h1};
+    reinterpret_cast<uint2*>(lo)[i] = uint2{l0, l1};
+}
+
 __global__ __launch_bounds__(256) void loss_finalize_kernel(const float* __restrict__ partial, int n, double count,
                                                             const int* __restrict__ status, float* __restrict__ loss) {
     __shared__ double red[256];
@@ -1807,6 +1897,45 @@
     return BVC_OK;
 }
 
+int launch_dec_slot(const int* dec_idx, int* dec_slot, int B, int L, int ndec, hipStream_t s) {
+    BVC_CHECK_HIP(hipMemsetAsync(dec_slot, 0xff, (size_t)B * L * sizeof(int), s));
+    hipLaunchKernelGGL(dec_slot_kernel, dim3(blocks_for((size_t)B * ndec)), dim3(256), 0, s, dec_idx, dec_slot, B, L, ndec);
+    BVC_CHECK_HIP(hipGetLastError());
+    return BVC_OK;
+}
+
+int launch_first_assemble(const bf16_t* qkv_vis, const bf16_t* t2, const float* t0, const int* dec_idx, bf16_t* qkv, float* xfull, int B,
+                          int nvis, int ndec, int W, int D, hipStream_t s) {
+    BVC_REQUIRE(W % 8 == 0 && D % 4 == 0, "first_assemble: W must be a multiple of 8, D of 4");
+    const size_t items = (size_t)B * (nvis + ndec) * (W / 8) + (size_t)B * ndec * (D / 4);
+    hipLaunchKernelGGL(first_assemble_kernel, dim3(blocks_for(items)), dim3(256), 0, s, qkv_vis, t2, t0, dec_idx, qkv, xfull, B, nvis, ndec, W, D);
+    BVC_CHECK_HIP(hipGetLastError());
+    return BVC_OK;
+}
+
+int launch_first_reduce(const bf16_t* dqkv, const int* dec_slot, int B, int L, int Ld, int nvis, int W, float* S, bf16_t* hi, bf16_t* lo,
+                        hipStream_t s) {
+    BVC_REQUIRE(B >= 1 && L >= 1 && W >= 8 && W % 8 == 0 && nvis >= 0 && Ld > nvis, "first_reduce: bad shape (B %d, L %d, Ld %d, nvis %d, W %d)", B, L, Ld, nvis, W);
+    BVC_REQUIRE((hi == nullptr) == (lo == nullptr) && (S || hi), "first_reduce: no output, or half of the bf16 pair");
+    hipLaunchKernelGGL(first_reduce_kernel, dim3(L, (W + 511) / 512), dim3(64), 0, s, dqkv, dec_slot, B, L, Ld, nvis, W, S, hi, lo);
+    BVC_CHECK_HIP(hipGetLastError());
+    return BVC_OK;
+}
+
+int launch_gather_rows_copy_bf16(const bf16_t* in, RowMap rm, bf16_t* out, int M, int W, hipStream_t s) {
+    BVC_REQUIRE(W % 8 == 0, "gather_rows_copy_bf16: W must be a multiple of 8");
+    hipLaunchKernelGGL(gather_rows_copy_bf16_kernel, dim3(blocks_for((size_t)M * (W / 8))), dim3(256), 0, s, in, rm, out, M, W);
+    BVC_CHECK_HIP(hipGetLastError());
+    return BVC_OK;
+}
+
+int launch_pair_split(const float* a, const float* b, bf16_t* hi, bf16_t* lo, size_t n, hipStream_t s) {
+    BVC_REQUIRE(n % 4 == 0 && n > 0, "pair_split: the element count must be a positive multiple of 4");
+    hipLaunchKernelGGL(pair_split_kernel, dim3(blocks_for(n / 4)), dim3(256), 0, s, a, b, hi, lo, n / 4);
+    BVC_CHECK_HIP(hipGetLastError());
+    return BVC_OK;
+}
+
 int launch_target_select(const float* h, const int* idx, float* out, int nsets, int B, int Np, int L, int D, float eps, hipStream_t s) {
     BVC_REQUIRE(D % 4 == 0 && D <= kWideChunks * 256, "target_select: D=%d unsupported", D);
     const int rows = nsets * B * Np;
diff --git a/baby-vision-curriculum_amd/csrc/stack.h b/baby-vision-curriculum_amd/csrc/stack.h
--- a/baby-vision-curriculum_amd/csrc/stack.h
+++ b/baby-vision-curriculum_amd/csrc/stack.h
@@ -96,6 +96,23 @@
 struct LayerTail { int nvis, ndec; };
 bool layer_tail_ok(const Work& w, const Stack& s, int B, int nvis, int ndec);
 
+struct LayerFirst {
+    int nvis, ndec, L;
+    const int* dec_idx;
+    const int* dec_slot;
+    const float* t0;
+    float *tmean, *trstd;
+    bf16_t* ln1c;
+    bf16_t* qc;
+    float *xt, *dt;
+    bf16_t* dyt;
+    float* part;
+    float* xv;
+    bf16_t* dyv;
+    float* dtoken;
+};
+bool layer_first_ok(const Work& w, const Stack& s, int B, int nvis, int ndec);
+
 LayerOff add_layer_params(ParamTable& t, const std::string& prefix, int64_t d, int64_t inter, bool hf_names);
 int alloc_stack(Arena& a, Stack& s, int D, int I, int H, int nlayers, float eps, size_t M, size_t BHN);
 int alloc_work(Arena& a, Work& w, size_t MD, size_t MI, size_t delta_elems, size_t lnpart_elems);
@@ -107,7 +124,7 @@
 int join_side(Work& w, int parity, hipStream_t st, bvc_bucket_fn on_bucket, void* user);
 void begin_backward(Work& w);
 int layer_forward(Work& w, Stack& s, int li, const LayerOff& o, const float* x_in, float* x_out, int B, int N, hipStream_t st,
-                  const LayerOff* next = nullptr, const LayerTail* tail = nullptr);
+                  const LayerOff* next = nullptr, const LayerTail* tail = nullptr, const LayerFirst* first = nullptr);
 bool fuse_row_ln(const Stack& s, int M);
 int set_drop(DropState& d, const bvc_branch_drop* drop, int samples, const char* who, hipStream_t st);
 int alloc_drop(Arena& a, DropState& d, int nlayers, int max_samples);
@@ -118,6 +135,6 @@
     return &store;
 }
 int layer_backward(Work& w, Stack& s, int li, const LayerOff& o, const float* x_in, float* dres, float* G, int B, int N,
-                   hipStream_t st, bvc_bucket_fn on_bucket, void* user, const LayerTail* tail = nullptr);
+                   hipStream_t st, bvc_bucket_fn on_bucket, void* user, const LayerTail* tail = nullptr, const LayerFirst* first = nullptr);
 
 }
diff --git a/baby-vision-curriculum_amd/csrc/stack.hip b/baby-vision-curriculum_amd/csrc/stack.hip
--- a/baby-vision-curriculum_amd/csrc/stack.hip
+++ b/baby-vision-curriculum_amd/csrc/stack.hip
@@ -157,6 +157,34 @@
         const bool long_enough = g8 > 0 ? ksteps >= 2 : (ksteps >= 16 && flops >= 80e9);
         if (ok && by384 && long_enough && units256 * 65536.0 >= 1.2 * outs) {
             const int smax = std::max(1, std::min(24, ksteps / (g8 > 0 ? 2 : 16)));
+            int kmax = 0;
+            for (int i = 0; i < n; ++i) kmax = std::max(kmax, (g[i].K + 63) / 64);
+            if (kmax >= 2 * ksteps) {
+                const int per_min = g8 > 0 ? 2 : 16;
+                int best_sp = 0;
+                double best_cost = 1e300;
+                for (int sp = 1; sp <= std::max(1, std::min(24, kmax / per_min)); ++sp) {
+                    const int len = (kmax + sp - 1) / sp;
+                    int units = 0, longest = 0;
+                    for (int i = 0; i < n; ++i) {
+                        const int kt = (g[i].K + 63) / 64;
+                        const int si = std::max(1, std::min((kt + len - 1) / len, std::max(1, kt / per_min)));
+                        units += ((g[i].M + 127) / 128) * ((g[i].N + 383) / 384) * si;
+                        longest = std::max(longest, (kt + si - 1) / si);
+                    }
+                    const int rounds = (units + 255) / 256;
+                    const double cost = (double)rounds * longest + 4.0 * rounds;
+                    if (cost < best_cost * 0.999) { best_cost = cost; best_sp = sp; }
+                }
+                const int len = (kmax + best_sp - 1) / best_sp;
+                int units = 0;
+                for (int i = 0; i < n; ++i) {
+                    const int kt = (g[i].K + 63) / 64;
+                    g[i].split_k = std::max(1, std::min((kt + len - 1) / len, std::max(1, kt / per_min)));
+                    units += ((g[i].M + 127) / 128) * ((g[i].N + 383) / 384) * g[i].split_k;
+                }
+                if (units >= (g8 > 0 ? 1 : 160)) return 12;
+            }
             int best = 1;
             double best_cost = 1e300;
             for (int sp = 1; sp <= smax; ++sp) {
@@ -222,6 +250,16 @@
     return fuse_row_ln(s, B * (nvis + ndec)) && gemm_row_ln_ok(B * ndec, s.D, s.D);
 }
 
+constexpr int kFirstAutoClips = 64;
+bool layer_first_ok(const Work& w, const Stack& s, int B, int nvis, int ndec) {
+    const int mode = options().dec_first;
+    if (mode == 0 || s.nlayers < 2 || nvis < 1 || ndec < 1 || B < 1) return false;
+    if (w.drop != nullptr && w.drop->active) return false;
+    if (s.hdp != s.hd || s.D % 8 != 0) return false;
+    if (mode > 0) return true;
+    return B >= kFirstAutoClips;
+}
+
 int alloc_drop(Arena& a, DropState& d, int nlayers, int max_samples) {
     d.nlayers = nlayers;
     d.max_samples = max_samples;
@@ -259,7 +297,7 @@
 }
 
 int layer_forward(Work& w, Stack& s, int li, const LayerOff& o, const float* x_in, float* x_out, int B, int N, hipStream_t st,
-                  const LayerOff* next, const LayerTail* tail) {
+                  const LayerOff* next, const LayerTail* tail, const LayerFirst* first) {
     LayerAct& a = s.act[li];
     const int D = s.D, I = s.I, M = B * N;
     const int Mq = tail ? B * tail->ndec : M;
@@ -271,7 +309,13 @@
     const int gl = w.drop_layer >= 0 ? w.drop_layer : li;
     const bool fuse = !gated && fuse_row_ln(s, M);
     if (li == 0) s.ln1_ready = false;
-    if (!(fuse && s.ln1_ready)) TRY(launch_ln_fwd(x_in, identity_rows(), P + o.ln1w, P + o.ln1b, a.ln1o, a.mean1, a.rstd1, M, D, eps, st));
+    if (first) BVC_REQUIRE(li == 0 && !tail && x_in == a.x_in && first->nvis + first->ndec == N && layer_first_ok(w, s, B, first->nvis, first->ndec),
+                           "layer_forward: first mode is not available for this layer");
+    if (first) {
+        const int Mv = B * first->nvis;
+        TRY(launch_ln_fwd(first->t0, identity_rows(), P + o.ln1w, P + o.ln1b, first->ln1c + (size_t)Mv * D, first->tmean, first->trstd, 2 * first->L, D, eps, st));
+        TRY(launch_ln_fwd(x_in, RowMap{first->nvis, N, 0}, P + o.ln1w, P + o.ln1b, first->ln1c, a.mean1, a.rstd1, Mv, D, eps, st));
+    } else if (!(fuse && s.ln1_ready)) TRY(launch_ln_fwd(x_in, identity_rows(), P + o.ln1w, P + o.ln1b, a.ln1o, a.mean1, a.rstd1, M, D, eps, st));
     s.ln1_ready = false;
     const int Da = s.Da;
     const bool pad = s.hdp != s.hd;
@@ -282,7 +326,14 @@
         TRY(launch_pad_heads(W + o.wqkv, P + o.bqkv, W + o.wo, s.wqkv_pad, s.bqkv_pad, s.wo_pad, D, s.H, s.hd, s.hdp, st));
         Wqkv = s.wqkv_pad; Wo = s.wo_pad; bqkv = s.bqkv_pad;
     }
-    {
+    if (first) {
+        const int Mf = B * first->nvis + first->L;
+        GemmProblem p = gemm(first->ln1c, (size_t)Mf * D, D, Wqkv, (size_t)3 * Da * D, D, Mf, 3 * Da, D, EPI_BF16, first->qc, 3 * Da);
+        p.bias = bqkv;
+        TRY(launch_gemm(&p, 1, GEMM_NT, -1, st));
+        TRY(launch_first_assemble(first->qc, first->qc + (size_t)B * first->nvis * 3 * Da, first->t0, first->dec_idx, a.qkv, a.x_in, B, first->nvis,
+                                  first->ndec, 3 * Da, D, st));
+    } else {
         GemmProblem p = gemm(a.ln1o, (size_t)M * D, D, Wqkv, (size_t)3 * Da * D, D, M, 3 * Da, D, EPI_BF16, a.qkv, 3 * Da);
         p.bias = bqkv;
         TRY(launch_gemm(&p, 1, GEMM_NT, -1, st));
@@ -327,7 +378,7 @@
 }
 
 int layer_backward(Work& c_, Stack& s, int li, const LayerOff& o, const float* x_in, float* dres, float* G, int B, int N,
-                   hipStream_t st, bvc_bucket_fn on_bucket, void* user, const LayerTail* tail) {
+                   hipStream_t st, bvc_bucket_fn on_bucket, void* user, const LayerTail* tail, const LayerFirst* first) {
     LayerAct& a = s.act[li];
     const int D = s.D, I = s.I, M = B * N;
     const int Mq = tail ? B * tail->ndec : M;
@@ -374,7 +425,20 @@
     }
     if (tail) TRY(launch_attn_bwd_win(a.qkv, a.ctx, c_.dctx, a.lse, c_.delta, dqkv, B, N, s.H, s.hdp, tail->nvis, tail->ndec, st, sm_scale));
     else TRY(launch_attn_bwd(a.qkv, a.ctx, c_.dctx, a.lse, c_.delta, dqkv, B, N, s.H, s.hdp, st, sm_scale));
-    if (fuse) {
+    const int Mv = first ? B * first->nvis : 0, Lp = first ? first->L : 0;
+    if (first) {
+        BVC_REQUIRE(li == 0 && !tail && !pad && !gated && first->nvis + first->ndec == N && first->dtoken, "layer_backward: first mode is not available for this layer");
+        const int W3 = 3 * Da;
+        bf16_t* shi = first->qc + (size_t)Mv * W3;
+        TRY(launch_first_reduce(dqkv, first->dec_slot, B, Lp, N, first->nvis, W3, nullptr, shi, shi + (size_t)Lp * W3, st));
+        TRY(launch_gather_rows_copy_bf16(dqkv, RowMap{first->nvis, N, 0}, first->qc, Mv, W3, st));
+        GemmProblem p = gemm(first->qc, (size_t)Mv * W3, W3, Wqkv, (size_t)W3 * D, D, Mv, D, W3, fuse ? EPI_F32 : EPI_BF16, fuse ? (void*)first->xv : (void*)c_.dln, D);
+        TRY(launch_gemm(&p, 1, GEMM_NN, -1, st));
+        if (fuse) TRY(launch_pair_split(first->xv, nullptr, first->dyv, first->dyv + (size_t)Mv * D, (size_t)Mv * D, st));
+        GemmProblem t = gemm(shi, (size_t)2 * Lp * W3, W3, Wqkv, (size_t)W3 * D, D, 2 * Lp, D, W3, EPI_F32, first->xt, D);
+        TRY(launch_gemm(&t, 1, GEMM_NN, -1, st));
+        TRY(launch_pair_split(first->xt, first->xt + (size_t)Lp * D, first->dyt, first->dyt + (size_t)Lp * D, (size_t)Lp * D, st));
+    } else if (fuse) {
         GemmProblem p = gemm(dqkv, (size_t)M * 3 * Da, 3 * Da, Wqkv, (size_t)3 * Da * D, D, M, D, 3 * Da, EPI_DLN, dres, D);
         p.C2 = dyb_next; p.ln_x = x_in; p.ln_mean = a.mean1; p.ln_rstd = a.rstd1; p.ln_gamma = P + o.ln1w;
         p.ln_part = c_.ln_part; p.ln_dgamma = G + o.ln1w; p.ln_dbeta = G + o.ln1b;
@@ -395,6 +459,10 @@
         g[1] = gemm(dh, (size_t)Mq * I, I, a.ln2o, (size_t)Mq * D, D, I, D, Mq, EPI_F32, G + o.w1, D);
         g[2] = gemm(dhb, (size_t)Mq * D, D, a.ctx, (size_t)Mq * Da, Da, D, Da, Mq, EPI_F32, pad ? s.gwo_pad : G + o.wo, Da);
         g[3] = gemm(dqkv, (size_t)M * 3 * Da, 3 * Da, a.ln1o, (size_t)M * D, D, 3 * Da, D, M, EPI_F32, pad ? s.gwqkv_pad : G + o.wqkv, D);
+        if (first) {
+            const int Kf = Mv + 2 * Lp;
+            g[3] = gemm(first->qc, (size_t)Kf * 3 * Da, 3 * Da, first->ln1c, (size_t)Kf * D, D, 3 * Da, D, Kf, EPI_F32, G + o.wqkv, D);
+        }
         g[0].rowsum = G + o.b2;
         g[1].rowsum = G + o.b1;
         g[2].rowsum = G + o.bo;
@@ -409,7 +477,14 @@
         if (pad)
             TRY(launch_unpad_head_grads(s.gwqkv_pad, s.gbqkv_pad, s.gwo_pad, G + o.wqkv, G + o.bqkv, G + o.wo, D, s.H, s.hd, s.hdp, ws));
     }
-    if (!fuse) TRY(launch_ln_bwd(c_.dln, x_in, identity_rows(), a.mean1, a.rstd1, P + o.ln1w, dres, 1, dyb_next, G + o.ln1w, G + o.ln1b, c_.ln_part, M, D, st,
+    if (first) {
+        const RowMap vis{first->nvis, N, 0};
+        TRY(launch_ln_bwd(fuse ? first->dyv : c_.dln, x_in, vis, a.mean1, a.rstd1, P + o.ln1w, dres, 1, nullptr, G + o.ln1w, G + o.ln1b, c_.ln_part, Mv, D, st));
+        if (fuse) TRY(launch_ln_bwd(first->dyv + (size_t)Mv * D, x_in, vis, a.mean1, a.rstd1, P + o.ln1w, dres, 1, nullptr, G + o.ln1w, G + o.ln1b, c_.ln_part, Mv, D, st));
+        TRY(launch_ln_bwd(first->dyt, first->t0, identity_rows(), first->tmean, first->trstd, P + o.ln1w, first->dt, 0, nullptr, G + o.ln1w, G + o.ln1b,
+                          first->part, 2 * Lp, D, st));
+        TRY(launch_colsum_f32(first->dt, identity_rows(), 2 * Lp, D, first->dtoken, st));
+    } else if (!fuse) TRY(launch_ln_bwd(c_.dln, x_in, identity_rows(), a.mean1, a.rstd1, P + o.ln1w, dres, 1, dyb_next, G + o.ln1w, G + o.ln1b, c_.ln_part, M, D, st,
                                  gated && li > 0 ? &g_below : nullptr));
     if (c_.overlap) {
         BVC_CHECK_HIP(hipEventRecord(c_.ev_join[par], c_.side));
diff --git a/baby-vision-curriculum_amd/csrc/videomae.hip b/baby-vision-curriculum_amd/csrc/videomae.hip
--- a/baby-vision-curriculum_amd/csrc/videomae.hip
+++ b/baby-vision-curriculum_amd/csrc/videomae.hip
@@ -84,6 +84,9 @@
     float *dres_enc, *dres_dec;
     bf16_t* de2d;
     bool tail_on = false;
+    int *dec_slot = nullptr, *pos_iota = nullptr;
+    LayerFirst first{};
+    bool first_on = false;
 };
 
 namespace {
@@ -181,6 +184,28 @@
                    std::max(ln_bwd_workspace_floats_upto((int)Mv, D), ln_bwd_workspace_floats_upto((int)Md, Dd))));
     TRY(upload_sinusoid(c->pos_enc, L, D));
     TRY(upload_sinusoid(c->pos_dec, L, Dd));
+    if (c->dec.nlayers >= 2 && c->dec.hdp == c->dec.hd) {
+        LayerFirst& f = c->first;
+        const size_t T = 2 * (size_t)L, Mf = Mv + T;
+        float* t0 = nullptr;
+        f.nvis = nvis; f.ndec = num_decoded; f.L = L;
+        TRY(c->arena.alloc(&c->dec_slot, B * L));
+        TRY(c->arena.alloc(&c->pos_iota, T));
+        TRY(c->arena.alloc(&t0, T * Dd));
+        TRY(c->arena.alloc(&f.tmean, T));
+        TRY(c->arena.alloc(&f.trstd, T));
+        TRY(c->arena.alloc(&f.ln1c, Mf * Dd));
+        TRY(c->arena.alloc(&f.qc, Mf * 3 * c->dec.Da));
+        TRY(c->arena.alloc(&f.xt, T * Dd));
+        TRY(c->arena.alloc(&f.dt, T * Dd));
+        TRY(c->arena.alloc(&f.dyt, T * Dd));
+        TRY(c->arena.alloc(&f.part, ln_bwd_workspace_floats_upto((int)T, Dd)));
+        TRY(c->arena.alloc(&f.xv, Mv * Dd));
+        TRY(c->arena.alloc(&f.dyv, 2 * Mv * Dd));
+        f.t0 = t0; f.dec_idx = c->dec_idx; f.dec_slot = c->dec_slot;
+        TRY(launch_iota_mod(c->pos_iota, (int)T, L, nullptr));
+        BVC_CHECK_HIP(hipStreamSynchronize(nullptr));
+    }
     guard.done = true;
     *out = c;
     return BVC_OK;
@@ -228,10 +253,16 @@
         p.rowtok = c->vis_idx; p.pos = c->pos_dec; p.rin = nvis; p.rout = Ld;
         TRY(launch_gemm(&p, 1, GEMM_NT, -1, st));
     }
-    TRY(launch_fill_masked(c->dec.act[0].x_in, params + L.mask_token, c->pos_dec, c->dec_idx, B, Ld, nvis, ndec, Dd, st));
+    c->first_on = c->dec_slot != nullptr && layer_first_ok(c->w, c->dec, B, nvis, ndec);
+    if (c->first_on) {
+        TRY(launch_dec_slot(c->dec_idx, c->dec_slot, B, Lq, ndec, st));
+        TRY(launch_fill_masked(const_cast<float*>(c->first.t0), params + L.mask_token, c->pos_dec, c->pos_iota, 1, 2 * Lq, 0, 2 * Lq, Dd, st));
+    } else {
+        TRY(launch_fill_masked(c->dec.act[0].x_in, params + L.mask_token, c->pos_dec, c->dec_idx, B, Ld, nvis, ndec, Dd, st));
+    }
     const LayerTail lt{nvis, ndec};
     c->tail_on = layer_tail_ok(c->w, c->dec, B, nvis, ndec);
-    TRY(stack_forward(c->w, c->dec, L.dec, B, Ld, st, true, c->tail_on ? &lt : nullptr));
+    TRY(stack_forward(c->w, c->dec, L.dec, B, Ld, st, true, c->tail_on ? &lt : nullptr, c->first_on ? &c->first : nullptr));
     const RowMap tail = c->tail_on ? identity_rows() : RowMap{ndec, Ld, nvis};
     TRY(launch_ln_fwd(c->dec.x_out, tail, params + L.norm_w, params + L.norm_b, c->lnf, c->meanf, c->rstdf, Mm, Dd, cf.decoder_norm_eps, st));
     TRY(launch_labels(pixels, c->dec_idx, c->labels, B, ndec, c->front.pg, cf.norm_pix_loss, st));
@@ -287,7 +318,8 @@
                           G + L.norm_w, G + L.norm_b, c->w.ln_part, Mm, Dd, st));
     }
     if (on_bucket) on_bucket(L.norm_w, L.total - L.norm_w, user);
-    TRY(stack_backward(c->w, c->dec, L.dec, c->dres_dec, G, B, Ld, st, on_bucket, user, c->tail_on ? &lt : nullptr));
+    c->first.dtoken = G + L.mask_token;
+    TRY(stack_backward(c->w, c->dec, L.dec, c->dres_dec, G, B, Ld, st, on_bucket, user, c->tail_on ? &lt : nullptr, c->first_on ? &c->first : nullptr));
     TRY(launch_colsum_f32(c->dres_dec, tail, Mm, Dd, G + L.mask_token, st));
     const RowMap headrows{nvis, Ld, 0};
     TRY(launch_gather_rows_bf16(c->dres_dec, headrows, c->de2d, Mv, Dd, st));
diff --git a/baby-vision-curriculum_amd/probe.py b/baby-vision-curriculum_amd/probe.py
--- a/baby-vision-curriculum_amd/probe.py
+++ b/baby-vision-curriculum_amd/probe.py
@@ -89,31 +89,38 @@
         us = _time(lambda: _ops.gemm(d, _ops.TN, tile))
         add(name, label, count, us, 2.0 * Mo * No * K, 2.0 * K * (Mo + No) + 4.0 * Mo * No)
 
-    def dw_group(label, M, Dm, Im, count):
-        dy, act, dh, ln2, dqkv = _rb(dev, M, Dm), _rb(dev, M, Im), _rb(dev, M, Im), _rb(dev, M, Dm), _rb(dev, M, 3 * Dm)
+    def dw_group(label, M, Dm, Im, count, Kq=None):
+        Kq = M if Kq is None else Kq
+        dy, act, dh, ln2, dqkv = _rb(dev, M, Dm), _rb(dev, M, Im), _rb(dev, M, Im), _rb(dev, M, Dm), _rb(dev, Kq, 3 * Dm)
+        lnq = ln2 if Kq == M else _rb(dev, Kq, Dm)
         shapes = [(Dm, Im), (Im, Dm), (Dm, Dm), (3 * Dm, Dm)]
         outs = [torch.zeros(s, device=dev) for s in shapes]
         bs = [torch.zeros(s[0], device=dev) for s in shapes]
         ds = [_ops.gemm_desc(dy, act, Dm, Im, M, E["F32"], outs[0], rowsum=bs[0]),
               _ops.gemm_desc(dh, ln2, Im, Dm, M, E["F32"], outs[1], rowsum=bs[1]),
               _ops.gemm_desc(dy, ln2, Dm, Dm, M, E["F32"], outs[2], rowsum=bs[2]),
-              _ops.gemm_desc(dqkv, ln2, 3 * Dm, Dm, M, E["F32"], outs[3], rowsum=bs[3])]
+              _ops.gemm_desc(dqkv, lnq, 3 * Dm, Dm, Kq, E["F32"], outs[3], rowsum=bs[3])]
         tile, split = _ops.plan_dw(ds)
         name = _ops.gemm_kernel_name(ds, _ops.TN, tile)
         us = _time(lambda: _ops.gemm(ds, _ops.TN, tile), iters=3)
-        fl = 2.0 * M * (2 * Dm * Im + 4 * Dm * Dm)
-        nb = 2.0 * M * (2 * Dm + 2 * Im + 2 * Dm + Dm + 3 * Dm) + 4.0 * (2 * Dm * Im + 4 * Dm * Dm)
-        add(name, f"{label} (tile {tile}, split {split})", count, us, fl, nb)
+        fl = 2.0 * M * (2 * Dm * Im + Dm * Dm) + 2.0 * Kq * 3 * Dm * Dm
+        nb = 2.0 * M * (2 * Dm + 2 * Im + 2 * Dm) + 2.0 * Kq * (Dm + 3 * Dm) + 4.0 * (2 * Dm * Im + 4 * Dm * Dm)
+        splits = split if Kq == M else "/".join(str(d.split_k) for d in ds)
+        add(name, f"{label} (tile {tile}, split {splits})", count, us, fl, nb)
 
     NT, NN = _ops.NT, _ops.NN
     fused = bool(_lib.lib().bvc_op_row_ln_selected(Md, Dd, Id, 6))
+    first = bool(_lib.lib().bvc_op_dec_first_selected(B, 4))
+    nq, Lp = (3, 1568) if first else (4, 0)
     one("patch embed", NT, Mv, D, 1536, "POS", 1)
     one("enc qkv", NT, Mv, 3 * D, D, "BF16", 12)
     one("enc proj", NT, Mv, D, D, "RESID", 12)
     one("enc fc1+GELU", NT, Mv, I, D, "GELU", 12)
     one("enc fc2", NT, Mv, D, I, "RESID", 12)
     one("enc->dec", NT, Mv, Dd, D, "E2D", 1)
-    one("dec qkv", NT, Md, 3 * Dd, Dd, "BF16", 4)
+    one("dec qkv", NT, Md, 3 * Dd, Dd, "BF16", nq)
+    if first:
+        one("dec0 qkv (visible rows, position table)", NT, Mv + Lp, 3 * Dd, Dd, "BF16", 1)
     if fused:
         one("dec proj + LayerNorm", NT, Md, Dd, Dd, "RESID_LN", 4)
     else:
@@ -129,7 +136,10 @@
     one("dec dX fc2", NN, Md, Id, Dd, "DGELU", 4)
     one("dec dX fc1 + LayerNorm bwd" if fused else "dec dX fc1", NN, Md, Dd, Id, "DLN" if fused else "BF16", 4)
     one("dec dX proj", NN, Md, Dd, Dd, "BF16", 4)
-    one("dec dX qkv + LayerNorm bwd" if fused else "dec dX qkv", NN, Md, Dd, 3 * Dd, "DLN" if fused else "BF16", 4)
+    one("dec dX qkv + LayerNorm bwd" if fused else "dec dX qkv", NN, Md, Dd, 3 * Dd, "DLN" if fused else "BF16", nq)
+    if first:
+        one("dec0 dX qkv (visible rows)", NN, Mv, Dd, 3 * Dd, "F32" if fused else "BF16", 1)
+        one("dec0 dX qkv (position sums, bf16 pair)", NN, 2 * Lp, Dd, 3 * Dd, "F32", 1)
     one("enc->dec dX", NN, Mv, D, Dd, "F32_BF16", 1)
     one("enc dX fc2", NN, Mv, I, D, "DGELU", 12)
     one("enc dX fc1", NN, Mv, D, I, "BF16", 12)
@@ -138,7 +148,9 @@
     dw_single("head dW", P, Dd, Mm, 1)
     dw_single("enc->dec dW", Dd, D, Mv, 1)
     dw_single("patch dW", D, 1536, Mv, 1)
-    dw_group("dec layer dW group", Md, Dd, Id, 4)
+    dw_group("dec layer dW group", Md, Dd, Id, nq)
+    if first:
+        dw_group("dec0 layer dW, qkv member by position", Md, Dd, Id, 1, Kq=Mv + 2 * Lp)
     dw_group("enc layer dW group", Mv, D, I, 12)
 
 
diff --git a/include/bvc.h b/include/bvc.h
--- a/include/bvc.h
+++ b/include/bvc.h
@@ -318,6 +318,10 @@
 int bvc_op_mask_index(const uint8_t* mask, int B, int L, int nvis, int nmask, int* vis_idx, int* msk_idx, int* status, void* stream);
 int bvc_op_dual_mask_index(const uint8_t* mask, const uint8_t* decode_mask, int B, int L, int nvis, int ndec, int* vis_idx, int* dec_idx,
                            int* status, void* stream);
+int bvc_op_dec_first_selected(int clips, int decoder_layers);
+int bvc_op_dec_slot(const int* dec_idx, int* dec_slot, int B, int L, int ndec, void* stream);
+int bvc_op_first_reduce(const void* dqkv_bf16, const int* dec_slot, int B, int L, int Ld, int nvis, int W, float* S, void* hi_bf16,
+                        void* lo_bf16, void* stream);
 int bvc_op_gather_patches(const float* clip, const int* vis_idx, void* A_bf16, int B, int nvis, int T, int C, int H, int W,
                           int ts, int ps, void* stream);
 int bvc_op_gather_patches_mix(const void* clip, const bvc_pixel_format* fmt, const int* idx, void* A_bf16, const bvc_clip_mix* mix,
```

New measurement: 3394 clips/s (median of 6 runs). 1.2% higher.
